# mit-han-lab/TinyChatEngine

Hardware: NVIDIA H100
Metric: llama3_8b_awq_int4_batch1_decode_tokens_per_s (higher is better)
Workload: dtype w4a16 (int4 weights; activations fp16 -> 32-bit block fixed point = four int8 digit planes; int32 accumulate, fp32 scale)

## Files before the change

### tinychatengine_b200/csrc/decode_persistent.cu

```cuda
#include <stdio.h>

#include "persistent.h"
#include "w4a16_act_planes.cuh"

namespace tce {
namespace pk {

namespace {

TCE_DEVINL unsigned ld_acquire_gpu(const unsigned *p) {
    unsigned v;
    asm volatile("ld.acquire.gpu.global.u32 %0, [%1];" : "=r"(v) : "l"(p) : "memory");
    return v;
}
TCE_DEVINL void red_release_gpu(unsigned *p) { asm volatile("red.release.gpu.global.add.u32 [%0], 1;" ::"l"(p) : "memory"); }

TCE_DEVINL void st_ll(uint2 *p, uint32_t data, uint32_t tag, bool sys) {
    if (sys)
        asm volatile("st.relaxed.sys.global.v2.b32 [%0], {%1, %2};" ::"l"(p), "r"(data), "r"(tag) : "memory");
    else
        asm volatile("st.relaxed.gpu.global.v2.b32 [%0], {%1, %2};" ::"l"(p), "r"(data), "r"(tag) : "memory");
}
TCE_DEVINL uint4 ld_ll2(const uint2 *p, bool sys) {
    uint4 r;
    if (sys)
        asm volatile("ld.relaxed.sys.global.v4.b32 {%0,%1,%2,%3}, [%4];" : "=r"(r.x), "=r"(r.y), "=r"(r.z), "=r"(r.w) : "l"(p) : "memory");
    else
        asm volatile("ld.relaxed.gpu.global.v4.b32 {%0,%1,%2,%3}, [%4];" : "=r"(r.x), "=r"(r.y), "=r"(r.z), "=r"(r.w) : "l"(p) : "memory");
    return r;
}
TCE_DEVINL uint2 ld_ll1(const uint2 *p, bool sys) {
    uint2 r;
    if (sys)
        asm volatile("ld.relaxed.sys.global.v2.b32 {%0,%1}, [%2];" : "=r"(r.x), "=r"(r.y) : "l"(p) : "memory");
    else
        asm volatile("ld.relaxed.gpu.global.v2.b32 {%0,%1}, [%2];" : "=r"(r.x), "=r"(r.y) : "l"(p) : "memory");
    return r;
}
constexpr unsigned kPeerPollBackoffNs = 100;
constexpr long long kSpinLimit = 20000000000LL;
TCE_DEVINL uint4 wait_ll2(const uint2 *p, uint32_t tag, bool sys) {
    uint4 r = ld_ll2(p, sys);
    if (r.y == tag && r.w == tag) return r;
    const long long t0 = clock64();
    while (true) {
        if (sys) __nanosleep(kPeerPollBackoffNs);
        r = ld_ll2(p, sys);
        if (r.y == tag && r.w == tag) return r;
        if (clock64() - t0 > kSpinLimit) __trap();
    }
}
TCE_DEVINL uint32_t wait_ll1(const uint2 *p, uint32_t tag, bool sys) {
    uint2 r = ld_ll1(p, sys);
    if (r.y == tag) return r.x;
    const long long t0 = clock64();
    while (true) {
        if (sys) __nanosleep(kPeerPollBackoffNs);
        r = ld_ll1(p, sys);
        if (r.y == tag) return r.x;
        if (clock64() - t0 > kSpinLimit) __trap();
    }
}
template <int N>
TCE_DEVINL void wait_ll2xN(const uint2 *p, uint32_t tag, bool sys, uint4 (&r)[N]) {
    long long t0 = 0;
    while (true) {
        bool ok = true;
#pragma unroll
        for (int i = 0; i < N; i++) r[i] = ld_ll2(p + 2 * i, sys);
#pragma unroll
        for (int i = 0; i < N; i++) ok = ok && (r[i].y == tag) && (r[i].w == tag);
        if (ok) return;
        if (t0 == 0) t0 = clock64();
        if (clock64() - t0 > kSpinLimit) __trap();
        if (sys) __nanosleep(kPeerPollBackoffNs);
    }
}

TCE_DEVINL float2 h2_to_f2(uint32_t u) { return __half22float2(*reinterpret_cast<const __half2 *>(&u)); }

TCE_DEVINL uint4 lds_u4(uint32_t a) {
    uint4 r;
    asm volatile("ld.shared.v4.u32 {%0,%1,%2,%3}, [%4];" : "=r"(r.x), "=r"(r.y), "=r"(r.z), "=r"(r.w) : "r"(a) : "memory");
    return r;
}
TCE_DEVINL uint2 lds_u2(uint32_t a) {
    uint2 r;
    asm volatile("ld.shared.v2.u32 {%0,%1}, [%2];" : "=r"(r.x), "=r"(r.y) : "r"(a) : "memory");
    return r;
}
TCE_DEVINL uint32_t lds_u32(uint32_t a) {
    uint32_t r;
    asm volatile("ld.shared.u32 %0, [%1];" : "=r"(r) : "r"(a) : "memory");
    return r;
}
TCE_DEVINL float lds_f32(uint32_t a) { return __uint_as_float(lds_u32(a)); }
TCE_DEVINL uint32_t lds_u16(uint32_t a) {
    unsigned short r;
    asm volatile("ld.shared.u16 %0, [%1];" : "=h"(r) : "r"(a) : "memory");
    return (uint32_t)r;
}
TCE_DEVINL bool mbar_try_wait_u32(uint32_t bar, uint32_t parity) {
    uint32_t ok;
    asm volatile("{\n\t.reg .pred p;\n\tmbarrier.try_wait.parity.shared::cta.b64 p, [%1], %2;\n\tselp.u32 %0, 1, 0, p;\n\t}" : "=r"(ok) : "r"(bar), "r"(parity) : "memory");
    return ok != 0;
}
TCE_DEVINL void mbar_wait_u32(uint32_t bar, uint32_t parity) {
    if (mbar_try_wait_u32(bar, parity)) return;
    const long long t0 = clock64();
    while (!mbar_try_wait_u32(bar, parity)) {
        if (clock64() - t0 > kSpinLimit) __trap();
    }
}
TCE_DEVINL void mbar_arrive_u32(uint32_t bar) { asm volatile("mbarrier.arrive.shared::cta.b64 _, [%0];" ::"r"(bar) : "memory"); }

TCE_DEVINL int lds_volatile_i32(const int *p) {
    int v;
    asm volatile("ld.volatile.shared.s32 %0, [%1];" : "=r"(v) : "r"(smem_u32(p)) : "memory");
    return v;
}

TCE_DEVINL void stamp(const Args &a, int cta, int nphase, int p, int k) {
    if (a.dbg) {
        unsigned long long t;
        asm volatile("mov.u64 %0, %%globaltimer;" : "=l"(t));
        a.dbg[((size_t)cta * nphase + p) * 8 + k] = t;
    }
}

TCE_DEVINL unsigned long long argmax_key(float v, int idx) {
    unsigned b = __float_as_uint(v);
    b = (b & 0x80000000u) ? ~b : (b | 0x80000000u);
    return ((unsigned long long)b << 32) | (unsigned long long)(0xFFFFFFFFu - (unsigned)idx);
}

struct PSmem {
    uint8_t *ring;
    uint8_t *xs;
    float *resid;
    float *gx;
    int *gsum;
    float *red;
    float *rms;
    float *rope;
    uint64_t *full, *empty, *red_full, *red_empty;
    uint64_t *rx;
    int *free_gen;
    int2 *red_pos;
    uint32_t ring_u32, xs_u32, gx_u32, gsum_u32, full_u32, empty_u32, redfull_u32, redempty_u32;
    int nst;
};

TCE_DEVINL PSmem carve(uint8_t *raw, const Args &a) {
    PSmem s;
    uint8_t *base = raw + ((1024u - (smem_u32(raw) & 1023u)) & 1023u);
    s.nst = a.nst;
    s.ring = base;
    uint8_t *p = base + (size_t)a.nst * kStageBytes;
    s.xs = p;
    p += a.xs_bytes;
    s.resid = reinterpret_cast<float *>(p);
    p += (size_t)a.E * 4;
    s.gx = reinterpret_cast<float *>(p);
    p += (size_t)a.max_ng * 4;
    s.gsum = reinterpret_cast<int *>(p);
    p += (size_t)a.max_ng * 8;
    s.red = reinterpret_cast<float *>(p);
    p += (size_t)kRedBufs * kCW * 16 * 4;
    s.rms = reinterpret_cast<float *>(p);
    p += 32 * 4;
    s.rope = reinterpret_cast<float *>(p);
    p += 256 * 4;
    s.full = reinterpret_cast<uint64_t *>(p);
    s.empty = s.full + a.nst;
    s.red_full = s.empty + a.nst;
    s.red_empty = s.red_full + kRedBufs;
    s.rx = s.red_empty + kRedBufs;
    s.free_gen = reinterpret_cast<int *>(s.rx + 1);
    s.red_pos = reinterpret_cast<int2 *>(s.rx + 2);
    s.ring_u32 = smem_u32(s.ring);
    s.xs_u32 = smem_u32(s.xs);
    s.gx_u32 = smem_u32(s.gx);
    s.gsum_u32 = smem_u32(s.gsum);
    s.full_u32 = smem_u32(s.full);
    s.empty_u32 = smem_u32(s.empty);
    s.redfull_u32 = smem_u32(s.red_full);
    s.redempty_u32 = smem_u32(s.red_empty);
    return s;
}

struct Ring {
    int stage = 0;
    uint32_t phase = 0;
    TCE_DEVINL void advance(int nst) {
        if (++stage == nst) {
            stage = 0;
            phase ^= 1;
        }
    }
};
struct Red {
    int rb = 0;
    uint32_t rphase = 0;
    TCE_DEVINL void advance() {
        if (++rb == kRedBufs) {
            rb = 0;
            rphase ^= 1;
        }
    }
};

TCE_DEVINL void partition(const GemvOp &op, int cta, int ncta, int &t0, int &t1) {
    const unsigned T = (unsigned)op.num_tiles;
    t0 = (int)((T * (unsigned)cta) / (unsigned)ncta);
    t1 = (int)((T * (unsigned)(cta + 1)) / (unsigned)ncta);
}

struct AttnSplit {
    int kvh, split, ch0, ch1, nsplit;
};
TCE_DEVINL AttnSplit attn_split(int cta, int ncta, int KVH, int pos) {
    AttnSplit s;
    const int T = pos + 1;
    const int nch = (T + kKvChunk - 1) / kKvChunk;
    int NS = ncta / KVH;
    if (NS < 1) NS = 1;
    int cps = (nch + NS - 1) / NS;
    if (cps * 32 < nch) cps = (nch + 31) / 32;
    s.nsplit = (nch + cps - 1) / cps;
    s.kvh = cta / NS;
    s.split = cta - s.kvh * NS;
    if (s.kvh >= KVH || s.split >= s.nsplit) {
        s.ch0 = s.ch1 = 0;
        s.kvh = 0;
    } else {
        s.ch0 = s.split * cps;
        s.ch1 = min(nch, s.ch0 + cps);
    }
    return s;
}

TCE_DEVINL void produce_gemv(const GemvOp &op, const CUtensorMap *m0, const uint8_t *meta, const PSmem &sm, Ring &rs, int cta, int ncta, uint32_t leader,
                             uint64_t policy) {
    int t0, t1;
    partition(op, cta, ncta, t0, t1);
    const uint32_t box_bytes = 16u * (uint32_t)op.bw * 64u;
    for (int tile = t0; tile < t1; tile++) {
        int row = op.pair ? tile * 8 : tile * 16;
        const CUtensorMap *m = m0;
        if (!op.pair && op.nseg > 1 && row >= op.rows0) {
            row -= op.rows0;
            m = m0 + 1;
            if (op.nseg > 2 && row >= op.rows1) {
                row -= op.rows1;
                m = m0 + 2;
            }
        }
        for (int s = 0; s < op.S; s++) {
            const int nbox = (min(kStageGroups, op.NG - kStageGroups * s) + 15) >> 4;
            mbar_wait(&sm.empty[rs.stage], rs.phase ^ 1);
            uint64_t *bar = &sm.full[rs.stage];
            uint8_t *dst = sm.ring + (size_t)rs.stage * kStageBytes;
            mbar_arrive_expect_tx_pred(bar, (uint32_t)nbox * box_bytes + kMetaBytes, leader);
#pragma unroll 1
            for (int b = 0; b < nbox; b++) {
                const int grp = kStageGroups * s + 16 * b;
                tma_load_3d_pred(dst + b * 16384, m, 0, row, grp, bar, policy, leader);
                if (op.pair) tma_load_3d_pred(dst + b * 16384 + 8192, m + 1, 0, row, grp, bar, policy, leader);
            }
            bulk_g2s_pred(dst + kMetaOff, meta + ((size_t)tile * op.S + s) * kMetaBytes, kMetaBytes, bar, policy, leader);
            __syncwarp();
            rs.advance(sm.nst);
        }
    }
}

TCE_DEVINL void produce_attn(const Args &a, const LayerDesc &L, const CUtensorMap *kvmap, const PSmem &sm, Ring &rs, int cta, int ncta, int pos,
                             uint32_t leader, uint64_t policy) {
    const AttnSplit sp = attn_split(cta, ncta, a.KVH, pos);
    for (int c = sp.ch0; c < sp.ch1; c++) {
        mbar_wait(&sm.empty[rs.stage], rs.phase ^ 1);
        uint64_t *bar = &sm.full[rs.stage];
        uint8_t *dst = sm.ring + (size_t)rs.stage * kStageBytes;
        const int krow = L.k_row0 + sp.kvh * a.max_ctx + c * kKvChunk, vrow = L.v_row0 + sp.kvh * a.max_ctx + c * kKvChunk;
        mbar_arrive_expect_tx_pred(bar, 2u * kHalfBytes, leader);
        tma_load_2d_pred(dst, kvmap, 0, krow, bar, policy, leader);
        tma_load_2d_pred(dst + 8192, kvmap, 64, krow, bar, policy, leader);
        tma_load_2d_pred(dst + kHalfBytes, kvmap, 0, vrow, bar, policy, leader);
        tma_load_2d_pred(dst + kHalfBytes + 8192, kvmap, 64, vrow, bar, policy, leader);
        __syncwarp();
        rs.advance(sm.nst);
    }
}

TCE_DEVINL void producer_walk(const Args &a, const PSmem &sm, int cta, int ncta, int pos, int lane) {
    Ring rs;
    const uint64_t policy = l2_policy_evict_first();
    const uint32_t leader = (lane == 0) ? 1u : 0u;
    const int Lyr = a.num_layers, nphase = 5 * Lyr + 1;
    const CUtensorMap *kvmap = a.maps + (size_t)Lyr * 7 + 1;
#pragma unroll 1
    for (int p = 0; p < nphase; p++) {
        const int l = p / 5, k = p - 5 * l;
        if (l == Lyr) {
            produce_gemv(a.op[OPI_LMHEAD], a.maps + (size_t)Lyr * 7, a.lm_meta, sm, rs, cta, ncta, leader, policy);
        } else if (k == 1) {
            produce_attn(a, a.layers[l], kvmap, sm, rs, cta, ncta, pos, leader, policy);
        } else {
            const int oi = (k == 0) ? OPI_QKV : (k - 1);
            const int mi = (k == 0) ? 0 : (k == 2 ? 3 : (k == 3 ? 4 : 6));
            produce_gemv(a.op[oi], a.maps + (size_t)l * 7 + mi, a.layers[l].meta[oi], sm, rs, cta, ncta, leader, policy);
        }
    }
}

struct PairCtx {
    bool on = false;
    uint32_t rank = 0;
    gemv::PairDst dst = {0u, 0u, 0u, 0u};
    uint32_t r_rms = 0, r_free = 0;
    uint32_t nstage = 0;
};
TCE_DEVINL uint32_t map_to_cta(uint32_t local_u32, uint32_t rank) {
    uint32_t r;
    asm volatile("mapa.shared::cluster.u32 %0, %1, %2;" : "=r"(r) : "r"(local_u32), "r"(rank));
    return r;
}
TCE_DEVINL void st_cluster_u32(uint32_t raddr, uint32_t v) { asm volatile("st.relaxed.cluster.shared::cluster.u32 [%0], %1;" ::"r"(raddr), "r"(v) : "memory"); }
TCE_DEVINL int own_groups(const PairCtx &pc, int NG) { return pc.on ? (NG + 1 - (int)pc.rank) / 2 : NG; }
TCE_DEVINL int peer_groups(const PairCtx &pc, int NG) { return pc.on ? (NG + (int)pc.rank) / 2 : 0; }
TCE_DEVINL void wait_partner_free(const PSmem &sm, const PairCtx &pc, int p) {
    if (!pc.on || p == 0) return;
    const long long t0 = clock64();
    while (lds_volatile_i32(sm.free_gen) < p) {
        if (clock64() - t0 > kSpinLimit) __trap();
    }
}
TCE_DEVINL void rx_expect(const PSmem &sm, const PairCtx &pc, uint32_t bytes) {
    asm volatile("mbarrier.arrive.expect_tx.shared::cta.b64 _, [%0], %1;" ::"r"(smem_u32(sm.rx)), "r"(bytes) : "memory");
}
TCE_DEVINL void rx_wait(const PSmem &sm, PairCtx &pc) {
    mbar_wait_u32(smem_u32(sm.rx), pc.nstage & 1u);
    pc.nstage++;
}

TCE_DEVINL int rot_unit(int u, int units, int cta) {
    const int ng = units >> 4;
    int g = (u >> 4) + (cta % ng);
    if (g >= ng) g -= ng;
    return (g << 4) | (u & 15);
}

TCE_DEVINL void stage_half(const GemvOp &op, const PSmem &sm, PairCtx &pc, const uint2 *src, uint32_t tag, int cta, int ctid, int lane, int p) {
    const int ng_own = own_groups(pc, op.NG);
    const int units = ng_own * 16;
    if (pc.on) {
        if (ctid == 0) rx_expect(sm, pc, (uint32_t)peer_groups(pc, op.NG) * 524u);
        wait_partner_free(sm, pc, p);
    }
    constexpr int PRE = 4;
    for (int ub = 0; ub < units; ub += PRE * kConsumerThreads) {
        uint4 w[PRE][2];
        int ui[PRE];
#pragma unroll
        for (int k = 0; k < PRE; k++) {
            const int u = ub + k * kConsumerThreads + ctid;
            ui[k] = -1;
            if (u < units) {
                const int ru = rot_unit(u, units, cta);
                ui[k] = pc.on ? (((ru >> 4) * 2 + (int)pc.rank) << 4) | (ru & 15) : ru;
            }
            w[k][0] = w[k][1] = make_uint4(0u, tag, 0u, tag);
            if (ui[k] >= 0) {
                w[k][0] = ld_ll2(src + (size_t)ui[k] * 4, false);
                w[k][1] = ld_ll2(src + (size_t)ui[k] * 4 + 2, false);
            }
        }
        {
            long long t0 = 0;
            while (true) {
                bool ok = true;
#pragma unroll
                for (int k = 0; k < PRE; k++) ok = ok && w[k][0].y == tag && w[k][0].w == tag && w[k][1].y == tag && w[k][1].w == tag;
                if (ok) break;
                if (t0 == 0) t0 = clock64();
                if (clock64() - t0 > kSpinLimit) __trap();
#pragma unroll
                for (int k = 0; k < PRE; k++) {
                    if (ui[k] >= 0 && !(w[k][0].y == tag && w[k][0].w == tag && w[k][1].y == tag && w[k][1].w == tag)) {
                        w[k][0] = ld_ll2(src + (size_t)ui[k] * 4, false);
                        w[k][1] = ld_ll2(src + (size_t)ui[k] * 4 + 2, false);
                    }
                }
            }
            __syncwarp();
        }
#pragma unroll
        for (int k = 0; k < PRE; k++) {
            if (ub + k * kConsumerThreads >= units) break;
            const bool valid = ui[k] >= 0;
            float v[8];
            const float2 f0 = h2_to_f2(w[k][0].x), f1 = h2_to_f2(w[k][0].z), f2 = h2_to_f2(w[k][1].x), f3 = h2_to_f2(w[k][1].z);
            v[0] = f0.x; v[1] = f0.y; v[2] = f1.x; v[3] = f1.y;
            v[4] = f2.x; v[5] = f2.y; v[6] = f3.x; v[7] = f3.y;
            if (pc.on)
                gemv::emit_unit<1, true>(sm.xs, op.IC, sm.gx, sm.gsum, valid ? ui[k] : 0, valid, v, lane, &pc.dst);
            else
                gemv::emit_unit<1>(sm.xs, op.IC, sm.gx, sm.gsum, valid ? ui[k] : 0, valid, v, lane);
        }
    }
    named_bar_sync(1, kConsumerThreads);
    if (pc.on) rx_wait(sm, pc);
}

TCE_DEVINL void tp_accumulate(float (&x)[8], const uint2 *slot0, int tp_size, int E, uint32_t tag) {
    int pr = 0;
    for (; pr + 2 <= tp_size; pr += 2) {
        const uint2 *pa = slot0 + (size_t)pr * E, *pb = pa + E;
        uint4 wa[4], wb[4];
        long long t0 = 0;
        while (true) {
            bool ok = true;
#pragma unroll
            for (int i = 0; i < 4; i++) wa[i] = ld_ll2(pa + 2 * i, true);
#pragma unroll
            for (int i = 0; i < 4; i++) wb[i] = ld_ll2(pb + 2 * i, true);
#pragma unroll
            for (int i = 0; i < 4; i++) ok = ok && wa[i].y == tag && wa[i].w == tag && wb[i].y == tag && wb[i].w == tag;
            if (ok) break;
            if (t0 == 0) t0 = clock64();
            if (clock64() - t0 > kSpinLimit) __trap();
            __nanosleep(kPeerPollBackoffNs);
        }
        x[0] += __uint_as_float(wa[0].x); x[1] += __uint_as_float(wa[0].z); x[2] += __uint_as_float(wa[1].x); x[3] += __uint_as_float(wa[1].z);
        x[4] += __uint_as_float(wa[2].x); x[5] += __uint_as_float(wa[2].z); x[6] += __uint_as_float(wa[3].x); x[7] += __uint_as_float(wa[3].z);
        x[0] += __uint_as_float(wb[0].x); x[1] += __uint_as_float(wb[0].z); x[2] += __uint_as_float(wb[1].x); x[3] += __uint_as_float(wb[1].z);
        x[4] += __uint_as_float(wb[2].x); x[5] += __uint_as_float(wb[2].z); x[6] += __uint_as_float(wb[3].x); x[7] += __uint_as_float(wb[3].z);
    }
    if (pr < tp_size) {
        uint4 w[4];
        wait_ll2xN<4>(slot0 + (size_t)pr * E, tag, true, w);
        x[0] += __uint_as_float(w[0].x); x[1] += __uint_as_float(w[0].z); x[2] += __uint_as_float(w[1].x); x[3] += __uint_as_float(w[1].z);
        x[4] += __uint_as_float(w[2].x); x[5] += __uint_as_float(w[2].z); x[6] += __uint_as_float(w[3].x); x[7] += __uint_as_float(w[3].z);
    }
}

TCE_DEVINL float stage_rms(const Args &a, const GemvOp &op, const PSmem &sm, PairCtx &pc, const uint2 *delta, uint32_t tag, const float *gamma, int token,
                           bool first, bool emit, int cta, int ctid, int cw, int lane, int p) {
    const int units = own_groups(pc, op.NG) * 16;
    const bool sys = a.tp_size > 1;
    if (pc.on && emit) {
        if (ctid == 0) rx_expect(sm, pc, (uint32_t)peer_groups(pc, op.NG) * 524u + (uint32_t)kCW * 4u);
        wait_partner_free(sm, pc, p);
    }
    float ss = 0.f;
    for (int ui0 = 0; ui0 < units; ui0 += kConsumerThreads) {
        const int u = ui0 + ctid;
        const bool valid = u < units;
        int ui = 0;
        if (valid) {
            const int ru = rot_unit(u, units, cta);
            ui = pc.on ? (((ru >> 4) * 2 + (int)pc.rank) << 4) | (ru & 15) : ru;
        }
        float x[8], v[8];
#pragma unroll
        for (int i = 0; i < 8; i++) x[i] = 0.f;
        float4 g0 = make_float4(0.f, 0.f, 0.f, 0.f), g1 = g0;
        if (valid) {
            g0 = *reinterpret_cast<const float4 *>(gamma + (size_t)ui * 8);
            g1 = *reinterpret_cast<const float4 *>(gamma + (size_t)ui * 8 + 4);
            if (first) {
                const uint4 raw = *reinterpret_cast<const uint4 *>(a.embed + (size_t)token * a.E + (size_t)ui * 8);
                const __half2 *h2 = reinterpret_cast<const __half2 *>(&raw);
#pragma unroll
                for (int i = 0; i < 4; i++) {
                    const float2 f = __half22float2(h2[i]);
                    x[2 * i] = f.x;
                    x[2 * i + 1] = f.y;
                }
            } else {
                const float4 r0 = *reinterpret_cast<const float4 *>(sm.resid + (size_t)ui * 8);
                const float4 r1 = *reinterpret_cast<const float4 *>(sm.resid + (size_t)ui * 8 + 4);
                x[0] = r0.x; x[1] = r0.y; x[2] = r0.z; x[3] = r0.w;
                x[4] = r1.x; x[5] = r1.y; x[6] = r1.z; x[7] = r1.w;
                if (a.tp_size == 1) {
                    uint4 w[4];
                    wait_ll2xN<4>(delta + (size_t)ui * 8, tag, false, w);
                    x[0] += __uint_as_float(w[0].x); x[1] += __uint_as_float(w[0].z); x[2] += __uint_as_float(w[1].x); x[3] += __uint_as_float(w[1].z);
                    x[4] += __uint_as_float(w[2].x); x[5] += __uint_as_float(w[2].z); x[6] += __uint_as_float(w[3].x); x[7] += __uint_as_float(w[3].z);
                } else {
                    tp_accumulate(x, delta + (size_t)ui * 8, a.tp_size, a.E, tag);
                }
            }
            *reinterpret_cast<float4 *>(sm.resid + (size_t)ui * 8) = make_float4(x[0], x[1], x[2], x[3]);
            *reinterpret_cast<float4 *>(sm.resid + (size_t)ui * 8 + 4) = make_float4(x[4], x[5], x[6], x[7]);
        }
        if (emit) {
#pragma unroll
            for (int i = 0; i < 8; i++) ss += x[i] * x[i];
            v[0] = x[0] * g0.x; v[1] = x[1] * g0.y; v[2] = x[2] * g0.z; v[3] = x[3] * g0.w;
            v[4] = x[4] * g1.x; v[5] = x[5] * g1.y; v[6] = x[6] * g1.z; v[7] = x[7] * g1.w;
            if (pc.on)
                gemv::emit_unit<1, true>(sm.xs, op.IC, sm.gx, sm.gsum, ui, valid, v, lane, &pc.dst);
            else
                gemv::emit_unit<1>(sm.xs, op.IC, sm.gx, sm.gsum, ui, valid, v, lane);
        }
    }
    if (!emit) return 1.f;
    ss = warp_sum(ss);
    if (lane == 0) {
        sm.rms[pc.rank * kCW + cw] = ss;
        if (pc.on) gemv::st_async_b32(pc.r_rms + (uint32_t)(pc.rank * kCW + cw) * 4u, __float_as_uint(ss), pc.dst.bar);
    }
    named_bar_sync(1, kConsumerThreads);
    if (pc.on) rx_wait(sm, pc);
    float tot = 0.f;
    const int nparts = pc.on ? 2 * kCW : kCW;
    for (int w = 0; w < nparts; w++) tot += sm.rms[w];
    return rsqrtf(tot / (float)op.IC + a.eps);
}

struct UnitRegs {
    uint4 wa, wb, xe, xo;
    uint32_t z;
    uint32_t sc;
    int sxv;
    float st;
};
TCE_DEVINL void unit_compute(const UnitRegs &u, float lscale, float &totA, float &totB) {
    constexpr uint32_t ML = 0x0f0f0f0fu, MH = 0xf0f0f0f0u;
    int accL[4], accH[4];
    mma_m16n8k32_u8s8_z(accL, u.wa.x & ML, u.wb.x & ML, u.wa.y & ML, u.wb.y & ML, u.xe.x, u.xe.y);
    mma_m16n8k32_u8s8_z(accH, u.wa.x & MH, u.wb.x & MH, u.wa.y & MH, u.wb.y & MH, u.xo.x, u.xo.y);
    mma_m16n8k32_u8s8(accL, u.wa.z & ML, u.wb.z & ML, u.wa.w & ML, u.wb.w & ML, u.xe.z, u.xe.w);
    mma_m16n8k32_u8s8(accH, u.wa.z & MH, u.wb.z & MH, u.wa.w & MH, u.wb.w & MH, u.xo.z, u.xo.w);
    const float2 sc = h2_to_f2(u.sc);
    const float st = u.st * lscale;
    const int zAq = (int)(u.z & 0xFFu), zBq = (int)(u.z >> 8);
    const int vA = (accL[0] << 8) + accL[1] + (((accH[0] << 8) + accH[1]) >> 4) - zAq * u.sxv;
    const int vB = (accL[2] << 8) + accL[3] + (((accH[2] << 8) + accH[3]) >> 4) - zBq * u.sxv;
    totA += (sc.x * st) * (float)vA;
    totB += (sc.y * st) * (float)vB;
}

TCE_DEVINL void consume_gemv(const Args &a, const GemvOp &op, const PSmem &sm, Ring &rs, float inv_in, int cta, int ncta, int cw, int p, int nphase) {
    int lane;
    asm volatile("mov.u32 %0, %%laneid;" : "=r"(lane));
    const float inv = __shfl_sync(0xffffffffu, inv_in, 0);
    Red cs;
    {
        const int2 rp = sm.red_pos[cw];
        cs.rb = rp.x;
        cs.rphase = (uint32_t)rp.y;
    }
    const int g = lane >> 2, t = lane & 3;
    int t0, t1;
    partition(op, cta, ncta, t0, t1);
    const int NG = op.NG, S = op.S;
    const uint32_t w_lane = (uint32_t)cw * (op.pair ? 512u : 1024u) + (uint32_t)g * 64u + (uint32_t)t * 16u;
    const uint32_t wb_off = op.pair ? 8192u : 512u;
    const uint32_t m_lane = (uint32_t)kMetaOff + (uint32_t)(cw * 8 + g) * 4u;
    const uint32_t z_lane = (uint32_t)kMetaOff + 1024u + (uint32_t)(cw * 8 + g) * 2u;
    const uint32_t x_lane = sm.xs_u32 + (uint32_t)((g >> 1) & 1) * (uint32_t)op.IC * 2u + (uint32_t)(t * 2 + (g & 1)) * 16u + (uint32_t)cw * 256u;
    const uint32_t s_lane = sm.gsum_u32 + (uint32_t)(2 * cw + (t & 1)) * 4u;
    const uint32_t q_lane = sm.gx_u32 + (uint32_t)cw * 4u;
    const float lscale = (t == 0) ? 65536.f : (t == 1 ? 1.f : 0.f);
    const bool xl = g < 4;
    if (a.dbg && t1 > t0 && cw == 0 && lane == 0) {
        mbar_wait_u32(sm.full_u32 + (uint32_t)rs.stage * 8u, rs.phase);
        stamp(a, cta, nphase, p, 4);
    }
    for (int tile = t0; tile < t1; tile++) {
        float totA = 0.f, totB = 0.f;
        for (int s = 0; s < S; s++) {
            const bool has0 = kStageGroups * s + cw < NG, has1 = kStageGroups * s + cw + 16 < NG;
            mbar_wait_u32(sm.full_u32 + (uint32_t)rs.stage * 8u, rs.phase);
            const uint32_t base = sm.ring_u32 + (uint32_t)rs.stage * (uint32_t)kStageBytes;
            const uint32_t wb_ = base + w_lane, mb_ = base + m_lane, zb_ = base + z_lane;
            const uint32_t xb_ = x_lane + (uint32_t)s * (kStageGroups * 256u), sb_ = s_lane + (uint32_t)s * (kStageGroups * 8u), qb_ = q_lane + (uint32_t)s * (kStageGroups * 4u);
            UnitRegs u0, u1;
            u0.xe = u0.xo = u1.xe = u1.xo = make_uint4(0u, 0u, 0u, 0u);
            if (has0) {
                u0.wa = lds_u4(wb_);
                u0.wb = lds_u4(wb_ + wb_off);
                if (xl) {
                    u0.xe = lds_u4(xb_);
                    u0.xo = lds_u4(xb_ + 128u);
                }
                u0.sc = lds_u32(mb_);
                u0.z = lds_u16(zb_);
                u0.sxv = (int)lds_u32(sb_);
                u0.st = lds_f32(qb_);
            }
            if (has1) {
                u1.wa = lds_u4(wb_ + 16384u);
                u1.wb = lds_u4(wb_ + 16384u + wb_off);
                if (xl) {
                    u1.xe = lds_u4(xb_ + 4096u);
                    u1.xo = lds_u4(xb_ + 4096u + 128u);
                }
                u1.sc = lds_u32(mb_ + 512u);
                u1.z = lds_u16(zb_ + 256u);
                u1.sxv = (int)lds_u32(sb_ + 128u);
                u1.st = lds_f32(qb_ + 64u);
            }
            if (has0) unit_compute(u0, lscale, totA, totB);
            if (has1) unit_compute(u1, lscale, totA, totB);
            __syncwarp();
            if (lane == 0) mbar_arrive_u32(sm.empty_u32 + (uint32_t)rs.stage * 8u);
            rs.advance(sm.nst);
        }
        if (tile == t1 - 1 && cw == 0 && lane == 0) stamp(a, cta, nphase, p, 5);
        totA += __shfl_xor_sync(0xffffffffu, totA, 1);
        totB += __shfl_xor_sync(0xffffffffu, totB, 1);
        mbar_wait_u32(sm.redempty_u32 + (uint32_t)cs.rb * 8u, cs.rphase ^ 1);
        float *rbuf = sm.red + ((size_t)cs.rb * kCW + cw) * 16;
        if (t == 0) {
            rbuf[g] = totA * inv;
            rbuf[g + 8] = totB * inv;
        }
        __syncwarp();
        if (lane == 0) mbar_arrive_u32(sm.redfull_u32 + (uint32_t)cs.rb * 8u);
        cs.advance();
    }
    __syncwarp();
    if (lane == 0) sm.red_pos[cw] = make_int2(cs.rb, (int)cs.rphase);
    __syncwarp();
    if (cw == 0 && lane == 0) stamp(a, cta, nphase, p, 6);
}

struct EpiState {
    unsigned long long best;
};

TCE_DEVINL void epilogue_gemv(const Args &a, const GemvOp &op, const PSmem &sm, Red &es, EpiState &st, uint2 *out_ll, int which, uint32_t tag, int cta, int ncta,
                              int p, int nphase) {
    int lane;
    asm volatile("mov.u32 %0, %%laneid;" : "=r"(lane));
    int t0, t1;
    partition(op, cta, ncta, t0, t1);
    const bool tp = a.tp_size > 1;
    for (int tile = t0; tile < t1; tile++) {
        mbar_wait_u32(sm.redfull_u32 + (uint32_t)es.rb * 8u, es.rphase);
        if (tile == t1 - 1 && lane == 0) stamp(a, cta, nphase, p, 7);
        const float *rbuf = sm.red + (size_t)es.rb * kCW * 16;
        float v = 0.f;
        {
            const int row = lane & 15, w0 = (lane >> 4) * 8;
#pragma unroll
            for (int w = 0; w < 8; w++) v += rbuf[(w0 + w) * 16 + row];
        }
        v += __shfl_down_sync(0xffffffffu, v, 16);
        __syncwarp();
        if (lane == 0) mbar_arrive_u32(sm.redempty_u32 + (uint32_t)es.rb * 8u);
        es.advance();
        switch (op.epi) {
            case PE_DELTA_LL:
                if (lane < 16) {
                    const size_t o = (size_t)a.tp_rank * a.E + (size_t)tile * 16 + lane;
                    if (tp) {
                        for (int pr = 0; pr < a.tp_size; pr++) st_ll(a.tp_delta[which][pr] + o, __float_as_uint(v), tag, true);
                    } else {
                        st_ll(out_ll + o, __float_as_uint(v), tag, false);
                    }
                }
                break;
            case PE_HALF_LL: {
                const float hi = __shfl_down_sync(0xffffffffu, v, 1);
                if (lane < 16 && !(lane & 1)) st_ll(out_ll + (size_t)tile * 8 + (lane >> 1), pack_half2(v, hi), tag, false);
                break;
            }
            case PE_SILU_LL: {
                const float up = __shfl_down_sync(0xffffffffu, v, 8);
                const float y = v / (1.f + __expf(-v)) * up;
                const float yhi = __shfl_down_sync(0xffffffffu, y, 1);
                if (lane < 8 && !(lane & 1)) st_ll(out_ll + (size_t)tile * 4 + (lane >> 1), pack_half2(y, yhi), tag, false);
                break;
            }
            case PE_LOGITS:
                if (lane < 16) {
                    const int idx = tile * 16 + lane;
                    a.logits[idx] = v;
                    const unsigned long long key = argmax_key(v, a.vocab_base + idx);
                    st.best = key > st.best ? key : st.best;
                }
                break;
        }
    }
}

TCE_DEVINL uint32_t kv_off(int r, int c) { return (uint32_t)((c >> 3) * 8192 + r * 128 + (((c & 7) ^ (r & 7)) << 4)); }

TCE_DEVINL float2 rope_pair(const uint2 *vec, int j, uint32_t tag, const float *cosr, const float *sinr) {
    const uint2 *pa = vec + j, *pb = vec + (j < 32 ? j + 32 : j - 32);
    uint2 wa = ld_ll1(pa, false), wb = ld_ll1(pb, false);
    if (wa.y != tag) wa.x = wait_ll1(pa, tag, false);
    if (wb.y != tag) wb.x = wait_ll1(pb, tag, false);
    const float2 x = h2_to_f2(wa.x), xp = h2_to_f2(wb.x);
    const float sgn = (j < 32) ? -1.f : 1.f;
    const int d = 2 * j;
    return make_float2(x.x * cosr[d] + sgn * xp.x * sinr[d], x.y * cosr[d + 1] + sgn * xp.y * sinr[d + 1]);
}

TCE_DEVINL void attention_phase(const Args &a, const LayerDesc &L, const PSmem &sm, Ring &rs, uint32_t tag_qkv, uint32_t tag_part, uint32_t tag_out, int cta,
                                int ncta, int pos, int ctid, int cw, int lane, int p, int nphase) {
    const AttnSplit sp = attn_split(cta, ncta, a.KVH, pos);
    const int nrep = a.nrep;
    const int g = lane >> 2, t = lane & 3;
    if (sp.ch0 < sp.ch1) {
        __half *sQ = reinterpret_cast<__half *>(sm.xs);
        float *sO = reinterpret_cast<float *>(sm.xs + 8 * 136 * 2);
        float *sML = sO + (size_t)kCW * nrep * 128;
        uint32_t *sKV = reinterpret_cast<uint32_t *>(sML + (size_t)kCW * nrep * 2);
        const float *cosr = sm.rope, *sinr = sm.rope + 128;
        const bool owns_new = sp.ch1 * kKvChunk > pos;
        static_assert(8 * 64 == kConsumerThreads, "one pass");
        {
            const int r = ctid >> 6, j = ctid & 63;
            float2 v = make_float2(0.f, 0.f);
            if (r < nrep) {
                v = rope_pair(a.qkv_ll + (size_t)(sp.kvh * nrep + r) * 64, j, tag_qkv, cosr, sinr);
                v.x *= a.alpha;
                v.y *= a.alpha;
            } else if (owns_new && r == 7) {
                const float2 kr = rope_pair(a.qkv_ll + (size_t)a.H * 64 + (size_t)sp.kvh * 64, j, tag_qkv, cosr, sinr);
                const __half2 kh = __floats2half2_rn(kr.x, kr.y);
                sKV[j] = *reinterpret_cast<const uint32_t *>(&kh);
            } else if (owns_new && r == 6) {
                sKV[64 + j] = wait_ll1(a.qkv_ll + (size_t)(a.H + a.KVH) * 64 + (size_t)sp.kvh * 64 + j, tag_qkv, false);
            }
            *reinterpret_cast<__half2 *>(sQ + r * 136 + 2 * j) = __floats2half2_rn(v.x, v.y);
        }
        named_bar_sync(1, kConsumerThreads);
        if (ctid == 0) stamp(a, cta, nphase, p, 4);
        const uint32_t qa_u32 = smem_u32(sQ + g * 136 + t * 2);
        float m_run = -INFINITY, l_run = 0.f;
        bool have = false;
        float *myO = sO + (size_t)cw * nrep * 128;
        const int kb = cw & 3;
        for (int c = sp.ch0; c < sp.ch1; c++) {
            const int kbase = c * kKvChunk + kb * 16;
            const bool mine = (((c - sp.ch0) & 3) == (cw >> 2)) && (kbase <= pos);
            const bool has_new = mine && pos < kbase + 16;
            mbar_wait_u32(sm.full_u32 + (uint32_t)rs.stage * 8u, rs.phase);
            if (c == sp.ch0 && ctid == 0) stamp(a, cta, nphase, p, 7);
            if (mine) {
                uint8_t *kst = sm.ring + (size_t)rs.stage * kStageBytes, *vst = kst + kHalfBytes;
                if (has_new) {
                    const int r = pos - c * kKvChunk;
#pragma unroll
                    for (int i = 0; i < 2; i++) {
                        const int j = lane * 2 + i;
                        const uint32_t kh = sKV[j], vv = sKV[64 + j];
                        *reinterpret_cast<uint32_t *>(kst + kv_off(r, j >> 2) + (j & 3) * 4) = kh;
                        *reinterpret_cast<uint32_t *>(vst + kv_off(r, j >> 2) + (j & 3) * 4) = vv;
                        *reinterpret_cast<uint32_t *>(L.k_cache + ((size_t)sp.kvh * a.max_ctx + pos) * 128 + 2 * j) = kh;
                        *reinterpret_cast<uint32_t *>(L.v_cache + ((size_t)sp.kvh * a.max_ctx + pos) * 128 + 2 * j) = vv;
                    }
                    for (int rr = r + 1; rr < kb * 16 + 16; rr++)
                        *reinterpret_cast<uint2 *>(vst + kv_off(rr, lane >> 1) + (lane & 1) * 8) = make_uint2(0u, 0u);
                    asm volatile("fence.proxy.async.shared::cta;" ::: "memory");
                    __syncwarp();
                }
                float s0[4] = {0.f, 0.f, 0.f, 0.f}, s1[4] = {0.f, 0.f, 0.f, 0.f};
                {
                    const int lr = (lane & 7) + ((lane >> 4) << 3);
                    const int lc = (lane >> 3) & 1;
#pragma unroll
                    for (int ks = 0; ks < 8; ks++) {
                        uint32_t b0, b1, b2, b3;
                        ldmatrix_x4(b0, b1, b2, b3, kst + kv_off(kb * 16 + lr, 2 * ks + lc));
                        const uint32_t qa0 = lds_u32(qa_u32 + ks * 32u), qa1 = lds_u32(qa_u32 + ks * 32u + 16u);
                        mma_m16n8k16(s0, qa0, 0u, qa1, 0u, b0, b1);
                        mma_m16n8k16(s1, qa0, 0u, qa1, 0u, b2, b3);
                    }
                }
                const int k0 = kbase + 2 * t;
                float e0 = (k0 <= pos) ? s0[0] : -INFINITY, e1 = (k0 + 1 <= pos) ? s0[1] : -INFINITY;
                float e2 = (k0 + 8 <= pos) ? s1[0] : -INFINITY, e3 = (k0 + 9 <= pos) ? s1[1] : -INFINITY;
                float mb = fmaxf(fmaxf(e0, e1), fmaxf(e2, e3));
                mb = fmaxf(mb, __shfl_xor_sync(0xffffffffu, mb, 1));
                mb = fmaxf(mb, __shfl_xor_sync(0xffffffffu, mb, 2));
                const float m_new = fmaxf(m_run, mb);
                e0 = __expf(e0 - m_new);
                e1 = __expf(e1 - m_new);
                e2 = __expf(e2 - m_new);
                e3 = __expf(e3 - m_new);
                float lb = (e0 + e1) + (e2 + e3);
                lb += __shfl_xor_sync(0xffffffffu, lb, 1);
                lb += __shfl_xor_sync(0xffffffffu, lb, 2);
                const float sc_old = have ? __expf(m_run - m_new) : 0.f;
                l_run = l_run * sc_old + lb;
                m_run = m_new;
                const uint32_t pa0 = pack_half2(e0, e1), pa2 = pack_half2(e2, e3);
                const int lr = (lane & 7) + (((lane >> 3) & 1) << 3);
                const int lc = lane >> 4;
#pragma unroll
                for (int h = 0; h < 2; h++) {
                    float oacc[8][4];
#pragma unroll
                    for (int j = 0; j < 8; j++) oacc[j][0] = oacc[j][1] = oacc[j][2] = oacc[j][3] = 0.f;
#pragma unroll
                    for (int jp = 0; jp < 4; jp++) {
                        uint32_t b0, b1, b2, b3;
                        ldmatrix_x4_t(b0, b1, b2, b3, vst + kv_off(kb * 16 + lr, 8 * h + 2 * jp + lc));
                        mma_m16n8k16(oacc[2 * jp], pa0, 0u, pa2, 0u, b0, b1);
                        mma_m16n8k16(oacc[2 * jp + 1], pa0, 0u, pa2, 0u, b2, b3);
                    }
                    if (g < nrep) {
#pragma unroll
                        for (int j = 0; j < 8; j++) {
                            float2 *dst = reinterpret_cast<float2 *>(myO + g * 128 + 64 * h + 8 * j + 2 * t);
                            float2 nv = make_float2(oacc[j][0], oacc[j][1]);
                            if (have) {
                                const float2 old = *dst;
                                nv.x += old.x * sc_old;
                                nv.y += old.y * sc_old;
                            }
                            *dst = nv;
                        }
                    }
                }
                have = true;
            }
            __syncwarp();
            if (lane == 0) mbar_arrive_u32(sm.empty_u32 + (uint32_t)rs.stage * 8u);
            rs.advance(sm.nst);
        }
        if (ctid == 0) stamp(a, cta, nphase, p, 5);
        if (t == 0 && g < nrep) {
            sML[(cw * nrep + g) * 2] = have ? m_run : -INFINITY;
            sML[(cw * nrep + g) * 2 + 1] = have ? l_run : 0.f;
        }
        named_bar_sync(1, kConsumerThreads);
        const int r = ctid >> 7, d = ctid & 127;
        if (ctid < nrep * 128) {
            float o = 0.f, M = -INFINITY, Lsum = 0.f;
            for (int w = 0; w < kCW; w++) M = fmaxf(M, sML[(w * nrep + r) * 2]);
            for (int w = 0; w < kCW; w++) {
                const float mw = sML[(w * nrep + r) * 2];
                if (mw != -INFINITY) {
                    const float wt = __expf(mw - M);
                    Lsum += wt * sML[(w * nrep + r) * 2 + 1];
                    o += wt * sO[((size_t)w * nrep + r) * 128 + d];
                }
            }
            const int head = sp.kvh * nrep + r;
            if (sp.nsplit == 1) {
                const float y = o / Lsum;
                const float yhi = __shfl_down_sync(0xffffffffu, y, 1);
                if (!(d & 1)) st_ll(a.attn_ll + (size_t)head * 64 + (d >> 1), pack_half2(y, yhi), tag_out, false);
            } else {
                uint2 *rec = a.part_ll + ((size_t)head * a.nsplit_max + sp.split) * 130;
                st_ll(rec + d, __float_as_uint(o), tag_part, false);
                if (d == 0) {
                    st_ll(rec + 128, __float_as_uint(M), tag_part, false);
                    st_ll(rec + 129, __float_as_uint(Lsum), tag_part, false);
                }
            }
        }
    }
    if (ctid == 0) stamp(a, cta, nphase, p, 6);
    if (sp.nsplit == 1) return;
    const int ntask = a.H * 4;
    for (int task = cta + cw * ncta; task < ntask; task += ncta * kCW) {
        const int head = task >> 2, d = ((task & 3) << 5) + lane;
        const uint2 *base = a.part_ll + (size_t)head * a.nsplit_max * 130;
        constexpr int kRound = 20;
        uint2 wm = make_uint2(0u, tag_part), wl = wm;
        uint2 ow[kRound];
#pragma unroll
        for (int i = 0; i < kRound; i++) ow[i] = make_uint2(0u, tag_part);
        {
            const bool stat = lane < sp.nsplit;
            if (stat) wm.y = wl.y = tag_part + 1u;
#pragma unroll
            for (int i = 0; i < kRound; i++)
                if (i < sp.nsplit) ow[i].y = tag_part + 1u;
            long long t0 = 0;
            while (true) {
                if (wm.y != tag_part) wm = ld_ll1(base + (size_t)lane * 130 + 128, false);
                if (wl.y != tag_part) wl = ld_ll1(base + (size_t)lane * 130 + 129, false);
#pragma unroll
                for (int i = 0; i < kRound; i++)
                    if (ow[i].y != tag_part) ow[i] = ld_ll1(base + (size_t)i * 130 + d, false);
                bool ok = wm.y == tag_part && wl.y == tag_part;
#pragma unroll
                for (int i = 0; i < kRound; i++) ok = ok && ow[i].y == tag_part;
                if (ok) break;
                if (t0 == 0) t0 = clock64();
                if (clock64() - t0 > kSpinLimit) __trap();
            }
            __syncwarp();
        }
        const float ms = (lane < sp.nsplit) ? __uint_as_float(wm.x) : -INFINITY, ls = (lane < sp.nsplit) ? __uint_as_float(wl.x) : 0.f;
        const float M = warp_max(ms);
        const float wgt = (lane < sp.nsplit) ? __expf(ms - M) : 0.f;
        const float Lt = warp_sum(wgt * ls);
        float acc = 0.f;
#pragma unroll
        for (int i = 0; i < kRound; i++) acc += __shfl_sync(0xffffffffu, wgt, i) * __uint_as_float(ow[i].x);
        for (int s0 = kRound; s0 < sp.nsplit; s0++)
            acc += __shfl_sync(0xffffffffu, wgt, s0) * __uint_as_float(wait_ll1(base + (size_t)s0 * 130 + d, tag_part, false));
        const float y = acc / Lt;
        const float yhi = __shfl_down_sync(0xffffffffu, y, 1);
        if (!(lane & 1)) st_ll(a.attn_ll + (size_t)head * 64 + (d >> 1), pack_half2(y, yhi), tag_out, false);
    }
}

__global__ void __launch_bounds__(kThreads, 1) decode_persistent_kernel(const __grid_constant__ Args a) {
    extern __shared__ uint8_t smem_raw[];
    const PSmem sm = carve(smem_raw, a);
    const int tid = threadIdx.x, warp = tid >> 5, lane = tid & 31;
    const int cta = blockIdx.x, ncta = gridDim.x;
    const int Lyr = a.num_layers;
    const int token = a.tokpos[0], pos = a.tokpos[1];
    if (token < 0 || token >= a.embed_rows || pos < 0 || pos >= a.max_ctx) {
        if (cta == 0 && tid == 0) {
            *a.error = 1;
            *a.next_token = -1;
        }
        return;
    }
    if (warp == 0) {
        if (lane < a.nst) {
            mbar_init(&sm.full[lane], 1);
            mbar_init(&sm.empty[lane], kCW);
        } else if (lane >= 16 && lane < 16 + kRedBufs) {
            mbar_init(&sm.red_full[lane - 16], kCW);
            mbar_init(&sm.red_empty[lane - 16], 1);
        }
        if (lane == 30) {
            mbar_init(sm.rx, 1);
            *sm.free_gen = 0;
        }
        mbar_fence_init();
    }
    __syncthreads();
    PairCtx pc;
    if (a.pair) {
        asm volatile("barrier.cluster.arrive.release.aligned;" ::: "memory");
        asm volatile("barrier.cluster.wait.acquire.aligned;" ::: "memory");
        pc.on = true;
        asm volatile("mov.u32 %0, %%cluster_ctarank;" : "=r"(pc.rank));
        const uint32_t peer = pc.rank ^ 1u;
        pc.dst.xs = map_to_cta(sm.xs_u32, peer);
        pc.dst.gx = map_to_cta(sm.gx_u32, peer);
        pc.dst.gsum = map_to_cta(sm.gsum_u32, peer);
        pc.dst.bar = map_to_cta(smem_u32(sm.rx), peer);
        pc.r_rms = map_to_cta(smem_u32(sm.rms), peer);
        pc.r_free = map_to_cta(smem_u32(sm.free_gen), peer);
    }
    const int nphase = 5 * Lyr + 1;
    const unsigned epoch = *a.epoch;
    const uint32_t tag_base = epoch * (uint32_t)(2 * nphase + 2) + 1u;

    if (warp < kAuxWarps) {
        asm volatile("setmaxnreg.dec.sync.aligned.u32 64;" ::: "memory");
        if (warp >= 2) return;
        if (warp == 0) {
            producer_walk(a, sm, cta, ncta, pos, lane);
            return;
        }
        Red es;
        EpiState st;
        st.best = 0ull;
#pragma unroll 1
        for (int p = 0; p < nphase; p++) {
            const int l = p / 5, k = p - 5 * l;
            if (l < Lyr && k == 1) continue;
            const int oi = (l == Lyr) ? OPI_LMHEAD : ((k == 0) ? OPI_QKV : (k - 1));
            uint2 *out = (oi == OPI_QKV) ? a.qkv_ll : (oi == OPI_GATEUP ? a.act_ll : (oi == OPI_O ? a.delta_ll[0] : a.delta_ll[1]));
            epilogue_gemv(a, a.op[oi], sm, es, st, out, (oi == OPI_DOWN) ? 1 : 0, tag_base + 2u * (uint32_t)p, cta, ncta, p, nphase);
            if (lane == 0) stamp(a, cta, nphase, p, 3);
        }
        unsigned long long key = st.best;
#pragma unroll
        for (int off = 16; off > 0; off >>= 1) {
            const unsigned long long other = __shfl_xor_sync(0xffffffffu, key, off);
            key = other > key ? other : key;
        }
        if (lane == 0 && key) atomicMax(a.argmax_cell, key);
        __threadfence();
        __syncwarp();
        if (lane == 0) red_release_gpu(a.done);
        return;
    }
    asm volatile("setmaxnreg.inc.sync.aligned.u32 104;" ::: "memory");

    const int ctid = tid - 32 * kAuxWarps;
    const int cw = warp - kAuxWarps;
    Ring rs;
    if (lane == 0) sm.red_pos[cw] = make_int2(0, 0);
    __syncwarp();
    if (ctid < 256) sm.rope[ctid] = (ctid < 128) ? a.cos[(size_t)pos * 128 + ctid] : a.sin[(size_t)pos * 128 + ctid - 128];
#pragma unroll 1
    for (int p = 0; p < nphase; p++) {
        const int l = p / 5, k = p - 5 * l;
        const uint32_t tag_in = tag_base + 2u * (uint32_t)(p - 1);
        if (ctid == 0) stamp(a, cta, nphase, p, 0);
        if (l < Lyr && k == 1) {
            attention_phase(a, a.layers[l], sm, rs, tag_in, tag_base + 2u * (uint32_t)p + 1u, tag_base + 2u * (uint32_t)p, cta, ncta, pos, ctid, cw, lane, p, nphase);
            if (ctid == 0) stamp(a, cta, nphase, p, 2);
            named_bar_sync(1, kConsumerThreads);
            if (pc.on && ctid == 0) st_cluster_u32(pc.r_free, (uint32_t)(p + 1));
            continue;
        }
        const int oi = (l == Lyr) ? OPI_LMHEAD : ((k == 0) ? OPI_QKV : (k - 1));
        const GemvOp &op = a.op[oi];
        int t0, t1;
        partition(op, cta, ncta, t0, t1);
        const bool work = t1 > t0;
        bool stage = work;
        if (pc.on) {
            int u0, u1;
            partition(op, cta ^ 1, ncta, u0, u1);
            stage = work || u1 > u0;
        }
        float inv = 1.f;
        if (oi == OPI_O) {
            if (stage) stage_half(op, sm, pc, a.attn_ll, tag_in, cta, ctid, lane, p);
        } else if (oi == OPI_DOWN) {
            if (stage) stage_half(op, sm, pc, a.act_ll, tag_in, cta, ctid, lane, p);
        } else {
            const float *gamma = (oi == OPI_LMHEAD) ? a.final_norm : (oi == OPI_QKV ? a.layers[l].input_norm : a.layers[l].post_norm);
            const uint2 *delta = (oi == OPI_GATEUP) ? a.delta_ll[0] : a.delta_ll[1];
            inv = stage_rms(a, op, sm, pc, delta, tag_in, gamma, token, p == 0, stage, cta, ctid, cw, lane, p);
        }
        if (ctid == 0) stamp(a, cta, nphase, p, 1);
        if (work) consume_gemv(a, op, sm, rs, inv, cta, ncta, cw, p, nphase);
        if (ctid == 0) stamp(a, cta, nphase, p, 2);
        named_bar_sync(1, kConsumerThreads);
        if (pc.on && ctid == 0 && p + 1 < nphase) st_cluster_u32(pc.r_free, (uint32_t)(p + 1));
    }
    if (cta == 0 && ctid == 0) {
        const unsigned target = (epoch + 1u) * (unsigned)ncta;
        const long long t0 = clock64();
        while ((int)(ld_acquire_gpu(a.done) - target) < 0) {
            if (clock64() - t0 > kSpinLimit) __trap();
        }
        unsigned long long key = *reinterpret_cast<volatile unsigned long long *>(a.argmax_cell);
        if (a.tp_size > 1) {
            const uint32_t tag = tag_base + 2u * (uint32_t)nphase;
            for (int pr = 0; pr < a.tp_size; pr++) {
                st_ll(a.tp_keys[pr] + (size_t)a.tp_rank * 2, (uint32_t)(key >> 32), tag, true);
                st_ll(a.tp_keys[pr] + (size_t)a.tp_rank * 2 + 1, (uint32_t)key, tag, true);
            }
            key = 0ull;
            for (int pr = 0; pr < a.tp_size; pr++) {
                const uint32_t hi = wait_ll1(a.tp_keys[a.tp_rank] + (size_t)pr * 2, tag, true), lo = wait_ll1(a.tp_keys[a.tp_rank] + (size_t)pr * 2 + 1, tag, true);
                const unsigned long long k2 = ((unsigned long long)hi << 32) | lo;
                key = k2 > key ? k2 : key;
            }
        }
        *a.next_token = (int)(0xFFFFFFFFu - (unsigned)(key & 0xFFFFFFFFull));
        *a.argmax_cell = 0ull;
        *a.epoch = epoch + 1u;
    }
}

__global__ void repack_meta_kernel(W4Seg s0, W4Seg s1, W4Seg s2, int nseg, int pair, int NG, int zeros_w, int sf_w, int S, int num_tiles, uint8_t *out) {
    const int idx = blockIdx.x * blockDim.x + threadIdx.x;
    if (idx >= num_tiles * S * kStageGroups) return;
    const int gi = idx % kStageGroups, su = idx / kStageGroups;
    const int tile = su / S, s = su - tile * S;
    const int G = kStageGroups * s + gi;
    uint8_t *rec = out + (size_t)su * kMetaBytes;
    __half *so = reinterpret_cast<__half *>(rec) + gi * 16;
    uint8_t *zo = rec + 1024 + gi * 16;
    for (int r = 0; r < 16; r++) {
        const W4Seg *seg = &s0;
        int row;
        if (pair) {
            seg = (r < 8) ? &s0 : &s1;
            row = tile * 8 + (r & 7);
        } else {
            row = tile * 16 + r;
            if (nseg > 1 && row >= s0.rows) {
                row -= s0.rows;
                seg = &s1;
                if (nseg > 2 && row >= s1.rows) {
                    row -= s1.rows;
                    seg = &s2;
                }
            }
        }
        const int slot = (r & 7) * 2 + (r >> 3);
        if (G < NG) {
            so[slot] = seg->scales[(size_t)row * sf_w + G];
            zo[slot] = (uint8_t)((seg->zeros[(size_t)row * zeros_w + (G >> 3)] >> ((G & 7) * 4)) & 0xFu);
        } else {
            so[slot] = __float2half(0.f);
            zo[slot] = 0;
        }
    }
}

}

int attn_scratch_bytes(int nrep) { return 8 * 136 * 2 + kCW * nrep * 128 * 4 + kCW * nrep * 2 * 4 + 2 * 64 * 4; }

int attn_nsplit_max(int ncta, int KVH, int max_ctx) {
    int NS = ncta / KVH;
    if (NS < 1) NS = 1;
    const int nch = (max_ctx + kKvChunk - 1) / kKvChunk;
    return NS < nch ? NS : nch;
}

static size_t fixed_bytes(int xs_bytes, int max_ng, int E) {
    return (size_t)xs_bytes + (size_t)E * 4 + (size_t)max_ng * 12 + (size_t)kRedBufs * kCW * 16 * 4 + 32 * 4 + 256 * 4 + (size_t)(2 * kMaxStages + 2 * kRedBufs) * 8 + 16 +
           (size_t)kCW * 8 + 1024;
}
int pick_stages(int smem_optin, int xs_bytes, int max_ng, int E) {
    const long long avail = (long long)smem_optin - (long long)fixed_bytes(xs_bytes, max_ng, E);
    long long n = avail / kStageBytes;
    if (n > kMaxStages) n = kMaxStages;
    return n < 2 ? 0 : (int)n;
}
size_t smem_bytes(const Args &a) { return fixed_bytes(a.xs_bytes, a.max_ng, a.E) + (size_t)a.nst * kStageBytes; }

cudaError_t repack_meta(Ctx *ctx, const W4Seg *segs, int nseg, int pair, int IC, uint8_t *out, cudaStream_t stream) {
    const int NG = IC / kW4Group, S = (NG + kStageGroups - 1) / kStageGroups;
    int rows = 0;
    for (int i = 0; i < nseg; i++) rows += segs[i].rows;
    const int num_tiles = rows / 16;
    const int zw = zeros_width(IC, kW4Group);
    const int total = num_tiles * S * kStageGroups;
    if (total == 0) return cudaSuccess;
    repack_meta_kernel<<<(total + 127) / 128, 128, 0, stream>>>(segs[0], segs[nseg > 1 ? 1 : 0], segs[nseg > 2 ? 2 : 0], nseg, pair, NG, zw, zw * 8, S, num_tiles, out);
    (void)ctx;
    return cudaGetLastError();
}

cudaError_t encode_kv_tmap(CUtensorMap *out, const void *kv, long long rows) {
    const TmapEncodeFn fn = tmap_encoder();
    if (!fn) return cudaErrorNotSupported;
    const cuuint64_t gdim[2] = {128, (cuuint64_t)rows};
    const cuuint64_t gstride[1] = {256};
    const cuuint32_t box[2] = {64, (cuuint32_t)kKvChunk};
    const cuuint32_t estr[2] = {1, 1};
    const CUresult r = fn(out, CU_TENSOR_MAP_DATA_TYPE_UINT16, 2, const_cast<void *>(kv), gdim, gstride, box, estr, CU_TENSOR_MAP_INTERLEAVE_NONE,
                          CU_TENSOR_MAP_SWIZZLE_128B, CU_TENSOR_MAP_L2_PROMOTION_L2_256B, CU_TENSOR_MAP_FLOAT_OOB_FILL_NONE);
    return r == CUDA_SUCCESS ? cudaSuccess : cudaErrorInvalidValue;
}

bool pair_supported(Ctx *ctx, const Args &a) {
    if (ctx->num_sms % 2) return false;
    const size_t smem = smem_bytes(a);
    if (cudaFuncSetAttribute(decode_persistent_kernel, cudaFuncAttributeMaxDynamicSharedMemorySize, ctx->smem_optin) != cudaSuccess) return false;
    cudaLaunchConfig_t cfg = {};
    cfg.gridDim = dim3(ctx->num_sms);
    cfg.blockDim = dim3(kThreads);
    cfg.dynamicSmemBytes = smem;
    cudaLaunchAttribute attr[1];
    attr[0].id = cudaLaunchAttributeClusterDimension;
    attr[0].val.clusterDim.x = 2;
    attr[0].val.clusterDim.y = 1;
    attr[0].val.clusterDim.z = 1;
    cfg.attrs = attr;
    cfg.numAttrs = 1;
    int nclusters = 0;
    if (cudaOccupancyMaxActiveClusters(&nclusters, decode_persistent_kernel, &cfg) != cudaSuccess) {
        cudaGetLastError();
        return false;
    }
    return nclusters * 2 >= ctx->num_sms;
}

cudaError_t launch(Ctx *ctx, const Args &a, cudaStream_t stream) {
    const size_t smem = smem_bytes(a);
    if ((int)smem > ctx->smem_optin) return cudaErrorInvalidConfiguration;
    cudaError_t e = cudaFuncSetAttribute(decode_persistent_kernel, cudaFuncAttributeMaxDynamicSharedMemorySize, ctx->smem_optin);
    if (e != cudaSuccess) return e;
    cudaLaunchConfig_t cfg = {};
    cfg.gridDim = dim3(ctx->num_sms);
    cfg.blockDim = dim3(kThreads);
    cfg.dynamicSmemBytes = smem;
    cfg.stream = stream;
    cudaLaunchAttribute attr[2];
    attr[0].id = cudaLaunchAttributeCooperative;
    attr[0].val.cooperative = 1;
    cfg.attrs = attr;
    cfg.numAttrs = 1;
    static bool pair_refused = false;
    if (a.pair && !pair_refused) {
        cudaLaunchAttribute cattr[1];
        cattr[0].id = cudaLaunchAttributeClusterDimension;
        cattr[0].val.clusterDim.x = 2;
        cattr[0].val.clusterDim.y = 1;
        cattr[0].val.clusterDim.z = 1;
        cfg.attrs = cattr;
        cfg.numAttrs = 1;
        e = cudaLaunchKernelEx(&cfg, decode_persistent_kernel, a);
        if (e == cudaSuccess) return e;
        cudaGetLastError();
        pair_refused = true;
        cfg.attrs = attr;
        cfg.numAttrs = 1;
    }
    Args single = a;
    single.pair = 0;
    return cudaLaunchKernelEx(&cfg, decode_persistent_kernel, single);
}

}
}
```

### tinychatengine_b200/csrc/kernels.h

```cpp
#pragma once
#include <cuda.h>
#include <cuda_fp16.h>
#include <cuda_runtime.h>
#include <stdint.h>

#include <atomic>

namespace tce {

struct Ctx {
    int device = 0;
    cudaStream_t stream = nullptr;
    int num_sms = 0;
    int smem_optin = 0;
    float *gemv_partials = nullptr;
    int gemv_partial_records = 0;
    unsigned *gemv_counters = nullptr;
    int gemv_max_ctas = 0;
    int gemv_max_tiles = 0;
    unsigned long long *gemv_dbg = nullptr;
    unsigned long long *gemv_dbg_keep = nullptr;
    unsigned option_gen = 0;
    float *opt_seed = nullptr;
    unsigned attn_seed_epoch = 0;
    int gemv_impl = 1;
    int gemv_ctas_per_sm = 1;
    int gemv_consumer_warps = 8;
    int gemv_stages = 8;
    bool use_pdl = false;
    int pdl_early = 0;
    __half *w16_scratch = nullptr;
    size_t w16_scratch_elems = 0;
    int gemm_min_m = 16;
};

struct DeviceOnce {
    std::atomic<unsigned long long> mask{0};
    bool pending(int device) const { return !((mask.load(std::memory_order_acquire) >> (device & 63)) & 1ull); }
    void done(int device) { mask.fetch_or(1ull << (device & 63), std::memory_order_release); }
};

constexpr int kW4Group = 128;

inline int zeros_width(int ic, int group) {
    int mult = group >= 128 ? 1 : (group == 64 ? 2 : 4);
    int base = (ic / group + 7) / 8;
    return (base + mult - 1) / mult * mult;
}

enum XMode : int { X_HALF = 0, X_RMSNORM_F32 = 1 };
enum EpiMode : int { EPI_STORE_HALF = 0, EPI_STORE_F32 = 1, EPI_ADD_F32 = 2, EPI_SILU_MUL_HALF = 3 };
constexpr int kMaxTP = 8;

struct W4Seg {
    const uint32_t *w;
    const uint32_t *zeros;
    const __half *scales;
    int rows;
};

struct W4GemvParams {
    W4Seg seg[3];
    int nseg = 1;
    int pair_mode = 0;
    int IC = 0;
    int M = 1;
    const void *x = nullptr;
    int x_mode = X_HALF;
    int ldx = 0;
    const float *gamma = nullptr;
    float eps = 0.f;
    void *y = nullptr;
    int epi = EPI_STORE_HALF;
    int ldy = 0;
    bool pdl = false;
    bool atomic_residual = false;
};

cudaError_t launch_w4a16_gemv(Ctx *ctx, const W4GemvParams &p);
long long w4a16_gemv_fixup_records(const Ctx *ctx, const W4GemvParams &p);
cudaError_t gemv_partials_reserve(Ctx *ctx, long long records);
cudaError_t launch_w4a16_gemv_simple(Ctx *ctx, const W4GemvParams &p);
cudaError_t launch_w4a16_gemv_g64(Ctx *ctx, const __half *x, const uint32_t *w, const uint32_t *zeros, const __half *scales, __half *y, int M, int IC, int OC);
cudaError_t encode_w4_tmap(CUtensorMap *out, const void *w, int rows, int IC, int sg, int box_rows);
cudaError_t encode_w4_tmap_units(CUtensorMap *out, const void *w, int rows, int IC, int sg, int box_rows);

cudaError_t launch_naive_fp16_int4(Ctx *ctx, const __half *A, const int32_t *B, const __half *scales, __half *C, int M, int IC, int OC, int block);
cudaError_t launch_f32_matmul_transposed(Ctx *ctx, const float *A, const float *B, float *C, int M, int N, int K);

cudaError_t launch_w4_expand(Ctx *ctx, const uint32_t *w, const uint32_t *zeros, const __half *scales, __half *out, int OC, int IC);
cudaError_t launch_gemm_f16_pair(Ctx *ctx, const __half *X, long long ldx, const __half *W, long long ldw, void *C, long long ldc, int M, int N, int K, int add_f32);
cudaError_t launch_gemm_f16_pair_silu(Ctx *ctx, const __half *X, long long ldx, const __half *W, long long ldw, __half *act, long long ldc, int M, int F, int K);
cudaError_t w4_scratch_reserve(Ctx *ctx, size_t elems);

struct alignas(16) LmStat {
    float m, s;
    int id, unused;
};
cudaError_t launch_gemm_f16_pair_stats(Ctx *ctx, const __half *X, long long ldx, const __half *W, long long ldw, int M, int N, int K, int col0, LmStat *stats,
                                       int stats_ld, const int *target, float *tgt, float *logits, long long ld_logits);
cudaError_t launch_lm_stats_merge(Ctx *ctx, const LmStat *stats, int stats_ld, int n_rec, int rows, bool first, bool last, LmStat *state, const int *target,
                                  const float *tgt, float *logprob, int *greedy, float *greedy_logprob);

struct StreamK {
    long long U;
    int nc;
    int NG;
    int aligned = 0;
    int T = 0;
    int gran = 1;
    __host__ __device__ long long start(int c) const {
        const long long n = aligned ? (long long)T : U / gran;
        const long long q = (n * nc < 0x7fffffffLL) ? (long long)(((unsigned)n * (unsigned)c) / (unsigned)nc) : (n * (long long)c) / nc;
        return q * (aligned ? NG : gran);
    }
    __host__ __device__ int cta_of(long long u) const {
        const long long Ug = U / gran, ug = u / gran;
        return (int)(((ug + 1) * nc + Ug - 1) / Ug - 1);
    }
};

struct SliceWalk {
    int T, NG, sl, nsl;
    __host__ __device__ int len(int s) const { return s < nsl - 1 ? sl : NG - s * sl; }
    __host__ __device__ int slice(int u) const {
        if (nsl == 1) return 0;
        const int s = u / (T * sl);
        return s < nsl - 1 ? s : nsl - 1;
    }
    __host__ __device__ void locate(int u, int &s, int &rt, int &gb, int &seg0) const {
        s = slice(u);
        const int base = s * T * sl, L = len(s);
        rt = (u - base) / L;
        seg0 = base + rt * L;
        gb = s * sl + (u - seg0);
    }
    __host__ __device__ int seg_unit(long long k) const {
        const long long kf = (long long)T * (nsl - 1);
        return (int)(k <= kf ? k * sl : kf * sl + (k - kf) * (NG - (nsl - 1) * sl));
    }
    __host__ __device__ int start(const StreamK &sk, int c) const {
        if (nsl == 1) return (int)sk.start(c);
        return seg_unit((long long)T * nsl * c / sk.nc);
    }
};

}
```

### tinychatengine_b200/csrc/llama_decoder.cu

```cuda
#include "llama_decoder.h"

#include "persistent.h"

#include <math.h>
#include <stdio.h>
#include <stdlib.h>
#include <string.h>

namespace tce {

#define DCK(call)                              \
    do {                                       \
        cudaError_t e__ = (call);              \
        if (e__ != cudaSuccess) return e__;    \
    } while (0)

static bool w4_ok(const tce_w4_tensor &t, int oc, int ic) { return t.w && t.zeros && t.scales && t.oc == oc && t.ic == ic; }

LlamaDecoder *LlamaDecoder::create(Ctx *ctx, int attn_chunk, const tce_llama_config &cfg, const tce_llama_weights &w, std::string *err) {
    auto bad = [&](const char *m) {
        *err = m;
        return (LlamaDecoder *)nullptr;
    };
    if (cfg.head_dim != 128) return bad("head_dim must be 128");
    if (cfg.num_layers < 1 || cfg.num_heads < 1 || cfg.num_kv_heads < 1 || cfg.num_heads % cfg.num_kv_heads) return bad("bad head configuration");
    if (cfg.embed_dim % 128 || cfg.hidden_dim % 128) return bad("embed_dim / hidden_dim must be multiples of the 128 group");
    if (cfg.tp_size > kMaxTP || cfg.tp_size < 0 || (cfg.tp_size > 1 && (cfg.tp_rank < 0 || cfg.tp_rank >= cfg.tp_size))) return bad("bad tensor-parallel rank/size");
    const bool persistent = getenv("TCE_PERSISTENT") ? atoi(getenv("TCE_PERSISTENT")) != 0 : true;
    if (cfg.tp_size > 1 && !persistent) return bad("tensor parallelism runs on the persistent decode kernel only (TCE_PERSISTENT=0 turns it off)");
    const int E = cfg.embed_dim, F = cfg.hidden_dim, H = cfg.num_heads, KVH = cfg.num_kv_heads, hd = cfg.head_dim, V = cfg.vocab_size;
    if (!w.embed_f16 || !w.layers || !w.final_norm) return bad("missing weights");
    if (!w4_ok(w.lm_head, V, E) || V % 16) return bad("lm_head shape");
    for (int l = 0; l < cfg.num_layers; l++) {
        const tce_llama_layer &L = w.layers[l];
        if (!w4_ok(L.q, H * hd, E) || !w4_ok(L.k, KVH * hd, E) || !w4_ok(L.v, KVH * hd, E) || !w4_ok(L.o, E, H * hd) || !w4_ok(L.gate, F, E) ||
            !w4_ok(L.up, F, E) || !w4_ok(L.down, E, F) || !L.input_norm || !L.post_norm)
            return bad("layer weight shape");
    }
    LlamaDecoder *d = new LlamaDecoder();
    d->ctx_ = ctx;
    d->attn_chunk_ = attn_chunk;
    d->cfg_ = cfg;
    d->w_ = w;
    d->layers_.assign(w.layers, w.layers + cfg.num_layers);
    d->w_.layers = d->layers_.data();
    d->use_graphs_ = getenv("TCE_NO_GRAPH") == nullptr;
    d->atomic_residual_ = getenv("TCE_DETERMINISTIC") == nullptr;
    const size_t kv_elems = (size_t)cfg.num_layers * 2 * KVH * cfg.max_ctx * hd;
    cudaError_t e = cudaSuccess;
    auto A = [&](auto &p, size_t count) {
        if (e == cudaSuccess) e = dev_alloc(p, count);
    };
    A(d->d_kv_, kv_elems);
    if (e == cudaSuccess) e = cudaMemset(d->d_kv_.get(), 0, kv_elems * sizeof(__half));
    if (e == cudaSuccess) e = d->io1_.alloc(1, V);
    if (e == cudaSuccess) e = cudaStreamCreateWithFlags(&d->cap_stream_, cudaStreamNonBlocking);
    if (e == cudaSuccess) {
        if (w.rope_cos && w.rope_sin) {
            d->d_cos_ = w.rope_cos;
            d->d_sin_ = w.rope_sin;
        } else {
            std::vector<float> hc((size_t)cfg.max_ctx * hd), hs((size_t)cfg.max_ctx * hd);
            const double theta = cfg.rope_theta > 0 ? cfg.rope_theta : 10000.0;
            for (int p = 0; p < cfg.max_ctx; p++)
                for (int i = 0; i < hd / 2; i++) {
                    const double inv = 1.0 / pow(theta, (2.0 * i) / hd);
                    const double ang = p * inv;
                    hc[(size_t)p * hd + i] = hc[(size_t)p * hd + i + hd / 2] = (float)cos(ang);
                    hs[(size_t)p * hd + i] = hs[(size_t)p * hd + i + hd / 2] = (float)sin(ang);
                }
            A(d->rope_, 2 * hc.size());
            if (e == cudaSuccess) e = cudaMemcpy(d->rope_.get(), hc.data(), hc.size() * sizeof(float), cudaMemcpyHostToDevice);
            if (e == cudaSuccess) e = cudaMemcpy(d->rope_.get() + hc.size(), hs.data(), hs.size() * sizeof(float), cudaMemcpyHostToDevice);
            d->d_cos_ = d->rope_.get();
            d->d_sin_ = d->rope_.get() + hc.size();
        }
    }
    if (e != cudaSuccess) {
        *err = std::string("allocation failed: ") + cudaGetErrorString(e);
        delete d;
        return nullptr;
    }
    d->persistent_ = persistent;
    d->tp_ = cfg.tp_size > 1 ? cfg.tp_size : 1;
    if (d->tp_ > 1) {
        d->tp_bytes_ = ((size_t)2 * d->tp_ * E + (size_t)2 * d->tp_) * sizeof(uint2);
        if (dev_alloc(d->tp_buf_, d->tp_bytes_) != cudaSuccess || cudaMemset(d->tp_buf_.get(), 0, d->tp_bytes_) != cudaSuccess) {
            *err = "tensor-parallel buffer allocation failed";
            delete d;
            return nullptr;
        }
        cudaDeviceSynchronize();
        return d;
    }
    if (d->persistent_) {
        std::string why;
        cudaError_t me = d->build_persistent(&why);
        if (me == cudaErrorNotSupported) {
            d->persistent_ = false;
        } else if (me != cudaSuccess) {
            *err = std::string("persistent kernel setup failed: ") + why + " " + cudaGetErrorString(me);
            delete d;
            return nullptr;
        }
    }
    return d;
}

LlamaDecoder::~LlamaDecoder() {
    if (cap_stream_) cudaStreamDestroy(cap_stream_);
    for (int b = 0; b < 2; b++) {
        if (pf_expanded_[b]) cudaEventDestroy(pf_expanded_[b]);
        if (pf_consumed_[b]) cudaEventDestroy(pf_consumed_[b]);
    }
    if (pf_side_) cudaStreamDestroy(pf_side_);
    for (int p = 0; p < tp_; p++)
        if (p != cfg_.tp_rank && tp_peer_[p]) cudaIpcCloseMemHandle(tp_peer_[p]);
}

void *LlamaDecoder::kv_cache_slot(int slot, int layer, int which) const {
    if (slot < 0 || slot >= n_slots() || layer < 0 || layer >= cfg_.num_layers || which < 0 || which > 1) return nullptr;
    const size_t per = (size_t)cfg_.num_kv_heads * cfg_.max_ctx * cfg_.head_dim;
    return (slot == 0 ? d_kv_ : slot_kv_[slot - 1]).get() + ((size_t)layer * 2 + which) * per;
}

static W4Seg seg_of(const tce_w4_tensor &t) { return W4Seg{(const uint32_t *)t.w, (const uint32_t *)t.zeros, (const __half *)t.scales, t.oc}; }

cudaError_t LlamaDecoder::enqueue_gemvs(int *count) {
    DCK(batch_alloc(nullptr));
    for (const W4GemvParams &p : bs_->gemv_ops) DCK(launch_w4a16_gemv(ctx_, p));
    *count = (int)bs_->gemv_ops.size();
    return cudaSuccess;
}

cudaError_t LlamaDecoder::tp_handle(void *out64) {
    if (tp_ <= 1 || !tp_buf_) return cudaErrorInvalidValue;
    static_assert(sizeof(cudaIpcMemHandle_t) == 64, "handle size");
    return cudaIpcGetMemHandle(reinterpret_cast<cudaIpcMemHandle_t *>(out64), tp_buf_.get());
}

cudaError_t LlamaDecoder::tp_connect(const void *handles, std::string *err) {
    if (tp_ <= 1) return cudaErrorInvalidValue;
    const cudaIpcMemHandle_t *h = reinterpret_cast<const cudaIpcMemHandle_t *>(handles);
    for (int p = 0; p < tp_; p++) {
        if (p == cfg_.tp_rank) {
            tp_peer_[p] = tp_buf_.get();
        } else {
            DCK(cudaIpcOpenMemHandle((void **)&tp_peer_[p], h[p], cudaIpcMemLazyEnablePeerAccess));
        }
    }
    DCK(build_persistent(err));
    tp_connected_ = true;
    return cudaSuccess;
}

cudaError_t LlamaDecoder::build_persistent(std::string *err) {
    const int E = cfg_.embed_dim, F = cfg_.hidden_dim, H = cfg_.num_heads, KVH = cfg_.num_kv_heads, hd = cfg_.head_dim, V = cfg_.vocab_size;
    const int Lyr = cfg_.num_layers, ncta = ctx_->num_sms;
    const int nrep = H / KVH;
    auto no = [&](const char *m) {
        if (err) *err = m;
        return cudaErrorNotSupported;
    };
    if (hd != 128 || nrep > 4 || ncta < KVH || F % 16 || V % 16) return no("shape outside the persistent kernel's envelope");
    int coop = 0;
    cudaDeviceGetAttribute(&coop, cudaDevAttrCooperativeLaunch, ctx_->device);
    if (!coop) return no("device cannot launch cooperative kernels");
    pk::Args a{};
    auto mk = [&](int IC, int rows, int nseg, int pair, int rows0, int rows1, int x_mode, int epi) {
        pk::GemvOp o{};
        o.IC = IC;
        o.NG = IC / kW4Group;
        o.S = (o.NG + pk::kStageGroups - 1) / pk::kStageGroups;
        o.num_tiles = rows / 16;
        o.nseg = nseg;
        o.pair = pair;
        o.rows0 = rows0;
        o.rows1 = rows1;
        o.x_mode = x_mode;
        o.epi = epi;
        return o;
    };
    const bool tp = tp_ > 1;
    a.op[pk::OPI_QKV] = mk(E, (H + 2 * KVH) * hd, 3, 0, H * hd, KVH * hd, pk::PX_RMS_F32, pk::PE_HALF_LL);
    a.op[pk::OPI_O] = mk(H * hd, E, 1, 0, E, 0, pk::PX_HALF, pk::PE_DELTA_LL);
    a.op[pk::OPI_GATEUP] = mk(E, 2 * F, 2, 1, F, F, pk::PX_RMS_F32, pk::PE_SILU_LL);
    a.op[pk::OPI_DOWN] = mk(F, E, 1, 0, E, 0, pk::PX_HALF, pk::PE_DELTA_LL);
    a.op[pk::OPI_LMHEAD] = mk(E, V, 1, 0, V, 0, pk::PX_RMS_F32, pk::PE_LOGITS);
    int max_ic = 0, max_ng = 0;
    for (int i = 0; i < pk::OPI_COUNT; i++) {
        a.op[i].bw = a.op[i].NG < 16 ? a.op[i].NG : 16;
        if (a.op[i].IC > max_ic) max_ic = a.op[i].IC;
        if (a.op[i].NG > max_ng) max_ng = a.op[i].NG;
        if (a.op[i].IC % kW4Group || a.op[i].num_tiles < 1) return no("bad GEMV shape");
    }
    max_ng = (max_ng + 3) & ~3;
    int xs = 4 * max_ic;
    if (xs < pk::attn_scratch_bytes(nrep)) xs = pk::attn_scratch_bytes(nrep);
    xs = (xs + 15) & ~15;
    a.xs_bytes = xs;
    a.max_ng = max_ng;
    a.E = E;
    a.nst = pk::pick_stages(ctx_->smem_optin, xs, max_ng, E);
    if (a.nst < 2) return no("shared memory too small for the persistent kernel");
    a.pair = 0;

    auto dalloc = [&](size_t bytes) -> void * {
        DevPtr<uint8_t> p;
        if (dev_alloc(p, bytes ? bytes : 16) != cudaSuccess) return nullptr;
        pk_allocs_.push_back(std::move(p));
        return pk_allocs_.back().get();
    };
    cudaStream_t s = ctx_->stream;
    std::vector<CUtensorMap> maps((size_t)Lyr * 7 + 2);
    memset(maps.data(), 0, maps.size() * sizeof(CUtensorMap));
    std::vector<pk::LayerDesc> descs(Lyr);
    const size_t per_kv = (size_t)KVH * cfg_.max_ctx;
    for (int l = 0; l < Lyr; l++) {
        const tce_llama_layer &L = layers_[l];
        const tce_w4_tensor *t7[7] = {&L.q, &L.k, &L.v, &L.o, &L.gate, &L.up, &L.down};
        const int opi[7] = {pk::OPI_QKV, pk::OPI_QKV, pk::OPI_QKV, pk::OPI_O, pk::OPI_GATEUP, pk::OPI_GATEUP, pk::OPI_DOWN};
        for (int i = 0; i < 7; i++) {
            const pk::GemvOp &o = a.op[opi[i]];
            DCK(encode_w4_tmap_units(&maps[(size_t)l * 7 + i], t7[i]->w, t7[i]->oc, t7[i]->ic, o.bw, o.pair ? 8 : 16));
        }
        pk::LayerDesc &D = descs[l];
        memset(&D, 0, sizeof(D));
        const W4Seg qkv[3] = {seg_of(L.q), seg_of(L.k), seg_of(L.v)}, o1[1] = {seg_of(L.o)}, gu[2] = {seg_of(L.gate), seg_of(L.up)}, d1[1] = {seg_of(L.down)};
        const W4Seg *segs[4] = {qkv, o1, gu, d1};
        const int nsegs[4] = {3, 1, 2, 1}, pairs[4] = {0, 0, 1, 0};
        const int ops4[4] = {pk::OPI_QKV, pk::OPI_O, pk::OPI_GATEUP, pk::OPI_DOWN};
        for (int i = 0; i < 4; i++) {
            const pk::GemvOp &o = a.op[ops4[i]];
            uint8_t *m = (uint8_t *)dalloc((size_t)o.num_tiles * o.S * pk::kMetaBytes);
            if (!m) return cudaErrorMemoryAllocation;
            DCK(pk::repack_meta(ctx_, segs[i], nsegs[i], pairs[i], o.IC, m, s));
            D.meta[i] = m;
        }
        D.input_norm = L.input_norm;
        D.post_norm = L.post_norm;
        D.k_cache = (__half *)kv_cache(l, 0);
        D.v_cache = (__half *)kv_cache(l, 1);
        D.k_row0 = (int)(((size_t)l * 2 + 0) * per_kv);
        D.v_row0 = (int)(((size_t)l * 2 + 1) * per_kv);
    }
    {
        const pk::GemvOp &o = a.op[pk::OPI_LMHEAD];
        DCK(encode_w4_tmap_units(&maps[(size_t)Lyr * 7], w_.lm_head.w, w_.lm_head.oc, w_.lm_head.ic, o.bw, 16));
        uint8_t *m = (uint8_t *)dalloc((size_t)o.num_tiles * o.S * pk::kMetaBytes);
        if (!m) return cudaErrorMemoryAllocation;
        const W4Seg lm[1] = {seg_of(w_.lm_head)};
        DCK(pk::repack_meta(ctx_, lm, 1, 0, o.IC, m, s));
        a.lm_meta = m;
        DCK(pk::encode_kv_tmap(&maps[(size_t)Lyr * 7 + 1], d_kv_.get(), (long long)Lyr * 2 * per_kv));
    }
    CUtensorMap *dmaps = (CUtensorMap *)dalloc(maps.size() * sizeof(CUtensorMap));
    pk::LayerDesc *ddesc = (pk::LayerDesc *)dalloc(descs.size() * sizeof(pk::LayerDesc));
    a.nsplit_max = pk::attn_nsplit_max(ncta, KVH, cfg_.max_ctx);
    const size_t n_qkv = (size_t)(H + 2 * KVH) * 64, n_attn = (size_t)H * 64, n_act = (size_t)F / 2, n_part = (size_t)H * a.nsplit_max * 130;
    const size_t ll_words = n_qkv + n_attn + n_act + n_part + (tp ? 0 : (size_t)2 * E);
    uint2 *ll = (uint2 *)dalloc(ll_words * sizeof(uint2));
    uint8_t *ctl = (uint8_t *)dalloc(32);
    if (!dmaps || !ddesc || !ll || !ctl) return cudaErrorMemoryAllocation;
    DCK(cudaMemcpyAsync(dmaps, maps.data(), maps.size() * sizeof(CUtensorMap), cudaMemcpyHostToDevice, s));
    DCK(cudaMemcpyAsync(ddesc, descs.data(), descs.size() * sizeof(pk::LayerDesc), cudaMemcpyHostToDevice, s));
    DCK(cudaMemsetAsync(ll, 0, ll_words * sizeof(uint2), s));
    DCK(cudaMemsetAsync(ctl, 0, 32, s));
    DCK(cudaStreamSynchronize(s));
    a.layers = ddesc;
    a.num_layers = Lyr;
    a.maps = dmaps;
    a.final_norm = w_.final_norm;
    a.embed = (const __half *)w_.embed_f16;
    a.embed_rows = V * tp_;
    a.qkv_ll = ll;
    a.attn_ll = a.qkv_ll + n_qkv;
    a.act_ll = a.attn_ll + n_attn;
    a.part_ll = a.act_ll + n_act;
    a.logits = io1_.logits.get();
    a.tokpos = io1_.req.get();
    a.next_token = io1_.next.get();
    a.argmax_cell = reinterpret_cast<unsigned long long *>(ctl);
    a.epoch = reinterpret_cast<unsigned *>(ctl + 8);
    a.error = reinterpret_cast<int *>(ctl + 12);
    a.done = reinterpret_cast<unsigned *>(ctl + 16);
    a.cos = d_cos_;
    a.sin = d_sin_;
    a.alpha = cfg_.qk_alpha > 0 ? cfg_.qk_alpha : 1.0f / sqrtf((float)hd);
    a.eps = cfg_.rms_eps;
    a.H = H;
    a.KVH = KVH;
    a.nrep = nrep;
    a.max_ctx = cfg_.max_ctx;
    a.V = V;
    a.F = F;
    a.tp_size = tp_;
    a.tp_rank = tp ? cfg_.tp_rank : 0;
    a.vocab_base = tp ? cfg_.tp_rank * V : 0;
    if (tp) {
        for (int q = 0; q < tp_; q++) {
            uint2 *base = reinterpret_cast<uint2 *>(tp_peer_[q]);
            a.tp_delta[0][q] = base;
            a.tp_delta[1][q] = base + (size_t)tp_ * E;
            a.tp_keys[q] = base + (size_t)2 * tp_ * E;
        }
        a.delta_ll[0] = a.tp_delta[0][a.tp_rank];
        a.delta_ll[1] = a.tp_delta[1][a.tp_rank];
    } else {
        a.delta_ll[0] = a.part_ll + n_part;
        a.delta_ll[1] = a.delta_ll[0] + E;
    }
    if (getenv("TCE_PK_DEBUG") && atoi(getenv("TCE_PK_DEBUG"))) {
        const size_t n = (size_t)ncta * ((size_t)5 * Lyr + 1) * 8 * sizeof(unsigned long long);
        a.dbg = (unsigned long long *)dalloc(n);
        if (!a.dbg) return cudaErrorMemoryAllocation;
        DCK(cudaMemset(a.dbg, 0, n));
    }
    if ((int)pk::smem_bytes(a) > ctx_->smem_optin) return no("shared memory");
    a.pair = (!getenv("TCE_PK_PAIR") || atoi(getenv("TCE_PK_PAIR")) != 0) && pk::pair_supported(ctx_, a) ? 1 : 0;
    pargs_ = a;
    return cudaSuccess;
}

cudaError_t StepIO::alloc(int n, int v) {
    V = v;
    DCK(host_alloc(h_req, (size_t)n * 3));
    DCK(dev_alloc(req, (size_t)n * 3));
    DCK(dev_alloc(logits, (size_t)n * v));
    DCK(dev_alloc(next, (size_t)n));
    DCK(host_alloc(h_logits, (size_t)n * v));
    DCK(host_alloc(h_next, (size_t)n));
    DCK(cudaMemset(req.get(), 0, (size_t)n * 3 * sizeof(int)));
    return cudaMemset(logits.get(), 0, (size_t)n * v * sizeof(float));
}

void StepIO::stage(int slot, int pos0, int n, const int *tokens) {
    for (int i = 0; i < n; i++) {
        h_req.get()[3 * i] = tokens[i];
        h_req.get()[3 * i + 1] = pos0 + i;
        h_req.get()[3 * i + 2] = slot;
    }
}

cudaError_t StepIO::read_back(int n, ReadBack r, cudaStream_t s) {
    if (r == kNone) return cudaSuccess;
    if (r == kLogitsIds) DCK(cudaMemcpyAsync(h_logits.get(), logits.get(), (size_t)n * V * sizeof(float), cudaMemcpyDeviceToHost, s));
    return cudaMemcpyAsync(h_next.get(), next.get(), (size_t)n * sizeof(int), cudaMemcpyDeviceToHost, s);
}

cudaError_t StepIO::copy_out(int n, float *logits_host, int *next_host, cudaStream_t s) const {
    DCK(cudaStreamSynchronize(s));
    if (logits_host) memcpy(logits_host, h_logits.get(), (size_t)n * V * sizeof(float));
    if (next_host) memcpy(next_host, h_next.get(), (size_t)n * sizeof(int));
    return cudaSuccess;
}

cudaError_t LlamaDecoder::step_ready(Step k, std::string *err) {
    if (k == Step::single && persistent_) return cudaSuccess;
    DCK(batch_alloc(err));
    return k == Step::span ? span_supported(err) : cudaSuccess;
}

cudaError_t LlamaDecoder::enqueue(Step k, int rows, const int *req, cudaStream_t s, bool pdl) {
    if (k == Step::single) return enqueue_step(req, s, pdl);
    return enqueue_batch(rows, req, bs_->io.logits.get(), bs_->io.next.get(), s, pdl, k == Step::span);
}

cudaError_t LlamaDecoder::enqueue_step(const int *tokpos, cudaStream_t s, bool pdl) {
    if (persistent_) {
        pk::Args m = pargs_;
        m.tokpos = tokpos;
        return pk::launch(ctx_, m, s);
    }
    int *req = io1_.req.get();
    if (tokpos != req) DCK(cudaMemcpyAsync(req, tokpos, 2 * sizeof(int), cudaMemcpyDeviceToDevice, s));
    return enqueue_batch(1, req, io1_.logits.get(), io1_.next.get(), s, pdl);
}

cudaError_t LlamaDecoder::run_graphed(CachedGraph &g, const void *key, const std::function<cudaError_t(cudaStream_t, bool)> &body) {
    cudaStream_t s = ctx_->stream;
    if (!use_graphs_) return body(s, ctx_->use_pdl);
    if (g.exec && g.key == key && g.gen == ctx_->option_gen) return cudaGraphLaunch(g.exec, s);
    g.reset();
    DCK(body(s, ctx_->use_pdl));
    for (int attempt = ctx_->use_pdl ? 0 : 1; attempt < 2; attempt++) {
        const bool pdl = attempt == 0;
        cudaGraph_t graph = nullptr;
        cudaError_t e = cudaStreamBeginCapture(cap_stream_, cudaStreamCaptureModeThreadLocal);
        if (e == cudaSuccess) {
            e = body(cap_stream_, pdl);
            const cudaError_t e2 = cudaStreamEndCapture(cap_stream_, &graph);
            if (e == cudaSuccess) e = e2;
        }
        if (e == cudaSuccess) e = cudaGraphInstantiate(&g.exec, graph, 0);
        if (graph) cudaGraphDestroy(graph);
        if (e == cudaSuccess) {
            if (!pdl) ctx_->use_pdl = false;
            g.key = key;
            g.gen = ctx_->option_gen;
            return cudaSuccess;
        }
        cudaGetLastError();
        g.exec = nullptr;
    }
    use_graphs_ = false;
    return cudaSuccess;
}

cudaError_t LlamaDecoder::run_host(Step k, int rows, StepIO::ReadBack r) {
    StepIO &b = io(k);
    return run_graphed(graphs_[{kHost, k, rows, r}], nullptr, [&](cudaStream_t st, bool pdl) {
        DCK(cudaMemcpyAsync(b.req.get(), b.h_req.get(), (size_t)rows * 3 * sizeof(int), cudaMemcpyHostToDevice, st));
        DCK(enqueue(k, rows, b.req.get(), st, pdl));
        return b.read_back(rows, r, st);
    });
}

cudaError_t LlamaDecoder::decode_host(int token, int pos, float *logits_host, int *next_token, std::string *err) {
    const int tp = cfg_.tp_size > 1 ? cfg_.tp_size : 1;
    if (pos < 0 || pos >= cfg_.max_ctx || token < 0 || token >= cfg_.vocab_size * tp) return cudaErrorInvalidValue;
    if (tp > 1 && !tp_connected_) return cudaErrorNotReady;
    DCK(step_ready(Step::single, err));
    io1_.stage(0, pos, 1, &token);
    DCK(run_host(Step::single, 1, StepIO::wanted(logits_host)));
    return io1_.copy_out(1, logits_host, next_token, ctx_->stream);
}

cudaError_t LlamaDecoder::generate(int first_token, int pos0, int n_predict, const tce_sampling &sc, const int *history_host, int n_history, int eos_id,
                                   int *out_tokens_host, int *n_out, std::string *err) {
    if (cfg_.tp_size > 1) {
        if (err) *err = "generate: single GPU only (the vocabulary is sharded under tensor parallelism)";
        return cudaErrorNotSupported;
    }
    const tce_gen_request r{first_token, pos0, 0, n_predict, eos_id, history_host, n_history, sc};
    return generate_rows(Step::single, 1, &r, out_tokens_host, n_predict, n_out, err);
}

cudaError_t LlamaDecoder::decode_device(const int *tokpos_dev, std::string *err) {
    if (tp_ > 1 && !tp_connected_) return cudaErrorNotReady;
    DCK(step_ready(Step::single, err));
    return run_graphed(graphs_[{kDevice, Step::single, 1, StepIO::kNone}], tokpos_dev,
                       [&](cudaStream_t st, bool pdl) { return enqueue_step(tokpos_dev, st, pdl); });
}

}

namespace tce {

cudaError_t LlamaDecoder::prefill_reserve(int n) {
    if (n <= pf_.cap) return cudaSuccess;
    DCK(cudaStreamSynchronize(ctx_->stream));
    pf_ = PromptBufs{};
    const size_t E = cfg_.embed_dim, F = cfg_.hidden_dim, Q = (size_t)(cfg_.num_heads + 2 * cfg_.num_kv_heads) * cfg_.head_dim,
                 A = (size_t)cfg_.num_heads * cfg_.head_dim;
    PromptBufs b;
    DCK(dev_alloc(b.x, n * E));
    DCK(dev_alloc(b.xn, n * E));
    DCK(dev_alloc(b.qkv, n * Q));
    DCK(dev_alloc(b.att, n * A));
    DCK(dev_alloc(b.act, n * F));
    DCK(dev_alloc(b.tok, (size_t)n));
    b.cap = n;
    pf_ = std::move(b);
    return cudaSuccess;
}

cudaError_t LlamaDecoder::prefill_linear(int j, const __half *x, void *C, long long ldc, int n, EpiMode epi) {
    const PfJob &job = pf_jobs_[j];
    const int ic = job.ts[0]->ic;
    size_t rows = 0;
    for (int i = 0; i < job.count; i++) rows += (size_t)job.rows[i];
    const __half *w16 = nullptr;
    DCK(pf_job_begin(j, &w16));
    if (epi == EPI_SILU_MUL_HALF)
        DCK(launch_gemm_f16_pair_silu(ctx_, x, ic, w16, ic, (__half *)C, ldc, n, (int)(rows / 2), ic));
    else
        DCK(launch_gemm_f16_pair(ctx_, x, ic, w16, ic, C, ldc, n, (int)rows, ic, epi == EPI_ADD_F32 ? 1 : 0));
    return cudaEventRecord(pf_consumed_[j & 1], ctx_->stream);
}

cudaError_t LlamaDecoder::pf_job_begin(int j, const __half **w16) {
    if (j + 1 < pf_njobs_) DCK(pf_expand_job(j + 1));
    DCK(cudaStreamWaitEvent(ctx_->stream, pf_expanded_[j & 1], 0));
    *w16 = pf_w16_[j & 1].get();
    return cudaSuccess;
}

cudaError_t LlamaDecoder::pf_expand_job(int j) {
    const PfJob &job = pf_jobs_[j];
    const int b = j & 1;
    Ctx side = *ctx_;
    side.stream = pf_side_;
    if (j >= 2) DCK(cudaStreamWaitEvent(pf_side_, pf_consumed_[b], 0));
    size_t r0 = 0;
    const int ic = job.ts[0]->ic, zw = zeros_width(ic, kW4Group);
    for (int i = 0; i < job.count; i++) {
        const tce_w4_tensor &t = *job.ts[i];
        const size_t r = (size_t)job.r0[i];
        DCK(launch_w4_expand(&side, (const uint32_t *)t.w + r * (ic / 8), (const uint32_t *)t.zeros + r * zw, (const __half *)t.scales + r * zw * 8,
                             pf_w16_[b].get() + r0 * ic, job.rows[i], ic));
        r0 += (size_t)job.rows[i];
    }
    return cudaEventRecord(pf_expanded_[b], pf_side_);
}

cudaError_t LlamaDecoder::pf_setup() {
    if (!pf_jobs_.empty()) return cudaSuccess;
    std::vector<PfJob> jobs;
    auto job = [](const tce_w4_tensor *a, const tce_w4_tensor *b, const tce_w4_tensor *c) {
        PfJob j{{a, b, c}, c ? 3 : (b ? 2 : 1), {0, 0, 0}, {0, 0, 0}};
        for (int i = 0; i < j.count; i++) j.rows[i] = j.ts[i]->oc;
        return j;
    };
    for (int l = 0; l < cfg_.num_layers; l++) {
        const tce_llama_layer &L = layers_[l];
        jobs.push_back(job(&L.q, &L.k, &L.v));
        jobs.push_back(job(&L.o, nullptr, nullptr));
        jobs.push_back(job(&L.gate, &L.up, nullptr));
        jobs.push_back(job(&L.down, nullptr, nullptr));
    }
    size_t need = 0;
    for (const PfJob &jb : jobs) {
        size_t e = 0;
        for (int i = 0; i < jb.count; i++) e += (size_t)jb.ts[i]->oc * jb.ts[i]->ic;
        need = e > need ? e : need;
    }
    const int E = cfg_.embed_dim, V = cfg_.vocab_size;
    pf_lm_chunk_ = (int)(need / (size_t)E / 256 * 256);
    for (int r0 = 0; r0 < V; r0 += pf_lm_chunk_) {
        PfJob j = job(&w_.lm_head, nullptr, nullptr);
        j.r0[0] = r0;
        j.rows[0] = V - r0 < pf_lm_chunk_ ? V - r0 : pf_lm_chunk_;
        jobs.push_back(j);
    }
    for (int b = 0; b < 2; b++) {
        DCK(dev_alloc(pf_w16_[b], need));
        if (!pf_expanded_[b]) DCK(cudaEventCreateWithFlags(&pf_expanded_[b], cudaEventDisableTiming));
        if (!pf_consumed_[b]) DCK(cudaEventCreateWithFlags(&pf_consumed_[b], cudaEventDisableTiming));
    }
    if (!pf_side_) DCK(cudaStreamCreateWithFlags(&pf_side_, cudaStreamNonBlocking));
    pf_jobs_ = std::move(jobs);
    return cudaSuccess;
}

cudaError_t LlamaDecoder::prefill_rows(int n_seqs, const int *tokens_host, const int *lengths, const int *pos0s, const int *slots, bool score) {
    int n = 0;
    for (int i = 0; i < n_seqs; i++) n += lengths[i];
    DCK(prefill_reserve(n));
    DCK(pf_setup());
    pf_njobs_ = score ? (int)pf_jobs_.size() : 4 * cfg_.num_layers;
    DCK(cudaEventRecord(pf_consumed_[0], ctx_->stream));
    DCK(cudaStreamWaitEvent(pf_side_, pf_consumed_[0], 0));
    DCK(pf_expand_job(0));
    cudaStream_t s = ctx_->stream;
    const int E = cfg_.embed_dim, F = cfg_.hidden_dim, H = cfg_.num_heads, KVH = cfg_.num_kv_heads, hd = cfg_.head_dim;
    const long long Q = (long long)(H + 2 * KVH) * hd;
    DCK(cudaMemcpyAsync(pf_.tok.get(), tokens_host, (size_t)n * sizeof(int), cudaMemcpyHostToDevice, s));
    DCK(launch_embedding_rows(ctx_, (const __half *)w_.embed_f16, pf_.tok.get(), pf_.x.get(), n, E));
    AttnPrefillArgs a{};
    a.qkv = pf_.qkv.get();
    a.cos = d_cos_;
    a.sin = d_sin_;
    a.out = pf_.att.get();
    a.alpha = cfg_.qk_alpha > 0 ? cfg_.qk_alpha : 1.0f / sqrtf((float)hd);
    a.num_heads = H;
    a.num_kv_heads = KVH;
    a.head_dim = hd;
    a.max_ctx = cfg_.max_ctx;
    a.n_seqs = n_seqs;
    for (int i = 0, row0 = 0; i < n_seqs; row0 += lengths[i++]) a.seq[i] = AttnPrefillSeq{row0, lengths[i], pos0s[i], nullptr, nullptr};
    for (int l = 0; l < cfg_.num_layers; l++) {
        const tce_llama_layer &L = layers_[l];
        DCK(launch_rmsnorm_rows_f32(ctx_, pf_.x.get(), L.input_norm, pf_.xn.get(), n, E, cfg_.rms_eps));
        DCK(prefill_linear(4 * l, pf_.xn.get(), pf_.qkv.get(), Q, n, EPI_STORE_HALF));
        for (int i = 0; i < n_seqs; i++) {
            a.seq[i].k_cache = (__half *)kv_cache_slot(slots[i], l, 0);
            a.seq[i].v_cache = (__half *)kv_cache_slot(slots[i], l, 1);
        }
        DCK(launch_attn_prefill(ctx_, a));
        DCK(prefill_linear(4 * l + 1, pf_.att.get(), pf_.x.get(), E, n, EPI_ADD_F32));
        DCK(launch_rmsnorm_rows_f32(ctx_, pf_.x.get(), L.post_norm, pf_.xn.get(), n, E, cfg_.rms_eps));
        DCK(prefill_linear(4 * l + 2, pf_.xn.get(), pf_.act.get(), F, n, EPI_SILU_MUL_HALF));
        DCK(prefill_linear(4 * l + 3, pf_.act.get(), pf_.x.get(), E, n, EPI_ADD_F32));
    }
    return cudaSuccess;
}

cudaError_t LlamaDecoder::prompt_logits(int n_seqs, const int *lengths, float *logits, int *next) {
    const int E = cfg_.embed_dim;
    for (int b = 0, row = 0; b < n_seqs; b++) {
        row += lengths[b];
        if (row - 1 != b)
            DCK(cudaMemcpyAsync(pf_.x.get() + (size_t)b * E, pf_.x.get() + (size_t)(row - 1) * E, (size_t)E * sizeof(float), cudaMemcpyDeviceToDevice,
                                ctx_->stream));
    }
    W4GemvParams p = lm_head_gemv(pf_.x.get(), logits);
    p.M = n_seqs;
    DCK(launch_w4a16_gemv(ctx_, p));
    return launch_argmax_rows(ctx_, logits, n_seqs, cfg_.vocab_size, next, false);
}

cudaError_t LlamaDecoder::prefill(const int *tokens_host, int n, int pos0, float *logits_host, int *next_token, std::string *err, int slot) {
    if (tp_ > 1) {
        if (err) *err = "prefill is single-GPU in this build (tensor-parallel ranks process the prompt with decode steps)";
        return cudaErrorNotSupported;
    }
    int rows = 0;
    DCK(check_prompts(1, tokens_host, &n, &pos0, &slot, &rows));
    DCK(prefill_rows(1, tokens_host, &n, &pos0, &slot));
    DCK(prompt_logits(1, &n, io1_.logits.get(), io1_.next.get()));
    DCK(io1_.read_back(1, StepIO::wanted(logits_host), ctx_->stream));
    return io1_.copy_out(1, logits_host, next_token, ctx_->stream);
}

}

namespace tce {

cudaError_t LlamaDecoder::batch_alloc(std::string *err) {
    auto no = [&](const char *m) {
        if (err) *err = m;
        return cudaErrorNotSupported;
// ... 549 lines not shown
```

### tinychatengine_b200/csrc/persistent.h

```cpp
#pragma once
#include "kernels.h"

namespace tce {
namespace pk {

constexpr int kCW = 16;
constexpr int kAuxWarps = 4;
constexpr int kThreads = 32 * (kAuxWarps + kCW);
constexpr int kConsumerThreads = 32 * kCW;
constexpr int kStageGroups = 32;
constexpr int kHalfBytes = 16384;
constexpr int kMetaOff = 2 * kHalfBytes;
constexpr int kMetaBytes = 1536;
constexpr int kStageBytes = 34816;
constexpr int kMaxStages = 6;
constexpr int kRedBufs = 3;
constexpr int kKvChunk = 64;

enum XMode : int { PX_HALF = 0, PX_RMS_F32 = 1 };
enum Epi : int { PE_HALF_LL = 0, PE_DELTA_LL = 1, PE_SILU_LL = 2, PE_LOGITS = 3 };
enum OpIdx : int { OPI_QKV = 0, OPI_O = 1, OPI_GATEUP = 2, OPI_DOWN = 3, OPI_LMHEAD = 4, OPI_COUNT = 5 };

struct GemvOp {
    int IC, NG;
    int bw;
    int S;
    int num_tiles;
    int nseg, pair;
    int rows0, rows1;
    int x_mode, epi;
};

struct LayerDesc {
    const uint8_t *meta[4];
    const float *input_norm, *post_norm;
    __half *k_cache, *v_cache;
    int k_row0, v_row0;
    int pad[2];
};

struct Args {
    GemvOp op[OPI_COUNT];
    const LayerDesc *layers;
    int num_layers;
    const CUtensorMap *maps;
    const uint8_t *lm_meta;
    const float *final_norm;
    const __half *embed;
    int embed_rows;
    uint2 *delta_ll[2];
    uint2 *qkv_ll;
    uint2 *attn_ll;
    uint2 *act_ll;
    uint2 *part_ll;
    float *logits;
    const int *tokpos;
    int *next_token;
    unsigned long long *argmax_cell;
    unsigned *done;
    unsigned *epoch;
    int *error;
    const float *cos, *sin;
    float alpha, eps;
    int H, KVH, nrep, max_ctx, E, V, F;
    int nsplit_max;
    int nst;
    int pair;
    int xs_bytes;
    int max_ng;
    int tp_size, tp_rank;
    uint2 *tp_delta[2][kMaxTP];
    uint2 *tp_keys[kMaxTP];
    int vocab_base;
    unsigned long long *dbg;
};

size_t smem_bytes(const Args &a);
int pick_stages(int smem_optin, int xs_bytes, int max_ng, int E);
int attn_scratch_bytes(int nrep);
int attn_nsplit_max(int ncta, int KVH, int max_ctx);
cudaError_t launch(Ctx *ctx, const Args &a, cudaStream_t stream);
bool pair_supported(Ctx *ctx, const Args &a);
cudaError_t repack_meta(Ctx *ctx, const W4Seg *segs, int nseg, int pair, int IC, uint8_t *out, cudaStream_t stream);
cudaError_t encode_kv_tmap(CUtensorMap *out, const void *kv, long long rows);

}
}
```

### tinychatengine_b200/csrc/w4a16_act_planes.cuh

```cuda
#pragma once
#include "common.cuh"

namespace tce {
namespace gemv {

constexpr float kActQ = 2130706432.f;

struct PairDst {
    uint32_t xs, gx, gsum, bar;
};
TCE_DEVINL void st_async_b32(uint32_t raddr, uint32_t v, uint32_t rbar) {
    asm volatile("st.async.weak.shared::cluster.mbarrier::complete_tx::bytes.b32 [%0], %1, [%2];" ::"r"(raddr), "r"(v), "r"(rbar) : "memory");
}

template <int NCOLS, bool PAIR = false>
TCE_DEVINL void emit_unit(uint8_t *xcol, int IC, float *gx, int *gsum, int ui, bool valid, const float (&v)[8], int lane, const PairDst *pd = nullptr) {
    float amax = 0.f;
#pragma unroll
    for (int i = 0; i < 8; i++) amax = fmaxf(amax, fabsf(v[i]));
    const unsigned half_mask = 0xFFFFu << (lane & 16);
    amax = __uint_as_float(__reduce_max_sync(half_mask, __float_as_uint(amax)));
    const float qinv = (amax > 0.f) ? (kActQ / amax) : 0.f;
    uint32_t Z[8];
#pragma unroll
    for (int i = 0; i < 8; i++) Z[i] = ((uint32_t)__float2int_rn(v[i] * qinv) + 0x80808080u) ^ 0x80808080u;
    uint32_t o3e, o2e, o1e, o0e, o3o, o2o, o1o, o0o;
    {
        const uint32_t t0 = __byte_perm(Z[0], Z[2], 0x6240), t1 = __byte_perm(Z[0], Z[2], 0x7351);
        const uint32_t u0 = __byte_perm(Z[4], Z[6], 0x6240), u1 = __byte_perm(Z[4], Z[6], 0x7351);
        o0e = __byte_perm(t0, u0, 0x5410); o2e = __byte_perm(t0, u0, 0x7632);
        o1e = __byte_perm(t1, u1, 0x5410); o3e = __byte_perm(t1, u1, 0x7632);
    }
    {
        const uint32_t t0 = __byte_perm(Z[1], Z[3], 0x6240), t1 = __byte_perm(Z[1], Z[3], 0x7351);
        const uint32_t u0 = __byte_perm(Z[5], Z[7], 0x6240), u1 = __byte_perm(Z[5], Z[7], 0x7351);
        o0o = __byte_perm(t0, u0, 0x5410); o2o = __byte_perm(t0, u0, 0x7632);
        o1o = __byte_perm(t1, u1, 0x5410); o3o = __byte_perm(t1, u1, 0x7632);
    }
    const int s3 = __dp4a((int)o3e, 0x01010101, __dp4a((int)o3o, 0x01010101, 0)), s2 = __dp4a((int)o2e, 0x01010101, __dp4a((int)o2o, 0x01010101, 0));
    const int s1 = __dp4a((int)o1e, 0x01010101, __dp4a((int)o1o, 0x01010101, 0)), s0 = __dp4a((int)o0e, 0x01010101, __dp4a((int)o0o, 0x01010101, 0));
    int sxh = s3 * 256 + s2, sxl = s1 * 256 + s0;
    const int G = ui >> 4, tj = ui & 15;
    if (NCOLS == 1) {
        if (valid) {
            uint32_t *dst = reinterpret_cast<uint32_t *>(xcol + (size_t)G * 256 + (size_t)(tj >> 2) * 32) + (tj & 3);
            dst[0] = o3e;
            dst[4] = o2e;
            dst[32] = o3o;
            dst[36] = o2o;
            uint32_t *dl = reinterpret_cast<uint32_t *>(xcol + (size_t)IC * 2 + (size_t)G * 256 + (size_t)(tj >> 2) * 32) + (tj & 3);
            dl[0] = o1e;
            dl[4] = o0e;
            dl[32] = o1o;
            dl[36] = o0o;
            if (PAIR) {
                const uint32_t ra = pd->xs + (uint32_t)G * 256u + (uint32_t)(tj >> 2) * 32u + (uint32_t)(tj & 3) * 4u, rb = ra + (uint32_t)IC * 2u;
                st_async_b32(ra, o3e, pd->bar);
                st_async_b32(ra + 16u, o2e, pd->bar);
                st_async_b32(ra + 128u, o3o, pd->bar);
                st_async_b32(ra + 144u, o2o, pd->bar);
                st_async_b32(rb, o1e, pd->bar);
                st_async_b32(rb + 16u, o0e, pd->bar);
                st_async_b32(rb + 128u, o1o, pd->bar);
                st_async_b32(rb + 144u, o0o, pd->bar);
            }
        }
    } else {
        const int pos = G * 16 + (tj & 3) * 4 + (tj >> 2);
        if (valid) {
            *reinterpret_cast<uint4 *>(xcol + (size_t)pos * 16) = make_uint4(o3e, o3o, o2e, o2o);
            *reinterpret_cast<uint4 *>(xcol + (size_t)IC * 2 + (size_t)pos * 16) = make_uint4(o1e, o1o, o0e, o0o);
        }
    }
    sxh = __reduce_add_sync(half_mask, sxh);
    sxl = __reduce_add_sync(half_mask, sxl);
    if (valid && (lane & 15) == 0) {
        const float step = (amax > 0.f) ? (amax / kActQ) : 0.f;
        gx[G] = step;
        gsum[G * 2] = sxh;
        gsum[G * 2 + 1] = sxl;
        if (PAIR) {
            st_async_b32(pd->gx + (uint32_t)G * 4u, __float_as_uint(step), pd->bar);
            st_async_b32(pd->gsum + (uint32_t)G * 8u, (uint32_t)sxh, pd->bar);
            st_async_b32(pd->gsum + (uint32_t)G * 8u + 4u, (uint32_t)sxl, pd->bar);
        }
    }
}

}
}
```

### tinychatengine_b200/csrc/w4a16_gemv.cu

```cuda
#include <stdio.h>

#include "w4a16_gemv_impl.cuh"

namespace tce {

namespace {

using namespace gemv;

template <int NCOLS, int CW>
__global__ void __launch_bounds__(32 * (kProducerWarps + 1 + CW), (NCOLS == 1 && CW == 8) ? 2 : 1) w4a16_gemv_kernel(const __grid_constant__ KArgs a) {
    extern __shared__ __align__(128) uint8_t smem[];
    using L = Layout<NCOLS, CW>;
    const int xw = a.sl * 128;
    const Smem sm = carve<NCOLS, CW>(smem, a.IC, a.nst, xw);
    const int tid = threadIdx.x, warp = tid >> 5, lane = tid & 31;
    const int cta = blockIdx.x, ncta = gridDim.x;

    if (a.pdl_early) pdl_launch_dependents();
    if (warp == 0) {
        if (lane == 0) dbg_stamp(a, cta, 0);
        init_barriers_warp<CW>(sm, lane);
    } else if (tid == 32) {
        for (int i = 0; i < a.nseg; i++) asm volatile("prefetch.tensormap [%0];" ::"l"(&a.tmap[i]) : "memory");
    }
    if (warp == 0) {
        __syncwarp();
        asm volatile("bar.arrive 3, %0;" ::"r"(32 * (kProducerWarps + 1 + CW)) : "memory");
    } else if (warp == kProducerWarps) {
        asm volatile("bar.sync 3, %0;" ::"r"(32 * (kProducerWarps + 1 + CW)) : "memory");
    }

    if (warp < kProducerWarps) {
        produce<NCOLS>(a, sm, cta, ncta, lane, l2_policy_evict_first());
        pdl_launch_dependents();
        return;
    }
    if (warp == kProducerWarps) {
        pdl_wait();
        epilogue<NCOLS, CW>(a, sm, cta, ncta, lane);
        if (lane == 0) dbg_stamp(a, cta, 5);
        return;
    }
    const int ctid = tid - 32 * (kProducerWarps + 1);
    const int cw = warp - (kProducerWarps + 1);
    pdl_wait();
    if (a.x_mode == X_RMSNORM_F32) rms_partials<NCOLS, CW>(a, sm, ctid, cw, lane);
    const int s0 = first_slice<NCOLS>(a, cta, ncta);
    stage_slice<NCOLS, CW>(a, sm, L::x_pitch(xw), s0, ctid, cw, lane);
    if (ctid == 0) dbg_stamp(a, cta, 2);
    asm volatile("bar.sync 3, %0;" ::"r"(32 * (kProducerWarps + 1 + CW)) : "memory");
    if constexpr (NCOLS == 1) {
        if (a.full)
            consume1<CW, true>(a, sm, L::x_pitch(xw), s0, cta, ncta, ctid, cw, lane);
        else
            consume1<CW, false>(a, sm, L::x_pitch(xw), s0, cta, ncta, ctid, cw, lane);
    } else {
        consume_cols<NCOLS, CW>(a, sm, L::x_pitch(xw), s0, cta, ncta, ctid, cw, lane);
    }
    if (ctid == 0) dbg_stamp(a, cta, 4);
}

template <int GS>
__global__ void w4a16_gemv_simple_kernel(const KArgs a, int total_rows) {
    const int row = blockIdx.x * (blockDim.x >> 5) + (threadIdx.x >> 5);
    const int lane = threadIdx.x & 31;
    if (row >= total_rows) return;
    int si = 0, r = row;
    if (a.nseg > 1 && r >= a.seg[0].rows) {
        r -= a.seg[0].rows;
        si = 1;
        if (a.nseg > 2 && r >= a.seg[1].rows) {
            r -= a.seg[1].rows;
            si = 2;
        }
    }
    const W4Seg &s = a.seg[si];
    const uint4 *wrow = reinterpret_cast<const uint4 *>(s.w + (size_t)r * (a.IC / 8));
    const uint32_t *zrow = s.zeros + (size_t)r * a.zeros_w;
    const __half *srow = s.scales + (size_t)r * a.sf_w;
    for (int m = 0; m < a.M; m++) {
        const __half *x = reinterpret_cast<const __half *>(a.x) + (size_t)m * a.ldx;
        float acc = 0.f;
        for (int c = lane; c < a.IC / 32; c += 32) {
            const uint4 wv = wrow[c];
            const int G = c >> (GS == 128 ? 2 : 1);
            const float sc = __half2float(srow[G]);
            const float z = (float)((zrow[G >> 3] >> ((G & 7) * 4)) & 0xF);
            const uint32_t words[4] = {wv.x, wv.y, wv.z, wv.w};
#pragma unroll
            for (int j = 0; j < 4; j++) {
#pragma unroll
                for (int i = 0; i < 8; i++) {
                    const float q = (float)((words[j] >> (4 * i)) & 0xF);
                    acc += (sc * (q - z)) * __half2float(x[c * 32 + j * 8 + i]);
                }
            }
        }
        acc = warp_sum(acc);
        if (lane == 0) {
            const size_t o = (size_t)m * a.ldy + row;
            if (a.epi == EPI_STORE_HALF)
                reinterpret_cast<__half *>(a.y)[o] = __float2half(acc);
            else if (a.epi == EPI_STORE_F32)
                reinterpret_cast<float *>(a.y)[o] = acc;
            else
                reinterpret_cast<float *>(a.y)[o] += acc;
        }
    }
}

}

cudaError_t launch_w4a16_gemv_g64(Ctx *ctx, const __half *x, const uint32_t *w, const uint32_t *zeros, const __half *scales, __half *y, int M, int IC, int OC) {
    KArgs a = {};
    a.seg[0].w = w;
    a.seg[0].zeros = zeros;
    a.seg[0].scales = scales;
    a.seg[0].rows = OC;
    a.nseg = 1;
    a.IC = IC;
    a.zeros_w = zeros_width(IC, 64);
    a.sf_w = a.zeros_w * 8;
    a.M = M;
    a.ldx = IC;
    a.x = x;
    a.y = y;
    a.epi = EPI_STORE_HALF;
    a.ldy = OC;
    const int warps = 8;
    w4a16_gemv_simple_kernel<64><<<(OC + warps - 1) / warps, warps * 32, 0, ctx->stream>>>(a, OC);
    return cudaGetLastError();
}

cudaError_t encode_w4_tmap(CUtensorMap *out, const void *w, int rows, int IC, int sg, int box_rows) {
    const TmapEncodeFn fn = tmap_encoder();
    if (!fn) return cudaErrorNotSupported;
    const cuuint64_t gdim[2] = {(cuuint64_t)(IC / 8), (cuuint64_t)rows};
    const cuuint64_t gstride[1] = {(cuuint64_t)(IC / 2)};
    const cuuint32_t box[2] = {(cuuint32_t)(sg * 16), (cuuint32_t)box_rows};
    const cuuint32_t estr[2] = {1, 1};
    const CUresult r = fn(out, CU_TENSOR_MAP_DATA_TYPE_UINT32, 2, const_cast<void *>(w), gdim, gstride, box, estr, CU_TENSOR_MAP_INTERLEAVE_NONE,
                          CU_TENSOR_MAP_SWIZZLE_NONE, CU_TENSOR_MAP_L2_PROMOTION_L2_256B, CU_TENSOR_MAP_FLOAT_OOB_FILL_NONE);
    return r == CUDA_SUCCESS ? cudaSuccess : cudaErrorInvalidValue;
}

cudaError_t encode_w4_tmap_units(CUtensorMap *out, const void *w, int rows, int IC, int sg, int box_rows) {
    const TmapEncodeFn fn = tmap_encoder();
    if (!fn) return cudaErrorNotSupported;
    const cuuint64_t gdim[3] = {16, (cuuint64_t)rows, (cuuint64_t)(IC / 128)};
    const cuuint64_t gstride[2] = {(cuuint64_t)(IC / 2), 64};
    const cuuint32_t box[3] = {16, (cuuint32_t)box_rows, (cuuint32_t)sg};
    const cuuint32_t estr[3] = {1, 1, 1};
    const CUresult r = fn(out, CU_TENSOR_MAP_DATA_TYPE_UINT32, 3, const_cast<void *>(w), gdim, gstride, box, estr, CU_TENSOR_MAP_INTERLEAVE_NONE,
                          CU_TENSOR_MAP_SWIZZLE_NONE, CU_TENSOR_MAP_L2_PROMOTION_L2_256B, CU_TENSOR_MAP_FLOAT_OOB_FILL_NONE);
    return r == CUDA_SUCCESS ? cudaSuccess : cudaErrorInvalidValue;
}

namespace {

KArgs make_kargs(Ctx *ctx, const W4GemvParams &p, int *total_rows) {
    KArgs a;
    for (int i = 0; i < 3; i++) a.seg[i] = p.seg[i < p.nseg ? i : 0];
    a.nseg = p.nseg;
    a.pair_mode = p.pair_mode;
    a.IC = p.IC;
    a.NG = p.IC / kW4Group;
    a.zeros_w = zeros_width(p.IC, kW4Group);
    a.sf_w = a.zeros_w * 8;
    int rows = 0;
    for (int i = 0; i < p.nseg; i++) rows += p.seg[i].rows;
    *total_rows = rows;
    a.num_tiles = rows / 16;
    a.M = p.M;
    a.ldx = p.ldx ? p.ldx : p.IC;
    a.x_mode = p.x_mode;
    a.x = p.x;
    a.gamma = p.gamma;
    a.eps = p.eps;
    a.y = p.y;
    a.epi = p.epi;
    a.ldy = p.ldy ? p.ldy : (p.pair_mode ? rows / 2 : rows);
    a.partials = ctx->gemv_partials;
    a.counters = ctx->gemv_counters;
    a.dbg = ctx->gemv_dbg;
    a.pdl_early = 0;
    a.nst = kStages;
    a.atomic_add = (p.atomic_residual && p.epi == EPI_ADD_F32 && !p.pair_mode) ? 1 : 0;
    a.aligned = 0;
    a.sg = a.NG < kStageGroups ? a.NG : kStageGroups;
    a.full = (a.NG % kStageGroups == 0) ? 1 : 0;
    a.sl = a.NG;
    a.nsl = 1;
    return a;
}

template <int NCOLS, int CW>
int ring_fit(int IC, int xw, int budget, int max_nst) {
    for (int nst = max_nst; nst >= 2; nst--)
        if ((int)Layout<NCOLS, CW>::bytes(IC, nst, xw) <= budget) return nst;
    return 0;
}

template <int CW>
int pick_slice(int IC, int budget) {
    const int NG = IC / kW4Group;
    if (ring_fit<8, CW>(IC, IC, budget, kStages) == kStages) return NG;
    for (int sl = (NG - 1) / kStageGroups * kStageGroups; sl >= kStageGroups; sl -= kStageGroups)
        if (ring_fit<8, CW>(IC, sl * kW4Group, budget, kStages) >= kStages) return sl;
    return ring_fit<8, CW>(IC, kStageGroups * kW4Group, budget, kStages) ? kStageGroups : 0;
}

template <int NCOLS, int CW>
cudaError_t launch_mma(Ctx *ctx, const KArgs &a_in, bool pdl) {
    KArgs a = a_in;
    const int xw = a.sl * kW4Group;
    if (!ring_fit<NCOLS, CW>(a.IC, xw, ctx->smem_optin, kStages)) return cudaErrorInvalidConfiguration;
    static DeviceOnce attr_once;
    if (attr_once.pending(ctx->device)) {
        cudaError_t e = cudaFuncSetAttribute(w4a16_gemv_kernel<NCOLS, CW>, cudaFuncAttributeMaxDynamicSharedMemorySize, ctx->smem_optin);
        if (e != cudaSuccess) return e;
        attr_once.done(ctx->device);
    }
    const long long U = (long long)a.num_tiles * a.NG;
    int per_sm = ctx->gemv_ctas_per_sm;
    a.pdl_early = (pdl && ctx->pdl_early) ? 1 : 0;
    const bool allow2 = !(pdl && ctx->pdl_early == 2);
    if (allow2 && per_sm == 1 && NCOLS == 1 && CW == 8 && a.IC <= 8192 && U >= (long long)ctx->num_sms * 2 * 128) per_sm = 2;
    int nc = ctx->num_sms * per_sm;
    if (nc > ctx->gemv_max_ctas) nc = ctx->gemv_max_ctas;
    const long long cuts = a.full ? U / kStageGroups : U;
    if ((long long)nc > cuts) nc = (int)cuts;
    if (a.nsl > 1) {
        if ((long long)nc > (long long)a.num_tiles * a.nsl) nc = a.num_tiles * a.nsl;
        if ((long long)a.num_tiles * a.nsl > ctx->gemv_partial_records) return cudaErrorInvalidValue;
    }
    a.aligned = (!a.atomic_add && a.num_tiles >= nc && a.nsl == 1) ? 1 : 0;
    {
        const int budget = ctx->smem_optin / per_sm - (per_sm > 1 ? 1024 : 0);
        int nst = ctx->gemv_stages > 0 ? ctx->gemv_stages : kMaxStages;
        if (nst > kMaxStages) nst = kMaxStages;
        const int fit = ring_fit<NCOLS, CW>(a.IC, xw, budget, nst);
        nst = fit ? fit : 2;
        const long long stages_per_cta = (U / nc + a.sg - 1) / a.sg + 1;
        if (nst > stages_per_cta && stages_per_cta >= 2) nst = (int)stages_per_cta;
        a.nst = nst;
    }
    const size_t smem = Layout<NCOLS, CW>::bytes(a.IC, a.nst, xw);
    cudaLaunchConfig_t cfg = {};
    cfg.gridDim = dim3(nc);
    cfg.blockDim = dim3(32 * (kProducerWarps + 1 + CW));
    cfg.dynamicSmemBytes = smem;
    cfg.stream = ctx->stream;
    cudaLaunchAttribute attr[1];
    attr[0].id = cudaLaunchAttributeProgrammaticStreamSerialization;
    attr[0].val.programmaticStreamSerializationAllowed = 1;
    cfg.attrs = attr;
    cfg.numAttrs = pdl ? 1 : 0;
    return cudaLaunchKernelEx(&cfg, w4a16_gemv_kernel<NCOLS, CW>, a);
}

}

cudaError_t launch_w4a16_gemv_simple(Ctx *ctx, const W4GemvParams &p) {
    if (p.pair_mode || p.x_mode != X_HALF) return cudaErrorNotSupported;
    int rows;
    KArgs a = make_kargs(ctx, p, &rows);
    const int warps = 8;
    w4a16_gemv_simple_kernel<kW4Group><<<(rows + warps - 1) / warps, warps * 32, 0, ctx->stream>>>(a, rows);
    return cudaGetLastError();
}

namespace {
int consumer_warps(const Ctx *ctx, const W4GemvParams &p) {
    return ctx->gemv_consumer_warps == 16 ? 16 : (ctx->gemv_consumer_warps == 8 ? 8 : (p.IC > 8192 && p.M == 1 ? 16 : 8));
}
int slice_of(const Ctx *ctx, const W4GemvParams &p) {
    return consumer_warps(ctx, p) == 16 ? pick_slice<16>(p.IC, ctx->smem_optin) : pick_slice<8>(p.IC, ctx->smem_optin);
}
}

long long w4a16_gemv_fixup_records(const Ctx *ctx, const W4GemvParams &p) {
    if (p.M <= 1 || p.IC < kW4Group) return 0;
    const int NG = p.IC / kW4Group, sl = slice_of(ctx, p);
    if (sl <= 0 || sl >= NG) return 0;
    int rows = 0;
    for (int i = 0; i < p.nseg && i < 3; i++) rows += p.seg[i].rows;
    return (long long)(rows / 16) * ((NG + sl - 1) / sl);
}

cudaError_t gemv_partials_reserve(Ctx *ctx, long long records) {
    if (records <= ctx->gemv_partial_records) return cudaSuccess;
    if (records > (1ll << 24)) return cudaErrorInvalidValue;
    cudaStreamCaptureStatus st = cudaStreamCaptureStatusNone;
    cudaError_t e = cudaStreamIsCapturing(ctx->stream, &st);
    if (e != cudaSuccess) return e;
    if (st != cudaStreamCaptureStatusNone) return cudaErrorStreamCaptureUnsupported;
    float *p = nullptr;
    e = cudaMalloc(&p, (size_t)records * 16 * 8 * sizeof(float));
    if (e != cudaSuccess) return e;
    e = cudaFree(ctx->gemv_partials);
    if (e != cudaSuccess) {
        cudaFree(p);
        return e;
    }
    ctx->gemv_partials = p;
    ctx->gemv_partial_records = (int)records;
    ctx->option_gen++;
    return cudaSuccess;
}

cudaError_t launch_w4a16_gemv(Ctx *ctx, const W4GemvParams &p) {
    if (p.M < 1 || p.M > 8 || p.IC % kW4Group || p.nseg < 1 || p.nseg > 3) return cudaErrorInvalidValue;
    int rows;
    KArgs a = make_kargs(ctx, p, &rows);
    for (int i = 0; i < p.nseg; i++)
        if (p.seg[i].rows % (p.pair_mode ? 8 : 16)) return cudaErrorInvalidValue;
    if (p.pair_mode && (p.nseg != 2 || p.seg[0].rows != p.seg[1].rows)) return cudaErrorInvalidValue;
    if (a.num_tiles > ctx->gemv_max_tiles) return cudaErrorInvalidValue;
    for (int i = 0; i < p.nseg; i++) {
        cudaError_t e = encode_w4_tmap(&a.tmap[i], p.seg[i].w, p.seg[i].rows, p.IC, a.sg, p.pair_mode ? 8 : 16);
        if (e != cudaSuccess) return e;
    }
    const int cw = consumer_warps(ctx, p);
    if (p.M == 1) return (cw == 16) ? launch_mma<1, 16>(ctx, a, p.pdl) : launch_mma<1, 8>(ctx, a, p.pdl);
    a.sl = slice_of(ctx, p);
    if (a.sl == 0) return cudaErrorInvalidConfiguration;
    a.nsl = (a.NG + a.sl - 1) / a.sl;
    if (a.nsl > kMaxSlices) return cudaErrorInvalidConfiguration;
    if (a.nsl > 1) {
        cudaError_t e = gemv_partials_reserve(ctx, (long long)a.num_tiles * a.nsl);
        if (e != cudaSuccess) return e;
        a.partials = ctx->gemv_partials;
    }
    return (cw == 16) ? launch_mma<8, 16>(ctx, a, p.pdl) : launch_mma<8, 8>(ctx, a, p.pdl);
}

}
```

Measured before the change: 494.4.

## Split K across cluster pair CTAs instead of exchanging activation planes

Reworks the two-CTA cluster pair mode so each CTA of a pair owns half of the input groups (K range), with separate tensor maps and metadata per rank, instead of both CTAs quantizing and exchanging the full activation planes via st.async. Each CTA now only stages and quantizes its own half of the activations into a smaller plane, and the pair combines partial dot products through a small per-slot reduction buffer with mbarriers. The producer streams per-box stages (two 16-group boxes per stage) with per-box metadata. This removes remote activation traffic and halves per-CTA activation work, but adds a cross-CTA partial-sum exchange and more tensor-map/metadata sets.

```diff
diff --git a/tinychatengine_b200/csrc/decode_persistent.cu b/tinychatengine_b200/csrc/decode_persistent.cu
--- a/tinychatengine_b200/csrc/decode_persistent.cu
+++ b/tinychatengine_b200/csrc/decode_persistent.cu
@@ -114,12 +114,6 @@
 }
 TCE_DEVINL void mbar_arrive_u32(uint32_t bar) { asm volatile("mbarrier.arrive.shared::cta.b64 _, [%0];" ::"r"(bar) : "memory"); }
 
-TCE_DEVINL int lds_volatile_i32(const int *p) {
-    int v;
-    asm volatile("ld.volatile.shared.s32 %0, [%1];" : "=r"(v) : "r"(smem_u32(p)) : "memory");
-    return v;
-}
-
 TCE_DEVINL void stamp(const Args &a, int cta, int nphase, int p, int k) {
     if (a.dbg) {
         unsigned long long t;
@@ -142,14 +136,19 @@
     int *gsum;
     float *red;
     float *rms;
+    float *inv;
     float *rope;
     uint64_t *full, *empty, *red_full, *red_empty;
     uint64_t *rx;
-    int *free_gen;
+    float *prx;
+    uint64_t *prx_full;
+    uint64_t *pfree;
     int2 *red_pos;
     uint32_t ring_u32, xs_u32, gx_u32, gsum_u32, full_u32, empty_u32, redfull_u32, redempty_u32;
     int nst;
 };
+
+__host__ __device__ inline int resid_floats(const Args &a) { return a.pair ? plane_ic(a.E / kW4Group, 1) : a.E; }
 
 TCE_DEVINL PSmem carve(uint8_t *raw, const Args &a) {
     PSmem s;
@@ -160,7 +159,7 @@
     s.xs = p;
     p += a.xs_bytes;
     s.resid = reinterpret_cast<float *>(p);
-    p += (size_t)a.E * 4;
+    p += (size_t)resid_floats(a) * 4;
     s.gx = reinterpret_cast<float *>(p);
     p += (size_t)a.max_ng * 4;
     s.gsum = reinterpret_cast<int *>(p);
@@ -169,15 +168,20 @@
     p += (size_t)kRedBufs * kCW * 16 * 4;
     s.rms = reinterpret_cast<float *>(p);
     p += 32 * 4;
+    s.inv = reinterpret_cast<float *>(p);
+    p += kCW * 4;
     s.rope = reinterpret_cast<float *>(p);
     p += 256 * 4;
+    s.prx = reinterpret_cast<float *>(p);
+    p += kPairSlots * 16 * 4;
     s.full = reinterpret_cast<uint64_t *>(p);
     s.empty = s.full + a.nst;
     s.red_full = s.empty + a.nst;
     s.red_empty = s.red_full + kRedBufs;
     s.rx = s.red_empty + kRedBufs;
-    s.free_gen = reinterpret_cast<int *>(s.rx + 1);
-    s.red_pos = reinterpret_cast<int2 *>(s.rx + 2);
+    s.prx_full = s.rx + 1;
+    s.pfree = s.prx_full + kPairSlots;
+    s.red_pos = reinterpret_cast<int2 *>(s.pfree + kPairSlots);
     s.ring_u32 = smem_u32(s.ring);
     s.xs_u32 = smem_u32(s.xs);
     s.gx_u32 = smem_u32(s.gx);
@@ -210,7 +214,11 @@
     }
 };
 
-TCE_DEVINL void partition(const GemvOp &op, int cta, int ncta, int &t0, int &t1) {
+TCE_DEVINL void partition(const GemvOp &op, int cta, int ncta, int pair, int &t0, int &t1) {
+    if (pair) {
+        cta >>= 1;
+        ncta >>= 1;
+    }
     const unsigned T = (unsigned)op.num_tiles;
     t0 = (int)((T * (unsigned)cta) / (unsigned)ncta);
     t1 = (int)((T * (unsigned)(cta + 1)) / (unsigned)ncta);
@@ -240,38 +248,43 @@
     return s;
 }
 
-TCE_DEVINL void produce_gemv(const GemvOp &op, const CUtensorMap *m0, const uint8_t *meta, const PSmem &sm, Ring &rs, int cta, int ncta, uint32_t leader,
-                             uint64_t policy) {
+TCE_DEVINL void produce_gemv(const GemvOp &op, const CUtensorMap *m0, const uint8_t *meta, const PSmem &sm, Ring &rs, int cta, int ncta, int pair, int rank,
+                             uint32_t leader, uint64_t policy) {
     int t0, t1;
-    partition(op, cta, ncta, t0, t1);
-    const uint32_t box_bytes = 16u * (uint32_t)op.bw * 64u;
-    for (int tile = t0; tile < t1; tile++) {
-        int row = op.pair ? tile * 8 : tile * 16;
-        const CUtensorMap *m = m0;
-        if (!op.pair && op.nseg > 1 && row >= op.rows0) {
-            row -= op.rows0;
-            m = m0 + 1;
-            if (op.nseg > 2 && row >= op.rows1) {
-                row -= op.rows1;
-                m = m0 + 2;
-            }
-        }
-        for (int s = 0; s < op.S; s++) {
-            const int nbox = (min(kStageGroups, op.NG - kStageGroups * s) + 15) >> 4;
-            mbar_wait(&sm.empty[rs.stage], rs.phase ^ 1);
-            uint64_t *bar = &sm.full[rs.stage];
-            uint8_t *dst = sm.ring + (size_t)rs.stage * kStageBytes;
-            mbar_arrive_expect_tx_pred(bar, (uint32_t)nbox * box_bytes + kMetaBytes, leader);
+    partition(op, cta, ncta, pair, t0, t1);
+    const KRange kr = k_range(op.NG, pair, rank);
+    const uint32_t box_bytes = 16u * (uint32_t)kr.bw * 64u;
+    const int nbox = (t1 - t0) * kr.nb;
+    const uint8_t *rec = meta + (size_t)t0 * kr.nb * kBoxMetaBytes;
+    int tile = t0, box = 0;
+    for (int i = 0; i < nbox; i += 2) {
+        const int n = min(2, nbox - i);
+        mbar_wait(&sm.empty[rs.stage], rs.phase ^ 1);
+        uint64_t *bar = &sm.full[rs.stage];
+        uint8_t *dst = sm.ring + (size_t)rs.stage * kStageBytes;
+        mbar_arrive_expect_tx_pred(bar, (uint32_t)n * (box_bytes + kBoxMetaBytes), leader);
 #pragma unroll 1
-            for (int b = 0; b < nbox; b++) {
-                const int grp = kStageGroups * s + 16 * b;
-                tma_load_3d_pred(dst + b * 16384, m, 0, row, grp, bar, policy, leader);
-                if (op.pair) tma_load_3d_pred(dst + b * 16384 + 8192, m + 1, 0, row, grp, bar, policy, leader);
-            }
-            bulk_g2s_pred(dst + kMetaOff, meta + ((size_t)tile * op.S + s) * kMetaBytes, kMetaBytes, bar, policy, leader);
-            __syncwarp();
-            rs.advance(sm.nst);
-        }
+        for (int b = 0; b < n; b++) {
+            int row = op.pair ? tile * 8 : tile * 16;
+            const CUtensorMap *m = m0;
+            if (!op.pair && op.nseg > 1 && row >= op.rows0) {
+                row -= op.rows0;
+                m = m0 + 1;
+                if (op.nseg > 2 && row >= op.rows1) {
+                    row -= op.rows1;
+                    m = m0 + 2;
+                }
+            }
+            tma_load_3d_pred(dst + b * 16384, m, 0, row, box * kBoxGroups, bar, policy, leader);
+            if (op.pair) tma_load_3d_pred(dst + b * 16384 + 8192, m + 1, 0, row, box * kBoxGroups, bar, policy, leader);
+            if (++box == kr.nb) {
+                box = 0;
+                tile++;
+            }
+        }
+        bulk_g2s_pred(dst + kMetaOff, rec + (size_t)i * kBoxMetaBytes, (uint32_t)n * kBoxMetaBytes, bar, policy, leader);
+        __syncwarp();
+        rs.advance(sm.nst);
     }
 }
 
@@ -293,23 +306,25 @@
     }
 }
 
-TCE_DEVINL void producer_walk(const Args &a, const PSmem &sm, int cta, int ncta, int pos, int lane) {
+TCE_DEVINL void producer_walk(const Args &a, const PSmem &sm, int cta, int ncta, int rank, int pos, int lane) {
     Ring rs;
     const uint64_t policy = l2_policy_evict_first();
     const uint32_t leader = (lane == 0) ? 1u : 0u;
     const int Lyr = a.num_layers, nphase = 5 * Lyr + 1;
     const CUtensorMap *kvmap = a.maps + (size_t)Lyr * 7 + 1;
+    const int set = a.pair ? 1 + rank : 0;
+    const CUtensorMap *wmaps = a.maps + (size_t)set * (Lyr * 7 + 2);
 #pragma unroll 1
     for (int p = 0; p < nphase; p++) {
         const int l = p / 5, k = p - 5 * l;
         if (l == Lyr) {
-            produce_gemv(a.op[OPI_LMHEAD], a.maps + (size_t)Lyr * 7, a.lm_meta, sm, rs, cta, ncta, leader, policy);
+            produce_gemv(a.op[OPI_LMHEAD], wmaps + (size_t)Lyr * 7, a.lm_meta[set], sm, rs, cta, ncta, a.pair, rank, leader, policy);
         } else if (k == 1) {
             produce_attn(a, a.layers[l], kvmap, sm, rs, cta, ncta, pos, leader, policy);
         } else {
             const int oi = (k == 0) ? OPI_QKV : (k - 1);
             const int mi = (k == 0) ? 0 : (k == 2 ? 3 : (k == 3 ? 4 : 6));
-            produce_gemv(a.op[oi], a.maps + (size_t)l * 7 + mi, a.layers[l].meta[oi], sm, rs, cta, ncta, leader, policy);
+            produce_gemv(a.op[oi], wmaps + (size_t)l * 7 + mi, a.layers[l].meta[set][oi], sm, rs, cta, ncta, a.pair, rank, leader, policy);
         }
     }
 }
@@ -317,8 +332,7 @@
 struct PairCtx {
     bool on = false;
     uint32_t rank = 0;
-    gemv::PairDst dst = {0u, 0u, 0u, 0u};
-    uint32_t r_rms = 0, r_free = 0;
+    uint32_t r_rms = 0, r_bar = 0;
     uint32_t nstage = 0;
 };
 TCE_DEVINL uint32_t map_to_cta(uint32_t local_u32, uint32_t rank) {
@@ -326,22 +340,24 @@
     asm volatile("mapa.shared::cluster.u32 %0, %1, %2;" : "=r"(r) : "r"(local_u32), "r"(rank));
     return r;
 }
-TCE_DEVINL void st_cluster_u32(uint32_t raddr, uint32_t v) { asm volatile("st.relaxed.cluster.shared::cluster.u32 [%0], %1;" ::"r"(raddr), "r"(v) : "memory"); }
-TCE_DEVINL int own_groups(const PairCtx &pc, int NG) { return pc.on ? (NG + 1 - (int)pc.rank) / 2 : NG; }
-TCE_DEVINL int peer_groups(const PairCtx &pc, int NG) { return pc.on ? (NG + (int)pc.rank) / 2 : 0; }
-TCE_DEVINL void wait_partner_free(const PSmem &sm, const PairCtx &pc, int p) {
-    if (!pc.on || p == 0) return;
+TCE_DEVINL void st_async_b32(uint32_t raddr, uint32_t v, uint32_t rbar) {
+    asm volatile("st.async.weak.shared::cluster.mbarrier::complete_tx::bytes.b32 [%0], %1, [%2];" ::"r"(raddr), "r"(v), "r"(rbar) : "memory");
+}
+TCE_DEVINL void mbar_arrive_remote(uint32_t rbar) { asm volatile("mbarrier.arrive.relaxed.cluster.shared::cluster.b64 _, [%0];" ::"r"(rbar) : "memory"); }
+TCE_DEVINL void mbar_wait_cluster(uint32_t bar, uint32_t parity) {
     const long long t0 = clock64();
-    while (lds_volatile_i32(sm.free_gen) < p) {
+    while (true) {
+        uint32_t ok;
+        asm volatile("{\n\t.reg .pred p;\n\tmbarrier.try_wait.parity.acquire.cluster.shared::cta.b64 p, [%1], %2;\n\tselp.u32 %0, 1, 0, p;\n\t}"
+                     : "=r"(ok) : "r"(bar), "r"(parity) : "memory");
+        if (ok) return;
         if (clock64() - t0 > kSpinLimit) __trap();
     }
 }
-TCE_DEVINL void rx_expect(const PSmem &sm, const PairCtx &pc, uint32_t bytes) {
-    asm volatile("mbarrier.arrive.expect_tx.shared::cta.b64 _, [%0], %1;" ::"r"(smem_u32(sm.rx)), "r"(bytes) : "memory");
-}
-TCE_DEVINL void rx_wait(const PSmem &sm, PairCtx &pc) {
-    mbar_wait_u32(smem_u32(sm.rx), pc.nstage & 1u);
-    pc.nstage++;
+TCE_DEVINL uint32_t cluster_rank() {
+    uint32_t r;
+    asm volatile("mov.u32 %0, %%cluster_ctarank;" : "=r"(r));
+    return r;
 }
 
 TCE_DEVINL int rot_unit(int u, int units, int cta) {
@@ -351,13 +367,10 @@
     return (g << 4) | (u & 15);
 }
 
-TCE_DEVINL void stage_half(const GemvOp &op, const PSmem &sm, PairCtx &pc, const uint2 *src, uint32_t tag, int cta, int ctid, int lane, int p) {
-    const int ng_own = own_groups(pc, op.NG);
-    const int units = ng_own * 16;
-    if (pc.on) {
-        if (ctid == 0) rx_expect(sm, pc, (uint32_t)peer_groups(pc, op.NG) * 524u);
-        wait_partner_free(sm, pc, p);
-    }
+TCE_DEVINL void stage_half(const GemvOp &op, const PSmem &sm, const PairCtx &pc, const uint2 *src, uint32_t tag, int cta, int ctid, int lane) {
+    const KRange kr = k_range(op.NG, pc.on, pc.rank);
+    const int units = kr.ng * 16;
+    const int xic = plane_ic(op.NG, pc.on);
     constexpr int PRE = 4;
     for (int ub = 0; ub < units; ub += PRE * kConsumerThreads) {
         uint4 w[PRE][2];
@@ -366,14 +379,11 @@
         for (int k = 0; k < PRE; k++) {
             const int u = ub + k * kConsumerThreads + ctid;
             ui[k] = -1;
-            if (u < units) {
-                const int ru = rot_unit(u, units, cta);
-                ui[k] = pc.on ? (((ru >> 4) * 2 + (int)pc.rank) << 4) | (ru & 15) : ru;
-            }
+            if (u < units) ui[k] = rot_unit(u, units, cta);
             w[k][0] = w[k][1] = make_uint4(0u, tag, 0u, tag);
             if (ui[k] >= 0) {
-                w[k][0] = ld_ll2(src + (size_t)ui[k] * 4, false);
-                w[k][1] = ld_ll2(src + (size_t)ui[k] * 4 + 2, false);
+                w[k][0] = ld_ll2(src + (size_t)(kr.g0 * 16 + ui[k]) * 4, false);
+                w[k][1] = ld_ll2(src + (size_t)(kr.g0 * 16 + ui[k]) * 4 + 2, false);
             }
         }
         {
@@ -388,8 +398,8 @@
 #pragma unroll
                 for (int k = 0; k < PRE; k++) {
                     if (ui[k] >= 0 && !(w[k][0].y == tag && w[k][0].w == tag && w[k][1].y == tag && w[k][1].w == tag)) {
-                        w[k][0] = ld_ll2(src + (size_t)ui[k] * 4, false);
-                        w[k][1] = ld_ll2(src + (size_t)ui[k] * 4 + 2, false);
+                        w[k][0] = ld_ll2(src + (size_t)(kr.g0 * 16 + ui[k]) * 4, false);
+                        w[k][1] = ld_ll2(src + (size_t)(kr.g0 * 16 + ui[k]) * 4 + 2, false);
                     }
                 }
             }
@@ -403,14 +413,10 @@
             const float2 f0 = h2_to_f2(w[k][0].x), f1 = h2_to_f2(w[k][0].z), f2 = h2_to_f2(w[k][1].x), f3 = h2_to_f2(w[k][1].z);
             v[0] = f0.x; v[1] = f0.y; v[2] = f1.x; v[3] = f1.y;
             v[4] = f2.x; v[5] = f2.y; v[6] = f3.x; v[7] = f3.y;
-            if (pc.on)
-                gemv::emit_unit<1, true>(sm.xs, op.IC, sm.gx, sm.gsum, valid ? ui[k] : 0, valid, v, lane, &pc.dst);
-            else
-                gemv::emit_unit<1>(sm.xs, op.IC, sm.gx, sm.gsum, valid ? ui[k] : 0, valid, v, lane);
+            gemv::emit_unit<1>(sm.xs, xic, sm.gx, sm.gsum, valid ? ui[k] : 0, valid, v, lane);
         }
     }
     named_bar_sync(1, kConsumerThreads);
-    if (pc.on) rx_wait(sm, pc);
 }
 
 TCE_DEVINL void tp_accumulate(float (&x)[8], const uint2 *slot0, int tp_size, int E, uint32_t tag) {
@@ -445,32 +451,34 @@
     }
 }
 
-TCE_DEVINL float stage_rms(const Args &a, const GemvOp &op, const PSmem &sm, PairCtx &pc, const uint2 *delta, uint32_t tag, const float *gamma, int token,
-                           bool first, bool emit, int cta, int ctid, int cw, int lane, int p) {
-    const int units = own_groups(pc, op.NG) * 16;
-    const bool sys = a.tp_size > 1;
-    if (pc.on && emit) {
-        if (ctid == 0) rx_expect(sm, pc, (uint32_t)peer_groups(pc, op.NG) * 524u + (uint32_t)kCW * 4u);
-        wait_partner_free(sm, pc, p);
-    }
+TCE_DEVINL float rms_inv(const PSmem &sm, int nparts, int IC, float eps) {
+    float tot = 0.f;
+    for (int w = 0; w < nparts; w++) tot += sm.rms[w];
+    return rsqrtf(tot / (float)IC + eps);
+}
+
+TCE_DEVINL float stage_rms(const Args &a, const GemvOp &op, const PSmem &sm, const PairCtx &pc, const uint2 *delta, uint32_t tag, const float *gamma, int token,
+                           bool first, bool emit, int cta, int ctid, int cw, int lane) {
+    const KRange kr = k_range(op.NG, pc.on, pc.rank);
+    const int units = kr.ng * 16;
+    const int xic = plane_ic(op.NG, pc.on);
+    if (pc.on && emit && ctid == 0)
+        asm volatile("mbarrier.arrive.expect_tx.shared::cta.b64 _, [%0], %1;" ::"r"(smem_u32(sm.rx)), "r"((uint32_t)kCW * 4u) : "memory");
     float ss = 0.f;
     for (int ui0 = 0; ui0 < units; ui0 += kConsumerThreads) {
         const int u = ui0 + ctid;
         const bool valid = u < units;
-        int ui = 0;
-        if (valid) {
-            const int ru = rot_unit(u, units, cta);
-            ui = pc.on ? (((ru >> 4) * 2 + (int)pc.rank) << 4) | (ru & 15) : ru;
-        }
+        const int ui = valid ? rot_unit(u, units, cta) : 0;
+        const int gu = kr.g0 * 16 + ui;
         float x[8], v[8];
 #pragma unroll
         for (int i = 0; i < 8; i++) x[i] = 0.f;
         float4 g0 = make_float4(0.f, 0.f, 0.f, 0.f), g1 = g0;
         if (valid) {
-            g0 = *reinterpret_cast<const float4 *>(gamma + (size_t)ui * 8);
-            g1 = *reinterpret_cast<const float4 *>(gamma + (size_t)ui * 8 + 4);
+            g0 = *reinterpret_cast<const float4 *>(gamma + (size_t)gu * 8);
+            g1 = *reinterpret_cast<const float4 *>(gamma + (size_t)gu * 8 + 4);
             if (first) {
-                const uint4 raw = *reinterpret_cast<const uint4 *>(a.embed + (size_t)token * a.E + (size_t)ui * 8);
+                const uint4 raw = *reinterpret_cast<const uint4 *>(a.embed + (size_t)token * a.E + (size_t)gu * 8);
                 const __half2 *h2 = reinterpret_cast<const __half2 *>(&raw);
 #pragma unroll
                 for (int i = 0; i < 4; i++) {
@@ -485,11 +493,11 @@
                 x[4] = r1.x; x[5] = r1.y; x[6] = r1.z; x[7] = r1.w;
                 if (a.tp_size == 1) {
                     uint4 w[4];
-                    wait_ll2xN<4>(delta + (size_t)ui * 8, tag, false, w);
+                    wait_ll2xN<4>(delta + (size_t)gu * 8, tag, false, w);
                     x[0] += __uint_as_float(w[0].x); x[1] += __uint_as_float(w[0].z); x[2] += __uint_as_float(w[1].x); x[3] += __uint_as_float(w[1].z);
                     x[4] += __uint_as_float(w[2].x); x[5] += __uint_as_float(w[2].z); x[6] += __uint_as_float(w[3].x); x[7] += __uint_as_float(w[3].z);
                 } else {
-                    tp_accumulate(x, delta + (size_t)ui * 8, a.tp_size, a.E, tag);
+                    tp_accumulate(x, delta + (size_t)gu * 8, a.tp_size, a.E, tag);
                 }
             }
             *reinterpret_cast<float4 *>(sm.resid + (size_t)ui * 8) = make_float4(x[0], x[1], x[2], x[3]);
@@ -500,24 +508,17 @@
             for (int i = 0; i < 8; i++) ss += x[i] * x[i];
             v[0] = x[0] * g0.x; v[1] = x[1] * g0.y; v[2] = x[2] * g0.z; v[3] = x[3] * g0.w;
             v[4] = x[4] * g1.x; v[5] = x[5] * g1.y; v[6] = x[6] * g1.z; v[7] = x[7] * g1.w;
-            if (pc.on)
-                gemv::emit_unit<1, true>(sm.xs, op.IC, sm.gx, sm.gsum, ui, valid, v, lane, &pc.dst);
-            else
-                gemv::emit_unit<1>(sm.xs, op.IC, sm.gx, sm.gsum, ui, valid, v, lane);
+            gemv::emit_unit<1>(sm.xs, xic, sm.gx, sm.gsum, ui, valid, v, lane);
         }
     }
     if (!emit) return 1.f;
     ss = warp_sum(ss);
     if (lane == 0) {
         sm.rms[pc.rank * kCW + cw] = ss;
-        if (pc.on) gemv::st_async_b32(pc.r_rms + (uint32_t)(pc.rank * kCW + cw) * 4u, __float_as_uint(ss), pc.dst.bar);
+        if (pc.on) st_async_b32(pc.r_rms + (uint32_t)(pc.rank * kCW + cw) * 4u, __float_as_uint(ss), pc.r_bar);
     }
     named_bar_sync(1, kConsumerThreads);
-    if (pc.on) rx_wait(sm, pc);
-    float tot = 0.f;
-    const int nparts = pc.on ? 2 * kCW : kCW;
-    for (int w = 0; w < nparts; w++) tot += sm.rms[w];
-    return rsqrtf(tot / (float)op.IC + a.eps);
+    return pc.on ? 0.f : rms_inv(sm, kCW, op.IC, a.eps);
 }
 
 struct UnitRegs {
@@ -525,9 +526,8 @@
     uint32_t z;
     uint32_t sc;
     int sxv;
-    float st;
 };
-TCE_DEVINL void unit_compute(const UnitRegs &u, float lscale, float &totA, float &totB) {
+TCE_DEVINL void unit_compute(const UnitRegs &u, uint32_t st_addr, float lscale, float &totA, float &totB) {
     constexpr uint32_t ML = 0x0f0f0f0fu, MH = 0xf0f0f0f0u;
     int accL[4], accH[4];
     mma_m16n8k32_u8s8_z(accL, u.wa.x & ML, u.wb.x & ML, u.wa.y & ML, u.wb.y & ML, u.xe.x, u.xe.y);
@@ -535,7 +535,7 @@
     mma_m16n8k32_u8s8(accL, u.wa.z & ML, u.wb.z & ML, u.wa.w & ML, u.wb.w & ML, u.xe.z, u.xe.w);
     mma_m16n8k32_u8s8(accH, u.wa.z & MH, u.wb.z & MH, u.wa.w & MH, u.wb.w & MH, u.xo.z, u.xo.w);
     const float2 sc = h2_to_f2(u.sc);
-    const float st = u.st * lscale;
+    const float st = lds_f32(st_addr) * lscale;
     const int zAq = (int)(u.z & 0xFFu), zBq = (int)(u.z >> 8);
     const int vA = (accL[0] << 8) + accL[1] + (((accH[0] << 8) + accH[1]) >> 4) - zAq * u.sxv;
     const int vB = (accL[2] << 8) + accL[3] + (((accH[2] << 8) + accH[3]) >> 4) - zBq * u.sxv;
@@ -543,10 +543,34 @@
     totB += (sc.y * st) * (float)vB;
 }
 
-TCE_DEVINL void consume_gemv(const Args &a, const GemvOp &op, const PSmem &sm, Ring &rs, float inv_in, int cta, int ncta, int cw, int p, int nphase) {
+TCE_DEVINL void hand_tile(const Args &a, const GemvOp &op, const PSmem &sm, Red &cs, float totA, float totB, int cw, int lane) {
+    const int g = lane >> 2, t = lane & 3;
+    float inv = sm.inv[cw];
+    if (inv < 0.f) {
+        mbar_wait_u32(smem_u32(sm.rx), inv < -1.5f ? 1u : 0u);
+        inv = rms_inv(sm, 2 * kCW, op.IC, a.eps);
+        __syncwarp();
+        if (lane == 0) sm.inv[cw] = inv;
+    }
+    totA += __shfl_xor_sync(0xffffffffu, totA, 1);
+    totB += __shfl_xor_sync(0xffffffffu, totB, 1);
+    mbar_wait_u32(sm.redempty_u32 + (uint32_t)cs.rb * 8u, cs.rphase ^ 1);
+    float *rbuf = sm.red + ((size_t)cs.rb * kCW + cw) * 16;
+    if (t == 0) {
+        rbuf[g] = totA * inv;
+        rbuf[g + 8] = totB * inv;
+    }
+    __syncwarp();
+    if (lane == 0) mbar_arrive_u32(sm.redfull_u32 + (uint32_t)cs.rb * 8u);
+    cs.advance();
+}
+
+TCE_DEVINL void consume_gemv(const Args &a, const GemvOp &op, const PSmem &sm, Ring &rs, float inv, int rx_parity, int cta, int ncta, int rank, int cw, int p,
+                             int nphase) {
     int lane;
     asm volatile("mov.u32 %0, %%laneid;" : "=r"(lane));
-    const float inv = __shfl_sync(0xffffffffu, inv_in, 0);
+    if (lane == 0) sm.inv[cw] = rx_parity >= 0 ? -1.f - (float)rx_parity : inv;
+    __syncwarp();
     Red cs;
     {
         const int2 rp = sm.red_pos[cw];
@@ -555,73 +579,78 @@
     }
     const int g = lane >> 2, t = lane & 3;
     int t0, t1;
-    partition(op, cta, ncta, t0, t1);
-    const int NG = op.NG, S = op.S;
+    partition(op, cta, ncta, a.pair, t0, t1);
+    const KRange kr = k_range(op.NG, a.pair, rank);
+    const int nb = kr.nb, nbox = (t1 - t0) * nb;
+    const int lim = kr.ng - cw;
     const uint32_t w_lane = (uint32_t)cw * (op.pair ? 512u : 1024u) + (uint32_t)g * 64u + (uint32_t)t * 16u;
     const uint32_t wb_off = op.pair ? 8192u : 512u;
     const uint32_t m_lane = (uint32_t)kMetaOff + (uint32_t)(cw * 8 + g) * 4u;
-    const uint32_t z_lane = (uint32_t)kMetaOff + 1024u + (uint32_t)(cw * 8 + g) * 2u;
-    const uint32_t x_lane = sm.xs_u32 + (uint32_t)((g >> 1) & 1) * (uint32_t)op.IC * 2u + (uint32_t)(t * 2 + (g & 1)) * 16u + (uint32_t)cw * 256u;
+    const uint32_t z_lane = (uint32_t)kMetaOff + 512u + (uint32_t)(cw * 8 + g) * 2u;
+    const uint32_t x_lane = sm.xs_u32 + (uint32_t)((g >> 1) & 1) * (uint32_t)plane_ic(op.NG, a.pair) * 2u + (uint32_t)(t * 2 + (g & 1)) * 16u + (uint32_t)cw * 256u;
     const uint32_t s_lane = sm.gsum_u32 + (uint32_t)(2 * cw + (t & 1)) * 4u;
     const uint32_t q_lane = sm.gx_u32 + (uint32_t)cw * 4u;
     const float lscale = (t == 0) ? 65536.f : (t == 1 ? 1.f : 0.f);
     const bool xl = g < 4;
-    if (a.dbg && t1 > t0 && cw == 0 && lane == 0) {
+    if (a.dbg && nbox > 0 && cw == 0 && lane == 0) {
         mbar_wait_u32(sm.full_u32 + (uint32_t)rs.stage * 8u, rs.phase);
         stamp(a, cta, nphase, p, 4);
     }
-    for (int tile = t0; tile < t1; tile++) {
-        float totA = 0.f, totB = 0.f;
-        for (int s = 0; s < S; s++) {
-            const bool has0 = kStageGroups * s + cw < NG, has1 = kStageGroups * s + cw + 16 < NG;
-            mbar_wait_u32(sm.full_u32 + (uint32_t)rs.stage * 8u, rs.phase);
-            const uint32_t base = sm.ring_u32 + (uint32_t)rs.stage * (uint32_t)kStageBytes;
-            const uint32_t wb_ = base + w_lane, mb_ = base + m_lane, zb_ = base + z_lane;
-            const uint32_t xb_ = x_lane + (uint32_t)s * (kStageGroups * 256u), sb_ = s_lane + (uint32_t)s * (kStageGroups * 8u), qb_ = q_lane + (uint32_t)s * (kStageGroups * 4u);
-            UnitRegs u0, u1;
-            u0.xe = u0.xo = u1.xe = u1.xo = make_uint4(0u, 0u, 0u, 0u);
-            if (has0) {
-                u0.wa = lds_u4(wb_);
-                u0.wb = lds_u4(wb_ + wb_off);
-                if (xl) {
-                    u0.xe = lds_u4(xb_);
-                    u0.xo = lds_u4(xb_ + 128u);
-                }
-                u0.sc = lds_u32(mb_);
-                u0.z = lds_u16(zb_);
-                u0.sxv = (int)lds_u32(sb_);
-                u0.st = lds_f32(qb_);
-            }
-            if (has1) {
-                u1.wa = lds_u4(wb_ + 16384u);
-                u1.wb = lds_u4(wb_ + 16384u + wb_off);
-                if (xl) {
-                    u1.xe = lds_u4(xb_ + 4096u);
-                    u1.xo = lds_u4(xb_ + 4096u + 128u);
-                }
-                u1.sc = lds_u32(mb_ + 512u);
-                u1.z = lds_u16(zb_ + 256u);
-                u1.sxv = (int)lds_u32(sb_ + 128u);
-                u1.st = lds_f32(qb_ + 64u);
-            }
-            if (has0) unit_compute(u0, lscale, totA, totB);
-            if (has1) unit_compute(u1, lscale, totA, totB);
-            __syncwarp();
-            if (lane == 0) mbar_arrive_u32(sm.empty_u32 + (uint32_t)rs.stage * 8u);
-            rs.advance(sm.nst);
-        }
-        if (tile == t1 - 1 && cw == 0 && lane == 0) stamp(a, cta, nphase, p, 5);
-        totA += __shfl_xor_sync(0xffffffffu, totA, 1);
-        totB += __shfl_xor_sync(0xffffffffu, totB, 1);
-        mbar_wait_u32(sm.redempty_u32 + (uint32_t)cs.rb * 8u, cs.rphase ^ 1);
-        float *rbuf = sm.red + ((size_t)cs.rb * kCW + cw) * 16;
-        if (t == 0) {
-            rbuf[g] = totA * inv;
-            rbuf[g + 8] = totB * inv;
-        }
+    int box = 0;
+    float totA = 0.f, totB = 0.f;
+    for (int left = nbox; left > 0; left -= 2) {
+        const int box0 = box, box1 = (box0 + 1 == nb) ? 0 : box0 + 1;
+        const bool two = left > 1;
+        box = (box1 + 1 == nb) ? 0 : box1 + 1;
+        const bool has0 = box0 * kBoxGroups < lim, has1 = two && box1 * kBoxGroups < lim;
+        mbar_wait_u32(sm.full_u32 + (uint32_t)rs.stage * 8u, rs.phase);
+        const uint32_t base = sm.ring_u32 + (uint32_t)rs.stage * (uint32_t)kStageBytes;
+        const uint32_t wb_ = base + w_lane, mb_ = base + m_lane, zb_ = base + z_lane;
+        UnitRegs u0, u1;
+        u0.xe = u0.xo = u1.xe = u1.xo = make_uint4(0u, 0u, 0u, 0u);
+        if (has0) {
+            const uint32_t xb_ = x_lane + (uint32_t)box0 * 4096u;
+            u0.wa = lds_u4(wb_);
+            u0.wb = lds_u4(wb_ + wb_off);
+            if (xl) {
+                u0.xe = lds_u4(xb_);
+                u0.xo = lds_u4(xb_ + 128u);
+            }
+            u0.sc = lds_u32(mb_);
+            u0.z = lds_u16(zb_);
+            u0.sxv = (int)lds_u32(s_lane + (uint32_t)box0 * 128u);
+        }
+        if (has1) {
+            const uint32_t xb_ = x_lane + (uint32_t)box1 * 4096u;
+            u1.wa = lds_u4(wb_ + 16384u);
+            u1.wb = lds_u4(wb_ + 16384u + wb_off);
+            if (xl) {
+                u1.xe = lds_u4(xb_);
+                u1.xo = lds_u4(xb_ + 128u);
+            }
+            u1.sc = lds_u32(mb_ + (uint32_t)kBoxMetaBytes);
+            u1.z = lds_u16(zb_ + (uint32_t)kBoxMetaBytes);
+            u1.sxv = (int)lds_u32(s_lane + (uint32_t)box1 * 128u);
+        }
+        if (has0) unit_compute(u0, q_lane + (uint32_t)box0 * 64u, lscale, totA, totB);
+        const bool end0 = box0 + 1 == nb;
+        float hA = 0.f, hB = 0.f;
+        if (end0) {
+            hA = totA;
+            hB = totB;
+            totA = totB = 0.f;
+        }
+        if (has1) unit_compute(u1, q_lane + (uint32_t)box1 * 64u, lscale, totA, totB);
         __syncwarp();
-        if (lane == 0) mbar_arrive_u32(sm.redfull_u32 + (uint32_t)cs.rb * 8u);
-        cs.advance();
+        if (lane == 0) mbar_arrive_u32(sm.empty_u32 + (uint32_t)rs.stage * 8u);
+        rs.advance(sm.nst);
+        if (left <= 2 && cw == 0 && lane == 0) stamp(a, cta, nphase, p, 5);
+        const bool end1 = two && box1 + 1 == nb;
+        if (end0) hand_tile(a, op, sm, cs, hA, hB, cw, lane);
+        if (end1) {
+            hand_tile(a, op, sm, cs, totA, totB, cw, lane);
+            totA = totB = 0.f;
+        }
     }
     __syncwarp();
     if (lane == 0) sm.red_pos[cw] = make_int2(cs.rb, (int)cs.rphase);
@@ -631,6 +660,7 @@
 
 struct EpiState {
     unsigned long long best;
+    uint32_t nsent, nrecv;
 };
 
 TCE_DEVINL void epilogue_gemv(const Args &a, const GemvOp &op, const PSmem &sm, Red &es, EpiState &st, uint2 *out_ll, int which, uint32_t tag, int cta, int ncta,
@@ -638,8 +668,10 @@
     int lane;
     asm volatile("mov.u32 %0, %%laneid;" : "=r"(lane));
     int t0, t1;
-    partition(op, cta, ncta, t0, t1);
+    partition(op, cta, ncta, a.pair, t0, t1);
     const bool tp = a.tp_size > 1;
+    const uint32_t rank = a.pair ? cluster_rank() : 2u;
+    const int tsplit = t0 + (t1 - t0 + 1) / 2;
     for (int tile = t0; tile < t1; tile++) {
         mbar_wait_u32(sm.redfull_u32 + (uint32_t)es.rb * 8u, es.rphase);
         if (tile == t1 - 1 && lane == 0) stamp(a, cta, nphase, p, 7);
@@ -654,6 +686,24 @@
         __syncwarp();
         if (lane == 0) mbar_arrive_u32(sm.redempty_u32 + (uint32_t)es.rb * 8u);
         es.advance();
+        if (rank < 2u) {
+            const bool mine = (tile >= tsplit) == (rank == 1u);
+            const uint32_t slot = (mine ? st.nrecv : st.nsent) % kPairSlots;
+            if (!mine) {
+                const uint32_t n = st.nsent++;
+                mbar_wait_cluster(smem_u32(sm.pfree + slot), ((n / kPairSlots) & 1u) ^ 1u);
+                if (lane < 16)
+                    st_async_b32(map_to_cta(smem_u32(sm.prx + slot * 16 + lane), rank ^ 1u), __float_as_uint(v), map_to_cta(smem_u32(sm.prx_full + slot), rank ^ 1u));
+                continue;
+            }
+            const uint32_t n = st.nrecv++;
+            const uint32_t fb = smem_u32(sm.prx_full + slot);
+            if (lane == 0) asm volatile("mbarrier.arrive.expect_tx.shared::cta.b64 _, [%0], %1;" ::"r"(fb), "r"(64u) : "memory");
+            mbar_wait_u32(fb, (n / kPairSlots) & 1u);
+            v += sm.prx[slot * 16 + (lane & 15)];
+            __syncwarp();
+            if (lane == 0) mbar_arrive_remote(map_to_cta(smem_u32(sm.pfree + slot), rank ^ 1u));
+        }
         switch (op.epi) {
             case PE_DELTA_LL:
                 if (lane < 16) {
@@ -930,9 +980,10 @@
             mbar_init(&sm.red_full[lane - 16], kCW);
             mbar_init(&sm.red_empty[lane - 16], 1);
         }
-        if (lane == 30) {
-            mbar_init(sm.rx, 1);
-            *sm.free_gen = 0;
+        if (lane == 30) mbar_init(sm.rx, 1);
+        if (lane >= 24 && lane < 24 + kPairSlots) {
+            mbar_init(&sm.prx_full[lane - 24], 1);
+            mbar_init(&sm.pfree[lane - 24], 1);
         }
         mbar_fence_init();
     }
@@ -942,14 +993,9 @@
         asm volatile("barrier.cluster.arrive.release.aligned;" ::: "memory");
         asm volatile("barrier.cluster.wait.acquire.aligned;" ::: "memory");
         pc.on = true;
-        asm volatile("mov.u32 %0, %%cluster_ctarank;" : "=r"(pc.rank));
-        const uint32_t peer = pc.rank ^ 1u;
-        pc.dst.xs = map_to_cta(sm.xs_u32, peer);
-        pc.dst.gx = map_to_cta(sm.gx_u32, peer);
-        pc.dst.gsum = map_to_cta(sm.gsum_u32, peer);
-        pc.dst.bar = map_to_cta(smem_u32(sm.rx), peer);
-        pc.r_rms = map_to_cta(smem_u32(sm.rms), peer);
-        pc.r_free = map_to_cta(smem_u32(sm.free_gen), peer);
+        pc.rank = cluster_rank();
+        pc.r_rms = map_to_cta(smem_u32(sm.rms), pc.rank ^ 1u);
+        pc.r_bar = map_to_cta(smem_u32(sm.rx), pc.rank ^ 1u);
     }
     const int nphase = 5 * Lyr + 1;
     const unsigned epoch = *a.epoch;
@@ -959,12 +1005,13 @@
         asm volatile("setmaxnreg.dec.sync.aligned.u32 64;" ::: "memory");
         if (warp >= 2) return;
         if (warp == 0) {
-            producer_walk(a, sm, cta, ncta, pos, lane);
+            producer_walk(a, sm, cta, ncta, (int)pc.rank, pos, lane);
             return;
         }
         Red es;
         EpiState st;
         st.best = 0ull;
+        st.nsent = st.nrecv = 0u;
 #pragma unroll 1
         for (int p = 0; p < nphase; p++) {
             const int l = p / 5, k = p - 5 * l;
@@ -973,6 +1020,9 @@
             uint2 *out = (oi == OPI_QKV) ? a.qkv_ll : (oi == OPI_GATEUP ? a.act_ll : (oi == OPI_O ? a.delta_ll[0] : a.delta_ll[1]));
             epilogue_gemv(a, a.op[oi], sm, es, st, out, (oi == OPI_DOWN) ? 1 : 0, tag_base + 2u * (uint32_t)p, cta, ncta, p, nphase);
             if (lane == 0) stamp(a, cta, nphase, p, 3);
+        }
+        if (a.pair) {
+            for (uint32_t n = st.nsent; n < st.nsent + kPairSlots; n++) mbar_wait_cluster(smem_u32(sm.pfree + n % kPairSlots), ((n / kPairSlots) & 1u) ^ 1u);
         }
         unsigned long long key = st.best;
 #pragma unroll
@@ -1003,35 +1053,29 @@
             attention_phase(a, a.layers[l], sm, rs, tag_in, tag_base + 2u * (uint32_t)p + 1u, tag_base + 2u * (uint32_t)p, cta, ncta, pos, ctid, cw, lane, p, nphase);
             if (ctid == 0) stamp(a, cta, nphase, p, 2);
             named_bar_sync(1, kConsumerThreads);
-            if (pc.on && ctid == 0) st_cluster_u32(pc.r_free, (uint32_t)(p + 1));
             continue;
         }
         const int oi = (l == Lyr) ? OPI_LMHEAD : ((k == 0) ? OPI_QKV : (k - 1));
         const GemvOp &op = a.op[oi];
         int t0, t1;
-        partition(op, cta, ncta, t0, t1);
+        partition(op, cta, ncta, pc.on, t0, t1);
         const bool work = t1 > t0;
-        bool stage = work;
-        if (pc.on) {
-            int u0, u1;
-            partition(op, cta ^ 1, ncta, u0, u1);
-            stage = work || u1 > u0;
-        }
         float inv = 1.f;
+        int rx_parity = -1;
         if (oi == OPI_O) {
-            if (stage) stage_half(op, sm, pc, a.attn_ll, tag_in, cta, ctid, lane, p);
+            if (work) stage_half(op, sm, pc, a.attn_ll, tag_in, cta, ctid, lane);
         } else if (oi == OPI_DOWN) {
-            if (stage) stage_half(op, sm, pc, a.act_ll, tag_in, cta, ctid, lane, p);
+            if (work) stage_half(op, sm, pc, a.act_ll, tag_in, cta, ctid, lane);
         } else {
             const float *gamma = (oi == OPI_LMHEAD) ? a.final_norm : (oi == OPI_QKV ? a.layers[l].input_norm : a.layers[l].post_norm);
             const uint2 *delta = (oi == OPI_GATEUP) ? a.delta_ll[0] : a.delta_ll[1];
-            inv = stage_rms(a, op, sm, pc, delta, tag_in, gamma, token, p == 0, stage, cta, ctid, cw, lane, p);
+            inv = stage_rms(a, op, sm, pc, delta, tag_in, gamma, token, p == 0, work, cta, ctid, cw, lane);
+            if (pc.on && work) rx_parity = (int)(pc.nstage++ & 1u);
         }
         if (ctid == 0) stamp(a, cta, nphase, p, 1);
-        if (work) consume_gemv(a, op, sm, rs, inv, cta, ncta, cw, p, nphase);
+        if (work) consume_gemv(a, op, sm, rs, inv, rx_parity, cta, ncta, (int)pc.rank, cw, p, nphase);
         if (ctid == 0) stamp(a, cta, nphase, p, 2);
         named_bar_sync(1, kConsumerThreads);
-        if (pc.on && ctid == 0 && p + 1 < nphase) st_cluster_u32(pc.r_free, (uint32_t)(p + 1));
     }
     if (cta == 0 && ctid == 0) {
         const unsigned target = (epoch + 1u) * (unsigned)ncta;
@@ -1059,15 +1103,15 @@
     }
 }
 
-__global__ void repack_meta_kernel(W4Seg s0, W4Seg s1, W4Seg s2, int nseg, int pair, int NG, int zeros_w, int sf_w, int S, int num_tiles, uint8_t *out) {
+__global__ void repack_meta_kernel(W4Seg s0, W4Seg s1, W4Seg s2, int nseg, int pair, int g0, int ng, int nb, int zeros_w, int sf_w, int num_tiles, uint8_t *out) {
     const int idx = blockIdx.x * blockDim.x + threadIdx.x;
-    if (idx >= num_tiles * S * kStageGroups) return;
-    const int gi = idx % kStageGroups, su = idx / kStageGroups;
-    const int tile = su / S, s = su - tile * S;
-    const int G = kStageGroups * s + gi;
-    uint8_t *rec = out + (size_t)su * kMetaBytes;
+    if (idx >= num_tiles * nb * kBoxGroups) return;
+    const int gi = idx % kBoxGroups, rb = idx / kBoxGroups;
+    const int tile = rb / nb, box = rb - tile * nb;
+    const int lg = kBoxGroups * box + gi, G = g0 + lg;
+    uint8_t *rec = out + (size_t)rb * kBoxMetaBytes;
     __half *so = reinterpret_cast<__half *>(rec) + gi * 16;
-    uint8_t *zo = rec + 1024 + gi * 16;
+    uint8_t *zo = rec + 512 + gi * 16;
     for (int r = 0; r < 16; r++) {
         const W4Seg *seg = &s0;
         int row;
@@ -1086,7 +1130,7 @@
             }
         }
         const int slot = (r & 7) * 2 + (r >> 3);
-        if (G < NG) {
+        if (lg < ng) {
             so[slot] = seg->scales[(size_t)row * sf_w + G];
             zo[slot] = (uint8_t)((seg->zeros[(size_t)row * zeros_w + (G >> 3)] >> ((G & 7) * 4)) & 0xFu);
         } else {
@@ -1107,27 +1151,29 @@
     return NS < nch ? NS : nch;
 }
 
-static size_t fixed_bytes(int xs_bytes, int max_ng, int E) {
-    return (size_t)xs_bytes + (size_t)E * 4 + (size_t)max_ng * 12 + (size_t)kRedBufs * kCW * 16 * 4 + 32 * 4 + 256 * 4 + (size_t)(2 * kMaxStages + 2 * kRedBufs) * 8 + 16 +
-           (size_t)kCW * 8 + 1024;
-}
-int pick_stages(int smem_optin, int xs_bytes, int max_ng, int E) {
-    const long long avail = (long long)smem_optin - (long long)fixed_bytes(xs_bytes, max_ng, E);
-    long long n = avail / kStageBytes;
-    if (n > kMaxStages) n = kMaxStages;
-    return n < 2 ? 0 : (int)n;
-}
-size_t smem_bytes(const Args &a) { return fixed_bytes(a.xs_bytes, a.max_ng, a.E) + (size_t)a.nst * kStageBytes; }
-
-cudaError_t repack_meta(Ctx *ctx, const W4Seg *segs, int nseg, int pair, int IC, uint8_t *out, cudaStream_t stream) {
-    const int NG = IC / kW4Group, S = (NG + kStageGroups - 1) / kStageGroups;
+static size_t fixed_bytes(const Args &a) {
+    return (size_t)a.xs_bytes + (size_t)resid_floats(a) * 4 + (size_t)a.max_ng * 12 + (size_t)kRedBufs * kCW * 16 * 4 + 32 * 4 + kCW * 4 + 256 * 4 + (size_t)kPairSlots * 16 * 4 +
+           (size_t)(2 * kMaxStages + 2 * kRedBufs + 1 + 2 * kPairSlots) * 8 + (size_t)kCW * 8 + 1024;
+}
+void plan_smem(Args &a, int smem_optin) {
+    int xs = attn_scratch_bytes(a.nrep);
+    for (int i = 0; i < OPI_COUNT; i++) xs = max(xs, 4 * plane_ic(a.op[i].NG, a.pair));
+    a.xs_bytes = (xs + 15) & ~15;
+    a.nst = 0;
+    const long long n = ((long long)smem_optin - (long long)fixed_bytes(a)) / kStageBytes;
+    if (n >= 2) a.nst = (int)(n > kMaxStages ? kMaxStages : n);
+}
+size_t smem_bytes(const Args &a) { return fixed_bytes(a) + (size_t)a.nst * kStageBytes; }
+
+cudaError_t repack_meta(Ctx *ctx, const W4Seg *segs, int nseg, int pair, int IC, const KRange &kr, uint8_t *out, cudaStream_t stream) {
     int rows = 0;
     for (int i = 0; i < nseg; i++) rows += segs[i].rows;
     const int num_tiles = rows / 16;
     const int zw = zeros_width(IC, kW4Group);
-    const int total = num_tiles * S * kStageGroups;
+    const int total = num_tiles * kr.nb * kBoxGroups;
     if (total == 0) return cudaSuccess;
-    repack_meta_kernel<<<(total + 127) / 128, 128, 0, stream>>>(segs[0], segs[nseg > 1 ? 1 : 0], segs[nseg > 2 ? 2 : 0], nseg, pair, NG, zw, zw * 8, S, num_tiles, out);
+    repack_meta_kernel<<<(total + 127) / 128, 128, 0, stream>>>(segs[0], segs[nseg > 1 ? 1 : 0], segs[nseg > 2 ? 2 : 0], nseg, pair, kr.g0, kr.ng, kr.nb, zw, zw * 8,
+                                                               num_tiles, out);
     (void)ctx;
     return cudaGetLastError();
 }
@@ -1199,7 +1245,12 @@
         cfg.numAttrs = 1;
     }
     Args single = a;
-    single.pair = 0;
+    if (a.pair) {
+        single.pair = 0;
+        plan_smem(single, ctx->smem_optin);
+        if (single.nst < 2) return cudaErrorInvalidConfiguration;
+        cfg.dynamicSmemBytes = smem_bytes(single);
+    }
     return cudaLaunchKernelEx(&cfg, decode_persistent_kernel, single);
 }
 
diff --git a/tinychatengine_b200/csrc/kernels.h b/tinychatengine_b200/csrc/kernels.h
--- a/tinychatengine_b200/csrc/kernels.h
+++ b/tinychatengine_b200/csrc/kernels.h
@@ -83,7 +83,7 @@
 cudaError_t launch_w4a16_gemv_simple(Ctx *ctx, const W4GemvParams &p);
 cudaError_t launch_w4a16_gemv_g64(Ctx *ctx, const __half *x, const uint32_t *w, const uint32_t *zeros, const __half *scales, __half *y, int M, int IC, int OC);
 cudaError_t encode_w4_tmap(CUtensorMap *out, const void *w, int rows, int IC, int sg, int box_rows);
-cudaError_t encode_w4_tmap_units(CUtensorMap *out, const void *w, int rows, int IC, int sg, int box_rows);
+cudaError_t encode_w4_tmap_units(CUtensorMap *out, const void *w, int rows, int IC, int sg, int box_rows, int g0 = 0, int ng = 0);
 
 cudaError_t launch_naive_fp16_int4(Ctx *ctx, const __half *A, const int32_t *B, const __half *scales, __half *C, int M, int IC, int OC, int block);
 cudaError_t launch_f32_matmul_transposed(Ctx *ctx, const float *A, const float *B, float *C, int M, int N, int K);
diff --git a/tinychatengine_b200/csrc/llama_decoder.cu b/tinychatengine_b200/csrc/llama_decoder.cu
--- a/tinychatengine_b200/csrc/llama_decoder.cu
+++ b/tinychatengine_b200/csrc/llama_decoder.cu
@@ -171,7 +171,6 @@
         pk::GemvOp o{};
         o.IC = IC;
         o.NG = IC / kW4Group;
-        o.S = (o.NG + pk::kStageGroups - 1) / pk::kStageGroups;
         o.num_tiles = rows / 16;
         o.nseg = nseg;
         o.pair = pair;
@@ -187,23 +186,23 @@
     a.op[pk::OPI_GATEUP] = mk(E, 2 * F, 2, 1, F, F, pk::PX_RMS_F32, pk::PE_SILU_LL);
     a.op[pk::OPI_DOWN] = mk(F, E, 1, 0, E, 0, pk::PX_HALF, pk::PE_DELTA_LL);
     a.op[pk::OPI_LMHEAD] = mk(E, V, 1, 0, V, 0, pk::PX_RMS_F32, pk::PE_LOGITS);
-    int max_ic = 0, max_ng = 0;
+    int max_ng = 0, min_ng = 1 << 30;
     for (int i = 0; i < pk::OPI_COUNT; i++) {
-        a.op[i].bw = a.op[i].NG < 16 ? a.op[i].NG : 16;
-        if (a.op[i].IC > max_ic) max_ic = a.op[i].IC;
         if (a.op[i].NG > max_ng) max_ng = a.op[i].NG;
+        if (a.op[i].NG < min_ng) min_ng = a.op[i].NG;
         if (a.op[i].IC % kW4Group || a.op[i].num_tiles < 1) return no("bad GEMV shape");
     }
-    max_ng = (max_ng + 3) & ~3;
-    int xs = 4 * max_ic;
-    if (xs < pk::attn_scratch_bytes(nrep)) xs = pk::attn_scratch_bytes(nrep);
-    xs = (xs + 15) & ~15;
-    a.xs_bytes = xs;
-    a.max_ng = max_ng;
+    a.max_ng = (max_ng + 3) & ~3;
     a.E = E;
-    a.nst = pk::pick_stages(ctx_->smem_optin, xs, max_ng, E);
+    a.nrep = nrep;
+    a.pair = (!getenv("TCE_PK_PAIR") || atoi(getenv("TCE_PK_PAIR")) != 0) && ncta % 2 == 0 && min_ng >= 2 ? 1 : 0;
+    pk::plan_smem(a, ctx_->smem_optin);
+    if (a.pair && (a.nst < 2 || !pk::pair_supported(ctx_, a))) {
+        a.pair = 0;
+        pk::plan_smem(a, ctx_->smem_optin);
+    }
     if (a.nst < 2) return no("shared memory too small for the persistent kernel");
-    a.pair = 0;
+    const int nsets = a.pair ? pk::kMapSets : 1;
 
     auto dalloc = [&](size_t bytes) -> void * {
         DevPtr<uint8_t> p;
@@ -212,7 +211,8 @@
         return pk_allocs_.back().get();
     };
     cudaStream_t s = ctx_->stream;
-    std::vector<CUtensorMap> maps((size_t)Lyr * 7 + 2);
+    const size_t nmaps = (size_t)Lyr * 7 + 2;
+    std::vector<CUtensorMap> maps(nsets * nmaps);
     memset(maps.data(), 0, maps.size() * sizeof(CUtensorMap));
     std::vector<pk::LayerDesc> descs(Lyr);
     const size_t per_kv = (size_t)KVH * cfg_.max_ctx;
@@ -220,9 +220,12 @@
         const tce_llama_layer &L = layers_[l];
         const tce_w4_tensor *t7[7] = {&L.q, &L.k, &L.v, &L.o, &L.gate, &L.up, &L.down};
         const int opi[7] = {pk::OPI_QKV, pk::OPI_QKV, pk::OPI_QKV, pk::OPI_O, pk::OPI_GATEUP, pk::OPI_GATEUP, pk::OPI_DOWN};
-        for (int i = 0; i < 7; i++) {
-            const pk::GemvOp &o = a.op[opi[i]];
-            DCK(encode_w4_tmap_units(&maps[(size_t)l * 7 + i], t7[i]->w, t7[i]->oc, t7[i]->ic, o.bw, o.pair ? 8 : 16));
+        for (int set = 0; set < nsets; set++) {
+            for (int i = 0; i < 7; i++) {
+                const pk::GemvOp &o = a.op[opi[i]];
+                const pk::KRange kr = pk::k_range(o.NG, set > 0, set - 1);
+                DCK(encode_w4_tmap_units(&maps[set * nmaps + (size_t)l * 7 + i], t7[i]->w, t7[i]->oc, t7[i]->ic, kr.bw, o.pair ? 8 : 16, kr.g0, kr.ng));
+            }
         }
         pk::LayerDesc &D = descs[l];
         memset(&D, 0, sizeof(D));
@@ -230,12 +233,15 @@
         const W4Seg *segs[4] = {qkv, o1, gu, d1};
         const int nsegs[4] = {3, 1, 2, 1}, pairs[4] = {0, 0, 1, 0};
         const int ops4[4] = {pk::OPI_QKV, pk::OPI_O, pk::OPI_GATEUP, pk::OPI_DOWN};
-        for (int i = 0; i < 4; i++) {
-            const pk::GemvOp &o = a.op[ops4[i]];
-            uint8_t *m = (uint8_t *)dalloc((size_t)o.num_tiles * o.S * pk::kMetaBytes);
-            if (!m) return cudaErrorMemoryAllocation;
-            DCK(pk::repack_meta(ctx_, segs[i], nsegs[i], pairs[i], o.IC, m, s));
-            D.meta[i] = m;
+        for (int set = 0; set < nsets; set++) {
+            for (int i = 0; i < 4; i++) {
+                const pk::GemvOp &o = a.op[ops4[i]];
+                const pk::KRange kr = pk::k_range(o.NG, set > 0, set - 1);
+                uint8_t *m = (uint8_t *)dalloc((size_t)o.num_tiles * kr.nb * pk::kBoxMetaBytes);
+                if (!m) return cudaErrorMemoryAllocation;
+                DCK(pk::repack_meta(ctx_, segs[i], nsegs[i], pairs[i], o.IC, kr, m, s));
+                D.meta[set][i] = m;
+            }
         }
         D.input_norm = L.input_norm;
         D.post_norm = L.post_norm;
@@ -246,13 +252,16 @@
     }
     {
         const pk::GemvOp &o = a.op[pk::OPI_LMHEAD];
-        DCK(encode_w4_tmap_units(&maps[(size_t)Lyr * 7], w_.lm_head.w, w_.lm_head.oc, w_.lm_head.ic, o.bw, 16));
-        uint8_t *m = (uint8_t *)dalloc((size_t)o.num_tiles * o.S * pk::kMetaBytes);
-        if (!m) return cudaErrorMemoryAllocation;
         const W4Seg lm[1] = {seg_of(w_.lm_head)};
-        DCK(pk::repack_meta(ctx_, lm, 1, 0, o.IC, m, s));
-        a.lm_meta = m;
-        DCK(pk::encode_kv_tmap(&maps[(size_t)Lyr * 7 + 1], d_kv_.get(), (long long)Lyr * 2 * per_kv));
+        for (int set = 0; set < nsets; set++) {
+            const pk::KRange kr = pk::k_range(o.NG, set > 0, set - 1);
+            DCK(encode_w4_tmap_units(&maps[set * nmaps + (size_t)Lyr * 7], w_.lm_head.w, w_.lm_head.oc, w_.lm_head.ic, kr.bw, 16, kr.g0, kr.ng));
+            uint8_t *m = (uint8_t *)dalloc((size_t)o.num_tiles * kr.nb * pk::kBoxMetaBytes);
+            if (!m) return cudaErrorMemoryAllocation;
+            DCK(pk::repack_meta(ctx_, lm, 1, 0, o.IC, kr, m, s));
+            a.lm_meta[set] = m;
+            DCK(pk::encode_kv_tmap(&maps[set * nmaps + (size_t)Lyr * 7 + 1], d_kv_.get(), (long long)Lyr * 2 * per_kv));
+        }
     }
     CUtensorMap *dmaps = (CUtensorMap *)dalloc(maps.size() * sizeof(CUtensorMap));
     pk::LayerDesc *ddesc = (pk::LayerDesc *)dalloc(descs.size() * sizeof(pk::LayerDesc));
@@ -290,7 +299,6 @@
     a.eps = cfg_.rms_eps;
     a.H = H;
     a.KVH = KVH;
-    a.nrep = nrep;
     a.max_ctx = cfg_.max_ctx;
     a.V = V;
     a.F = F;
@@ -317,7 +325,6 @@
         DCK(cudaMemset(a.dbg, 0, n));
     }
     if ((int)pk::smem_bytes(a) > ctx_->smem_optin) return no("shared memory");
-    a.pair = (!getenv("TCE_PK_PAIR") || atoi(getenv("TCE_PK_PAIR")) != 0) && pk::pair_supported(ctx_, a) ? 1 : 0;
     pargs_ = a;
     return cudaSuccess;
 }
diff --git a/tinychatengine_b200/csrc/persistent.h b/tinychatengine_b200/csrc/persistent.h
--- a/tinychatengine_b200/csrc/persistent.h
+++ b/tinychatengine_b200/csrc/persistent.h
@@ -8,13 +8,14 @@
 constexpr int kAuxWarps = 4;
 constexpr int kThreads = 32 * (kAuxWarps + kCW);
 constexpr int kConsumerThreads = 32 * kCW;
-constexpr int kStageGroups = 32;
 constexpr int kHalfBytes = 16384;
+constexpr int kBoxGroups = 16;
 constexpr int kMetaOff = 2 * kHalfBytes;
-constexpr int kMetaBytes = 1536;
+constexpr int kBoxMetaBytes = 768;
 constexpr int kStageBytes = 34816;
 constexpr int kMaxStages = 6;
 constexpr int kRedBufs = 3;
+constexpr int kPairSlots = 8;
 constexpr int kKvChunk = 64;
 
 enum XMode : int { PX_HALF = 0, PX_RMS_F32 = 1 };
@@ -23,16 +24,31 @@
 
 struct GemvOp {
     int IC, NG;
-    int bw;
-    int S;
     int num_tiles;
     int nseg, pair;
     int rows0, rows1;
     int x_mode, epi;
 };
 
+struct KRange {
+    int g0, ng;
+    int nb, bw;
+};
+__host__ __device__ inline KRange k_range(int NG, int pair, int rank) {
+    KRange k;
+    const int h = (NG + 1) / 2;
+    k.g0 = (pair && rank) ? h : 0;
+    k.ng = pair ? (rank ? NG - h : h) : NG;
+    k.nb = (k.ng + kBoxGroups - 1) / kBoxGroups;
+    k.bw = k.ng < kBoxGroups ? k.ng : kBoxGroups;
+    return k;
+}
+__host__ __device__ inline int plane_ic(int NG, int pair) { return k_range(NG, pair, 0).ng * 128; }
+
+constexpr int kMapSets = 3;
+
 struct LayerDesc {
-    const uint8_t *meta[4];
+    const uint8_t *meta[kMapSets][4];
     const float *input_norm, *post_norm;
     __half *k_cache, *v_cache;
     int k_row0, v_row0;
@@ -44,7 +60,7 @@
     const LayerDesc *layers;
     int num_layers;
     const CUtensorMap *maps;
-    const uint8_t *lm_meta;
+    const uint8_t *lm_meta[kMapSets];
     const float *final_norm;
     const __half *embed;
     int embed_rows;
@@ -76,12 +92,12 @@
 };
 
 size_t smem_bytes(const Args &a);
-int pick_stages(int smem_optin, int xs_bytes, int max_ng, int E);
+void plan_smem(Args &a, int smem_optin);
 int attn_scratch_bytes(int nrep);
 int attn_nsplit_max(int ncta, int KVH, int max_ctx);
 cudaError_t launch(Ctx *ctx, const Args &a, cudaStream_t stream);
 bool pair_supported(Ctx *ctx, const Args &a);
-cudaError_t repack_meta(Ctx *ctx, const W4Seg *segs, int nseg, int pair, int IC, uint8_t *out, cudaStream_t stream);
+cudaError_t repack_meta(Ctx *ctx, const W4Seg *segs, int nseg, int pair, int IC, const KRange &kr, uint8_t *out, cudaStream_t stream);
 cudaError_t encode_kv_tmap(CUtensorMap *out, const void *kv, long long rows);
 
 }
diff --git a/tinychatengine_b200/csrc/w4a16_act_planes.cuh b/tinychatengine_b200/csrc/w4a16_act_planes.cuh
--- a/tinychatengine_b200/csrc/w4a16_act_planes.cuh
+++ b/tinychatengine_b200/csrc/w4a16_act_planes.cuh
@@ -6,15 +6,8 @@
 
 constexpr float kActQ = 2130706432.f;
 
-struct PairDst {
-    uint32_t xs, gx, gsum, bar;
-};
-TCE_DEVINL void st_async_b32(uint32_t raddr, uint32_t v, uint32_t rbar) {
-    asm volatile("st.async.weak.shared::cluster.mbarrier::complete_tx::bytes.b32 [%0], %1, [%2];" ::"r"(raddr), "r"(v), "r"(rbar) : "memory");
-}
-
-template <int NCOLS, bool PAIR = false>
-TCE_DEVINL void emit_unit(uint8_t *xcol, int IC, float *gx, int *gsum, int ui, bool valid, const float (&v)[8], int lane, const PairDst *pd = nullptr) {
+template <int NCOLS>
+TCE_DEVINL void emit_unit(uint8_t *xcol, int IC, float *gx, int *gsum, int ui, bool valid, const float (&v)[8], int lane) {
     float amax = 0.f;
 #pragma unroll
     for (int i = 0; i < 8; i++) amax = fmaxf(amax, fabsf(v[i]));
@@ -53,17 +46,6 @@
             dl[4] = o0e;
             dl[32] = o1o;
             dl[36] = o0o;
-            if (PAIR) {
-                const uint32_t ra = pd->xs + (uint32_t)G * 256u + (uint32_t)(tj >> 2) * 32u + (uint32_t)(tj & 3) * 4u, rb = ra + (uint32_t)IC * 2u;
-                st_async_b32(ra, o3e, pd->bar);
-                st_async_b32(ra + 16u, o2e, pd->bar);
-                st_async_b32(ra + 128u, o3o, pd->bar);
-                st_async_b32(ra + 144u, o2o, pd->bar);
-                st_async_b32(rb, o1e, pd->bar);
-                st_async_b32(rb + 16u, o0e, pd->bar);
-                st_async_b32(rb + 128u, o1o, pd->bar);
-                st_async_b32(rb + 144u, o0o, pd->bar);
-            }
         }
     } else {
         const int pos = G * 16 + (tj & 3) * 4 + (tj >> 2);
@@ -79,11 +61,6 @@
         gx[G] = step;
         gsum[G * 2] = sxh;
         gsum[G * 2 + 1] = sxl;
-        if (PAIR) {
-            st_async_b32(pd->gx + (uint32_t)G * 4u, __float_as_uint(step), pd->bar);
-            st_async_b32(pd->gsum + (uint32_t)G * 8u, (uint32_t)sxh, pd->bar);
-            st_async_b32(pd->gsum + (uint32_t)G * 8u + 4u, (uint32_t)sxl, pd->bar);
-        }
     }
 }
 
diff --git a/tinychatengine_b200/csrc/w4a16_gemv.cu b/tinychatengine_b200/csrc/w4a16_gemv.cu
--- a/tinychatengine_b200/csrc/w4a16_gemv.cu
+++ b/tinychatengine_b200/csrc/w4a16_gemv.cu
@@ -145,10 +145,11 @@
     return r == CUDA_SUCCESS ? cudaSuccess : cudaErrorInvalidValue;
 }
 
-cudaError_t encode_w4_tmap_units(CUtensorMap *out, const void *w, int rows, int IC, int sg, int box_rows) {
+cudaError_t encode_w4_tmap_units(CUtensorMap *out, const void *w, int rows, int IC, int sg, int box_rows, int g0, int ng) {
     const TmapEncodeFn fn = tmap_encoder();
     if (!fn) return cudaErrorNotSupported;
-    const cuuint64_t gdim[3] = {16, (cuuint64_t)rows, (cuuint64_t)(IC / 128)};
+    w = static_cast<const uint8_t *>(w) + (size_t)g0 * 64;
+    const cuuint64_t gdim[3] = {16, (cuuint64_t)rows, (cuuint64_t)(ng ? ng : IC / 128)};
     const cuuint64_t gstride[2] = {(cuuint64_t)(IC / 2), 64};
     const cuuint32_t box[3] = {16, (cuuint32_t)box_rows, (cuuint32_t)sg};
     const cuuint32_t estr[3] = {1, 1, 1};
```

Measured after the change: 511.6 (median of 6 runs). 3.5% higher.
